# degleris1/CMF.jl

Hardware: NVIDIA B200
Metric: CNMF iterations/sec (higher is better)
Workload: dtype f32

## Files before the change

### cmf.jl_b200/_lib.py

```python
from __future__ import annotations

import ctypes
import os

import numpy as np

_HERE = os.path.dirname(os.path.abspath(__file__))
SO_PATH = os.environ.get("CMF_SM100_LIB") or os.path.join(_HERE, "libcmf_sm100.so")

F64, F32 = 0, 1
MULT, HALS, PGD = 0, 1, 2
_c = ctypes
_i64, _dbl, _int, _vp = _c.c_int64, _c.c_double, _c.c_int, _c.c_void_p
_h = _c.c_void_p

SIGNATURES = {
    "cmf_create": [_c.POINTER(_h), _i64, _i64, _i64, _i64, _int, _int, _int],
    "cmf_create_shard": [_c.POINTER(_h), _i64, _i64, _i64, _i64, _i64, _i64, _int, _int, _int],
    "cmf_create_multi": [_c.POINTER(_h), _i64, _i64, _i64, _i64, _int, _int, _int, _c.POINTER(_int)],
    "cmf_comm_unique_id": [_vp],
    "cmf_create_rank": [_c.POINTER(_h), _i64, _i64, _i64, _i64, _int, _int, _int, _vp, _int, _int],
    "cmf_shard_range": [_i64, _int, _int, _c.POINTER(_i64), _c.POINTER(_i64)],
    "cmf_comm_info": [_h, _c.POINTER(_int), _c.POINTER(_int), _c.POINTER(_i64), _c.POINTER(_i64)],
    "cmf_exchange_halos": [_h],
    "cmf_destroy": [_h],
    "cmf_set_data": [_h, _vp, _i64],
    "cmf_synth_data": [_h, _c.c_uint64, _i64, _i64, _dbl, _dbl],
    "cmf_get_data": [_h, _vp, _int],
    "cmf_data_sumsq": [_h, _c.POINTER(_dbl)],
    "cmf_set_data_norm": [_h, _dbl],
    "cmf_set_factors": [_h, _vp, _vp, _i64],
    "cmf_init_rand": [_h, _c.c_uint64],
    "cmf_init_scale_partials": [_h, _c.POINTER(_dbl)],
    "cmf_scale_factors": [_h, _dbl],
    "cmf_get_factors": [_h, _vp, _vp],
    "cmf_update_motifs": [_h, _dbl, _dbl],
    "cmf_update_feature_maps": [_h, _dbl, _dbl, _c.POINTER(_dbl)],
    "cmf_loss": [_h, _c.POINTER(_dbl)],
    "cmf_fit": [_h, _i64, _dbl, _int, _int, _int, _dbl, _dbl, _dbl, _dbl, _dbl, _c.POINTER(_dbl),
                _c.POINTER(_dbl), _i64, _c.POINTER(_i64), _c.POINTER(_int)],
    "cmf_w_partials": [_h],
    "cmf_w_apply": [_h, _dbl, _dbl],
    "cmf_h_update": [_h, _dbl, _dbl],
    "cmf_loss_partial": [_h, _c.POINTER(_dbl)],
    "cmf_exchange_buffer": [_h, _int, _c.POINTER(_vp), _c.POINTER(_i64), _c.POINTER(_int)],
    "cmf_halo_buffers": [_h, _c.POINTER(_vp), _c.POINTER(_vp), _c.POINTER(_vp), _c.POINTER(_vp),
                         _c.POINTER(_i64)],
    "cmf_sync": [_h],
    "cmf_launch_count": [_h, _c.POINTER(_i64)],
    "cmf_stream": [_h, _c.POINTER(_vp)],
    "cmf_set_stream": [_h, _vp],
    "cmf_set_engine": [_h, _int],
    "cmf_get_engine": [_h, _c.POINTER(_int)],
    "cmf_get_fd_layout": [_h, _c.POINTER(_int), _c.POINTER(_int), _c.POINTER(_i64)],
    "cmf_set_loss_mode": [_h, _int],
    "cmf_get_loss_mode": [_h, _c.POINTER(_int)],
    "cmf_set_loss_guard": [_h, _dbl, _int],
    "cmf_get_loss_stats": [_h, _c.POINTER(_i64), _c.POINTER(_i64), _c.POINTER(_int), _c.POINTER(_dbl)],
    "cmf_profile": [_h, _int],
    "cmf_profile_read": [_h, _int, _c.POINTER(_dbl), _c.POINTER(_i64)],
    "cmf_set_pgd_loss": [_h, _int, _vp],
    "cmf_set_pgd_constraints": [_h, _int, _int],
    "cmf_tensor_conv": [_i64, _i64, _i64, _i64, _int, _vp, _vp, _vp],
    "cmf_tensor_transconv": [_i64, _i64, _i64, _i64, _int, _vp, _vp, _vp],
    "cmf_corr_w": [_i64, _i64, _i64, _i64, _int, _vp, _vp, _vp],
    "cmf_compute_resids": [_i64, _i64, _i64, _i64, _int, _vp, _vp, _vp, _vp],
    "cmf_shift_and_stack": [_i64, _i64, _i64, _int, _vp, _vp],
    "cmf_create_batch": [_c.POINTER(_h), _i64, _i64, _i64, _i64, _int, _int, _i64, _int],
    "cmf_create_batch_ranks": [_c.POINTER(_h), _i64, _i64, _c.POINTER(_i64), _i64, _int, _int, _i64, _int],
    "cmf_set_factors_batch": [_h, _vp, _vp],
    "cmf_get_factors_batch": [_h, _vp, _vp],
    "cmf_init_scale_partials_batch": [_h, _c.POINTER(_dbl)],
    "cmf_scale_factors_batch": [_h, _c.POINTER(_dbl)],
    "cmf_loss_batch": [_h, _c.POINTER(_dbl)],
    "cmf_fit_batch": [_h, _i64, _dbl, _int, _int, _int, _dbl, _c.POINTER(_dbl), _c.POINTER(_dbl), _c.POINTER(_dbl),
                      _c.POINTER(_dbl), _c.POINTER(_dbl), _c.POINTER(_dbl), _i64, _c.POINTER(_i64), _c.POINTER(_int)],
}

_LIB = None


class CMFError(RuntimeError):
    def __init__(self, code, msg):
        super().__init__(f"libcmf_sm100 error {code}: {msg}")
        self.code = code


def load():
    global _LIB
    if _LIB is None:
        if not os.path.exists(SO_PATH):
            raise ImportError(
                f"{SO_PATH} is missing: build it with `python -c 'import __graft_entry__ as g; g.build()'`"
                " (the CUDA path has no CPU fallback)")
        lib = ctypes.CDLL(SO_PATH)
        for name, args in SIGNATURES.items():
            fn = getattr(lib, name)
            fn.argtypes = args
            fn.restype = _int
        lib.cmf_last_error.argtypes = []
        lib.cmf_last_error.restype = _c.c_char_p
        _LIB = lib
    return _LIB


def check(code):
    if code != 0:
        raise CMFError(code, load().cmf_last_error().decode("utf-8", "replace"))


def np_dtype(dtype):
    return np.float64 if dtype == F64 else np.float32


def parse_dtype(d):
    if d in (F64, "f64", "float64", np.float64, "Float64"):
        return F64
    if d in (F32, "f32", "float32", np.float32, "Float32"):
        return F32
    raise ValueError(f"dtype must be f64 or f32, got {d!r}")


def fptr(a):
    return a.ctypes.data_as(_vp)


def julia_array(a, dtype):
    return np.asfortranarray(a, dtype=np_dtype(dtype))
```

### cmf.jl_b200/csrc/cmf_sm100.cu

```cuda
#include "../../include/cmf_sm100.h"

#include <cuda_runtime.h>

#include <algorithm>
#include <chrono>
#include <cmath>
#include <cstdio>
#include <cstring>
#include <map>
#include <memory>
#include <numeric>
#include <mutex>
#include <tuple>
#include <stdexcept>
#include <string>
#include <vector>

#include <type_traits>
#include <variant>

#include "kernels_simt.cuh"
#include "kernels_tc.cuh"
#include "kernels_fd.cuh"
#include "kernels_hals.cuh"
// ... 143 lines not shown
CUtensorMap make_map_mn(void *base, uint64_t rows, uint64_t row_stride, uint64_t groups, uint32_t box_rows, uint32_t box_groups) {
    CUtensorMap m;
    cuuint64_t gdim[3] = {64, rows, groups};
    cuuint64_t gstr[2] = {row_stride, 128};
    cuuint32_t box[3] = {64, box_rows, box_groups};
    cuuint32_t estr[3] = {1, 1, 1};
    CUresult r = encode_tiled_fn()(&m, CU_TENSOR_MAP_DATA_TYPE_BFLOAT16, 3, base, gdim, gstr, box, estr,
                                   CU_TENSOR_MAP_INTERLEAVE_NONE, CU_TENSOR_MAP_SWIZZLE_128B, CU_TENSOR_MAP_L2_PROMOTION_L2_256B,
                                   CU_TENSOR_MAP_FLOAT_OOB_FILL_NONE);
    if (r != CUDA_SUCCESS) throw CmfError(CMF_ERR_CUDA, "cuTensorMapEncodeTiled (3-D) failed with code " + std::to_string((int)r));
    return m;
}

struct TcState {
    bool ok = false, tried = false;
    int Kp = 0, G = 0, num_sms = 148;
    int64_t KLp = 0, rows_u = 0, groups = 0, hrows = 0;
    DevBuf<__nv_bfloat16> X_hi, X_lo, Hw_hi, Hw_lo, Hm_hi, Hm_lo, Wc_hi, Wc_lo, Wu_hi, Wu_lo, Cc_hi, Cc_lo;
    CUtensorMap mWc[2], mHw[2], mHm[2], mWu[2], mXk[2], mXmn[2];
    CUtensorMap mHmn[2];
    CUtensorMap mCu[2];
    CUtensorMap mHk[2];
    CUtensorMap mGc[2];
    CUtensorMap mWuB[2], mWcB[2];
    DevBuf<__nv_bfloat16> Gc_hi, Gc_lo;
    int nsplit = 1, nsplit_g = 1;
    int64_t split_len = 0, split_len_g = 0, tiles_m = 0, tiles_n = 0, groups_c = 0, rows_c = 0;
    bool x_dirty = true, w_dirty = true;
};

struct FdState {
    bool ok = false, tried = false;
    int B = 0, logB = 0, V = 0, F = 0;
    int64_t nblk = 0, nblkp = 0;
    int Kq = 64, MR = 128;
    int V2 = 0;
    int64_t nblk2 = 0;
    DevBuf<__nv_bfloat16> Xf_hi, Xf_lo, Ah_hi, Ah_lo, Aw_hi, Aw_lo, Hf_hi, Hf_lo, Ac_hi, Ac_lo;
    DevBuf<float> Of, Df, Gf, Yf;
    DevBuf<float2> tw;
    DevBuf<__nv_bfloat16> Awm_hi, Awm_lo;
    int64_t nbc = 0;
    bool wx_dirty = true;
    CUtensorMap mXfK[2], mXfMN[2], mAw[2], mAh[2], mHfMN[2], mAc[2], mHf2K[2], mAwm[2], mHcK[2];
    bool x_dirty = true, w_dirty = true, h_dirty = true;
    bool hf2_valid = false;
    std::string why;
    void release() {
        Xf_hi.free(); Xf_lo.free(); Ah_hi.free(); Ah_lo.free(); Aw_hi.free(); Aw_lo.free(); Of.free(); Df.free();
        Hf_hi.free(); Hf_lo.free(); Gf.free(); Ac_hi.free(); Ac_lo.free(); tw.free();
        Yf.free(); Awm_hi.free(); Awm_lo.free(); nbc = 0; wx_dirty = true;
        ok = tried = false;
        x_dirty = w_dirty = h_dirty = true; hf2_valid = false;
    }
};

template <typename Fn>
void fd_with_b(int logB, Fn &&fn) {
    switch (logB) {
    case 6: fn(std::integral_constant<int, 6>{}); break;
    case 7: fn(std::integral_constant<int, 7>{}); break;
    case 8: fn(std::integral_constant<int, 8>{}); break;
    case 9: fn(std::integral_constant<int, 9>{}); break;
    case 10: fn(std::integral_constant<int, 10>{}); break;
    default: REQUIRE(false, "frequency-domain transforms: block length must be a power of two in [64, 1024]");
    }
}
template <typename Fn>
void fd_with_bc(int logB, int C, Fn &&fn) {
    fd_with_b(logB, [&](auto lb) {
        switch (C) {
        case 8: fn(lb, std::integral_constant<int, 8>{}); break;
        case 16: fn(lb, std::integral_constant<int, 16>{}); break;
        case 32: fn(lb, std::integral_constant<int, 32>{}); break;
        default: REQUIRE(false, "frequency-domain transforms: unsupported tile width");
        }
    });
}

template <typename S>
struct Ctx : RankState {
    static constexpr int dtype = std::is_same<S, double>::value ? CMF_F64 : CMF_F32;
    TcState tcs;
    FdState fds;
    DevBuf<S> X, Hbuf, Wi, Wtmp, numW, denW, GS, Cf, numH, denH, tailC;
    DevBuf<int> progress, lockstep;
    DevBuf<S> tailCt;
    int hals_grid = 0;
    DevBuf<double> exch1, corr_part, loss_part, scal;
    S *H = nullptr;
    int nsplit_w = 1, nsplit_g = 1;
    int64_t split_w = 0, split_g = 0;
    int conv_blocks_max = 0;

    static constexpr int TN = sizeof(S) == 4 ? 8 : 4;
    static constexpr int TT = 8, TY = 16;
    static constexpr int BN = 16 * TN, BT = TY * TT;

    int64_t KL() const { return K * L; }

    void hals_setup() {
        REQUIRE(L - 1 <= HW_TC, "HALS: L-1 must not exceed the sweep chunk (1024 columns)");
        const size_t smem = hals_wave_smem_elems<S>(L) * sizeof(S);
        int per_sm = 0, sms = 0, coop = 0;
        CK(cudaDeviceGetAttribute(&sms, cudaDevAttrMultiProcessorCount, device));
        CK(cudaDeviceGetAttribute(&coop, cudaDevAttrCooperativeLaunch, device));
        REQUIRE(coop != 0, "HALS needs cooperative launch support");
        CK(cudaFuncSetAttribute(hals_h_wave_kernel<S>, cudaFuncAttributeMaxDynamicSharedMemorySize, (int)smem));
        CK(cudaOccupancyMaxActiveBlocksPerMultiprocessor(&per_sm, hals_h_wave_kernel<S>, HW_NT, smem));
        hals_grid = (int)std::min<int64_t>(K, (int64_t)per_sm * sms);
        REQUIRE(hals_grid >= 1, "HALS: H sweep kernel does not fit on the device");
        tailC.alloc((size_t)hals_grid * (size_t)(L * L));
        progress.alloc((size_t)K);
    }

    void init() {
        if (R > 0) { init_batch(); return; }
        CK(cudaSetDevice(device));
        CK(cudaStreamCreateWithFlags(&stream, cudaStreamNonBlocking));
        own_stream = true;
        const int64_t hal = L - 1;
        X.alloc((size_t)((Tl + hal) * N));
        Hbuf.alloc((size_t)((Tl + 2 * hal) * K));
        H = Hbuf.p + hal * K;
        Wi.alloc((size_t)(KL() * N));
        Wtmp.alloc((size_t)(KL() * N));
        numW.alloc((size_t)(KL() * N));
        denW.alloc((size_t)(KL() * N));
        GS.alloc((size_t)(KL() * KL()));
        Cf.alloc((size_t)((2 * L - 1) * K * K));
        numH.alloc((size_t)(Tl * K));
        denH.alloc((size_t)(std::max<int64_t>(Tl * K, Tl)));
        exch1.alloc((size_t)(L * K * K + hal * K + 1));
        scal.alloc(8);
        if (alg == CMF_HALS) hals_setup();
        plan_split(N, Tl + hal, nsplit_w, split_w);
        plan_split(K, Tl + hal, nsplit_g, split_g);
        corr_part.alloc((size_t)std::max<int64_t>((int64_t)nsplit_w * KL() * N, (int64_t)nsplit_g * KL() * K));
        conv_blocks_max = (int)(cdiv(N, BN) * cdiv(Tl + hal, BT));
        loss_part.alloc((size_t)std::max(2 * conv_blocks_max, 4096));
        if constexpr (is_f32) {
            if (N >= 256 && Tl >= 4096 && K * L >= 256) {
                tc_setup();
                const char *e = getenv("CMF_ENGINE_DEFAULT");
                if (tcs.ok && engine == 1 && L >= 8 && K <= fd::KQ_MAX && !(e && atoi(e) == 1)) {
                    fd_setup();
                    if (fds.ok) { engine = 2; loss_mode = 1; }
                }
            }
        }
        CK(cudaStreamSynchronize(stream));
    }

    static constexpr bool is_f32 = std::is_same<S, float>::value;
    bool tc_active() const { return engine >= 1 && tcs.ok; }
    bool fd_active() const { return engine == 2 && tcs.ok && fds.ok; }
    bool fd_available() {
        if constexpr (is_f32) {
            if (!tc_available()) return false;
            if (!fds.ok && !fds.tried) fd_setup();
            if (fds.ok) { tcs.X_hi.free(); tcs.X_lo.free(); tcs.x_dirty = true; }
        }
        return fds.ok;
    }
    void fd_release() { fds.release(); }
    void fd_layout(int *B, int *V, int64_t *nblk) {
        *B = fd_active() ? fds.B : 0; *V = fd_active() ? fds.V : 0; *nblk = fd_active() ? fds.nblkp : 0;
    }

    void fd_setup() {
        FdState &f = fds;
        f.tried = true;
        if (!tcs.ok) { f.why = "needs the tcgen05 engine"; return; }
        if (K > fd::KQ_MAX || L > 256 || N < 16) { f.why = "needs K <= 128, L <= 256, N >= 16"; return; }
        f.Kq = (K <= 64) ? 64 : 128;
        f.MR = 2 * f.Kq;
        int B0 = 64;
        while (B0 < 8 * L && B0 < 1024) B0 *= 2;
        while (B0 < 4 * L) B0 *= 2;
        if (B0 / 2 >= 4 * L && B0 / 2 >= 64) {
            auto work = [&](int B) {
                const int64_t nb = cdiv(Tl, (int64_t)(B - (int)L + 1));
                return (double)(B / 2 + 1) * (double)(cdiv(nb, tc::BN) * tc::BN + cdiv(nb, 16) * 16);
            };
            if (work(B0) > 0.97 * work(B0 / 2)) B0 /= 2;
        }
        int forced = 0;
        if (const char *e = getenv("CMF_FD_B")) {
            const int want = atoi(e);
            if (want >= 4 * L && want >= 64 && want <= 1024 && (want & (want - 1)) == 0) forced = want;
        }
        tcs.X_hi.free(); tcs.X_lo.free(); tcs.x_dirty = true;
        size_t free_b = 0, total_b = 0;
        CK(cudaMemGetInfo(&free_b, &total_b));
        size_t later = (size_t)1 << 30;
        if (alg == CMF_HALS) later += (size_t)2 * (size_t)(Tl + 2048) * (size_t)K * 4 + (size_t)hals2::RING * (size_t)cdiv(K, hals2::GS) * (size_t)K * hals2::CW * 4;
        size_t xf = 0, ah = 0, aw = 0, of = 0, df = 0, hf = 0, gf = 0, ac = 0;
        bool fits = false;
        for (int B = forced ? forced : B0; B <= (forced ? forced : std::min(2 * B0, 1024)); B *= 2) {
            int logB = 0;
            while ((1 << logB) < B) ++logB;
            f.B = B; f.logB = logB; f.V = B - (int)L + 1; f.F = B / 2 + 1;
            f.nblk = cdiv(Tl, f.V);
            f.nblkp = cdiv(f.nblk, 16) * 16;
            xf = (size_t)f.F * (size_t)f.nblkp * 2 * (size_t)N + 64;
            ah = (size_t)f.F * (size_t)f.nblkp * 2 * f.MR + 64;
            aw = (size_t)f.F * f.MR * 2 * (size_t)N + 64;
            f.V2 = B - 2 * (int)L + 2;
            f.nblk2 = cdiv(Tl, f.V2);
            of = (size_t)f.F * (size_t)std::max(f.nblkp, f.nblk2) * f.MR; df = (size_t)f.F * f.MR * (size_t)N;
            hf = (size_t)f.F * (size_t)std::max(f.nblkp, f.nblk2) * 2 * f.Kq + 256; gf = (size_t)f.F * f.MR * f.Kq;
            ac = (size_t)f.F * f.MR * f.MR;
            const size_t need = 4 * (xf + ah + aw + hf + ac) + 4 * (of + df + gf);
            const size_t loss_pass = 4 * aw + (size_t)256 * (size_t)f.F * 2 * (size_t)N * sizeof(float);
            if (need + later + loss_pass <= free_b) { fits = true; break; }
        }
        if (!fits) { f.why = "not enough device memory for the spectrum of X"; return; }
        f.Xf_hi.alloc(xf); f.Xf_lo.alloc(xf);
        f.Ah_hi.alloc(ah); f.Ah_lo.alloc(ah);
        f.Aw_hi.alloc(aw); f.Aw_lo.alloc(aw);
        f.Of.alloc(of); f.Df.alloc(df);
        f.Hf_hi.alloc(hf); f.Hf_lo.alloc(hf); f.Gf.alloc(gf);
        f.Ac_hi.alloc(ac); f.Ac_lo.alloc(ac);
        f.tw.alloc((size_t)f.B);
        fd::twiddle_kernel<<<(unsigned)cdiv(f.B, 256), 256, 0, stream>>>(f.tw.p, f.B);
        post_launch();
        __nv_bfloat16 *xs[2] = {f.Xf_hi.p, f.Xf_lo.p}, *as[2] = {f.Ah_hi.p, f.Ah_lo.p}, *ws[2] = {f.Aw_hi.p, f.Aw_lo.p};
        const uint64_t rows = (uint64_t)f.F * (uint64_t)f.nblkp;
        for (int i = 0; i < 2; ++i) {
            f.mXfK[i] = make_map_2d(xs[i], (uint64_t)(2 * N), rows, (uint64_t)N * 4, tc::BK, tc::BN, CU_TENSOR_MAP_SWIZZLE_64B);
            f.mXfMN[i] = make_map_mn(xs[i], rows * 2, (uint64_t)N * 2, (uint64_t)cdiv(N, 64), tc::BK, 4);
            f.mAw[i] = make_map_2d(ws[i], (uint64_t)(2 * N), (uint64_t)f.F * f.MR, (uint64_t)N * 4, tc::BK, tc::BM, CU_TENSOR_MAP_SWIZZLE_64B);
            f.mAh[i] = make_map_mn(as[i], rows * 2, (uint64_t)f.MR * 2, (uint64_t)(f.MR / 64), tc::BK, 2);
            f.mHfMN[i] = make_map_mn(i == 0 ? f.Hf_hi.p : f.Hf_lo.p, rows * 2, (uint64_t)f.Kq * 2, (uint64_t)(f.Kq / 64), tc::BK, 4);
            f.mAc[i] = make_map_2d(i == 0 ? f.Ac_hi.p : f.Ac_lo.p, f.MR, (uint64_t)f.F * f.MR, (uint64_t)f.MR * 2, tc::BK, tc::BM, CU_TENSOR_MAP_SWIZZLE_64B);
            f.mHf2K[i] = make_map_2d(i == 0 ? f.Hf_hi.p : f.Hf_lo.p, f.MR, (uint64_t)f.F * (uint64_t)f.nblk2, (uint64_t)f.MR * 2, tc::BK, tc::BN, CU_TENSOR_MAP_SWIZZLE_64B);
        }
        CK(cudaFuncSetAttribute(tc::tc_kernel<tc::TC_FQT>, cudaFuncAttributeMaxDynamicSharedMemorySize, tc::SMEM_BYTES));
        CK(cudaFuncSetAttribute(tc::tc_kernel<tc::TC_FQC>, cudaFuncAttributeMaxDynamicSharedMemorySize, tc::SMEM_BYTES));
        CK(cudaFuncSetAttribute(tc::tc_kernel<tc::TC_FQX>, cudaFuncAttributeMaxDynamicSharedMemorySize, tc::SMEM_BYTES));

        fd_with_b(f.logB, [&](auto lb) {
            constexpr int LB = decltype(lb)::value;
            const int x16 = (int)fd_smem(16), w = (int)fd_smem(fd_cols_w());
            CK(cudaFuncSetAttribute(fd::fft_x_kernel<LB>, cudaFuncAttributeMaxDynamicSharedMemorySize, x16));
            CK(cudaFuncSetAttribute(fd::ifft_resid_kernel<LB>, cudaFuncAttributeMaxDynamicSharedMemorySize, x16));
            fd_with_bc(f.logB, fd_cols_w(), [&](auto, auto c) {
                constexpr int CW = decltype(c)::value;
                CK(cudaFuncSetAttribute(fd::fft_w_kernel<LB, CW>, cudaFuncAttributeMaxDynamicSharedMemorySize, w));
                CK(cudaFuncSetAttribute(fd::ifft_numW_kernel<float, LB, CW>, cudaFuncAttributeMaxDynamicSharedMemorySize, w));
                CK(cudaFuncSetAttribute(fd::ifft_numW_kernel<double, LB, CW>, cudaFuncAttributeMaxDynamicSharedMemorySize, w));
            });
            for (int ch : {8, 16, 32}) {
                if (LB == 10 && ch == 32) continue;
                const int h = (int)fd_smem(ch);
                fd_with_bc(f.logB, ch, [&](auto, auto c) {
                    constexpr int CH = decltype(c)::value;
                    CK(cudaFuncSetAttribute(fd::fft_h_kernel<LB, CH>, cudaFuncAttributeMaxDynamicSharedMemorySize, h));
                    CK(cudaFuncSetAttribute(fd::ifft_numH_kernel<LB, CH>, cudaFuncAttributeMaxDynamicSharedMemorySize, h));
                });
            }
        });
        f.x_dirty = f.w_dirty = f.h_dirty = true;
        f.ok = true;
    }
    int fd_cols_h() const {
        if (const char *e = getenv("CMF_FD_COLS")) {
            const int c = atoi(e);
            if ((c == 8 || c == 16 || c == 32) && (size_t)fds.B * (size_t)c * sizeof(float2) <= 160 * 1024) return c;
        }
        return fds.B >= 1024 ? 8 : 16;
    }
    int64_t fd_order(int64_t nblocks) const { static const int o = getenv("CMF_FD_ORDER") ? atoi(getenv("CMF_FD_ORDER")) : 0; return o ? nblocks : 0; }
    int fd_cols_w() const { return fds.B >= 1024 ? 8 : 16; }
    size_t fd_smem(int C) const { return ((size_t)fds.B * (size_t)C + (size_t)fds.B) * sizeof(float2); }
    void fd_fft_h(__nv_bfloat16 *hi, __nv_bfloat16 *lo, int64_t nb, int V, int full, int64_t t_off) {
        const int C = fd_cols_h();
        fd_with_bc(fds.logB, C, [&](auto lb, auto c) {
            fd::fft_h_kernel<decltype(lb)::value, decltype(c)::value><<<(unsigned)(nb * (fds.Kq / 2 / C)), fd::NT, fd_smem(C), stream>>>(
                H, hi, lo, K, Tl, Tl + (L - 1), V, nb, full, t_off, fds.Kq, fd_order(nb), fds.tw.p);
        });
    }
    void fd_ifft_numH(const float *Of, float *out, int64_t nb, int V, int64_t nblkp_) {
        const int C = fd_cols_h();
        fd_with_bc(fds.logB, C, [&](auto lb, auto c) {
            fd::ifft_numH_kernel<decltype(lb)::value, decltype(c)::value><<<(unsigned)(nb * (fds.Kq / 2 / C)), fd::NT, fd_smem(C), stream>>>(
                Of, out, K, Tl, V, nblkp_, fds.Kq, fd_order(nb), fds.tw.p);
        });
    }
    void fd_fft_w(const float *src, __nv_bfloat16 *hi, __nv_bfloat16 *lo, int64_t Nw, int64_t Lw, int64_t ldw, int64_t coff, int xmode) {
        const int C = fd_cols_w();
        fd_with_bc(fds.logB, C, [&](auto lb, auto c) {
            fd::fft_w_kernel<decltype(lb)::value, decltype(c)::value><<<dim3((unsigned)cdiv(Nw, 2 * C), (unsigned)K), fd::NT, fd_smem(C), stream>>>(
                src, hi, lo, Nw, K, Lw, ldw, coff, xmode, fds.Kq, fds.tw.p);
        });
    }
    template <typename OutT>
    void fd_ifft_numW(const float *Df, OutT *out, int64_t Nw, int64_t ldi) {
        const int C = fd_cols_w();
        fd_with_bc(fds.logB, C, [&](auto lb, auto c) {
            fd::ifft_numW_kernel<OutT, decltype(lb)::value, decltype(c)::value><<<dim3((unsigned)cdiv(Nw, 2 * C), (unsigned)K), fd::NT, fd_smem(C), stream>>>(
                Df, out, Nw, ldi, K, L, fds.Kq, fds.tw.p);
        });
    }

    void fd_build_X() {
        FdState &f = fds;
        if (!f.x_dirty) return;
        dim3 grid((unsigned)(f.nblkp * cdiv(N, 32)));
        fd_with_b(f.logB, [&](auto lb) {
            fd::fft_x_kernel<decltype(lb)::value><<<grid, fd::NT, fd_smem(16), stream>>>(X.p, f.Xf_hi.p, f.Xf_lo.p, N, Tl + (L - 1), f.V, f.nblkp,
                                                                                        fd_order(f.nblkp), f.tw.p);
        });
        post_launch();
        f.x_dirty = false;
    }
    void fd_corr() {
        FdState &f = fds;
        fd_build_X();
        fd_spectrum_H();
        tc::Params q = tc_base_params();
        q.nprod = 3;
        q.tiles_n = cdiv(N, tc::BN);
        q.nkb = f.nblkp * 2 / tc::BK;
        q.MR = f.MR; q.mtiles = f.MR / tc::BM; q.units = (int64_t)f.F * q.tiles_n * q.mtiles;
        q.fq_rows = f.nblkp * 2;
        q.out = f.Df.p; q.Mrows = f.MR; q.Ncols = N; q.ldo = N;
        const unsigned grid = (unsigned)std::min<int64_t>(q.units, tcs.num_sms);
        prof_begin(PROF_CORR);
        tc::tc_kernel<tc::TC_FQC><<<grid, tc::THREADS, tc::SMEM_BYTES, stream>>>(f.mAh[0], f.mAh[1], f.mXfMN[0], f.mXfMN[1], q);
        prof_end();
        post_launch();
        fd_ifft_numW(f.Df.p, numW.p, N, N);
        post_launch();
    }
    void fd_denomH() {
        FdState &f = fds;
        fd_fft_w(Cf.p, f.Ac_hi.p, f.Ac_lo.p, K, 2 * L - 1, f.MR, f.Kq, 0);
        post_launch();
        fd_denomH_prefetch();
        f.hf2_valid = false;
        tc::Params q = tc_base_params();
        q.nprod = 3;
        q.tiles_n = cdiv(f.nblk2, tc::BN);
        q.nkb = f.MR / tc::BK;
        q.MR = f.MR; q.mtiles = f.MR / tc::BM; q.units = (int64_t)f.F * q.tiles_n * q.mtiles;
        q.fq_rows = f.nblk2;
        q.out = f.Of.p;
        const unsigned grid = (unsigned)std::min<int64_t>(q.units, tcs.num_sms);
        tc::tc_kernel<tc::TC_FQT><<<grid, tc::THREADS, tc::SMEM_BYTES, stream>>>(f.mAc[0], f.mAc[1], f.mHf2K[0], f.mHf2K[1], q);
        post_launch();
        fd_ifft_numH(f.Of.p, denH.p, f.nblk2, f.V2, f.nblk2);
        post_launch();
    }
    void fd_denomH_prefetch() {
        if constexpr (is_f32) {
            FdState &f = fds;
            if (!fd_active() || f.hf2_valid) return;
            fd_fft_h(f.Hf_hi.p, f.Hf_lo.p, f.nblk2, f.V2, 1, -(L - 1));
            post_launch();
            f.hf2_valid = true;
        }
    }
    int64_t fd_conv_loss() {
        FdState &f = fds;
        f.hf2_valid = false;
        const int64_t ntile32 = cdiv(N, 32);
        if (f.Awm_hi.n == 0) {
            const size_t aw = (size_t)f.F * 2 * f.MR * (size_t)N + 64;
            size_t free_b = 0, total_b = 0;
            CK(cudaMemGetInfo(&free_b, &total_b));
            const size_t per_block = (size_t)f.F * 2 * (size_t)N * sizeof(float);
            REQUIRE(free_b > 4 * aw + 256 * per_block + ((size_t)1 << 29), "not enough device memory for the frequency-domain loss pass");
            size_t budget = std::min<size_t>((free_b - 4 * aw - ((size_t)1 << 29)) / 2, (size_t)12 << 30);
            int64_t nbc = (int64_t)(budget / per_block) / tc::BN * tc::BN;
            nbc = std::max<int64_t>(tc::BN, std::min<int64_t>(nbc, cdiv(f.nblk, tc::BN) * tc::BN));
            if (const char *e = getenv("CMF_FD_NBC")) { const int64_t v = atoll(e); if (v >= tc::BN && v % tc::BN == 0 && v < nbc) nbc = v; }
            f.nbc = nbc;
            f.Awm_hi.alloc(aw); f.Awm_lo.alloc(aw);
            f.Yf.alloc((size_t)f.F * (size_t)nbc * 2 * (size_t)N);
            for (int i = 0; i < 2; ++i) {
                f.mAwm[i] = make_map_mn(i == 0 ? f.Awm_hi.p : f.Awm_lo.p, (uint64_t)f.F * 2 * f.MR, (uint64_t)N * 2, (uint64_t)cdiv(N, 64), tc::BK, 2);
                f.mHcK[i] = make_map_2d(i == 0 ? f.Hf_hi.p : f.Hf_lo.p, f.MR, (uint64_t)f.F * (uint64_t)f.nblk, (uint64_t)f.MR * 2, tc::BK, tc::BN, CU_TENSOR_MAP_SWIZZLE_64B);
            }
            f.wx_dirty = true;
        }
        const size_t need_lp = (size_t)(f.nblk * ntile32);
        if (loss_part.n < need_lp) loss_part.alloc(std::max<size_t>(need_lp, 4096));
        if (f.wx_dirty) {
            fd_fft_w(Wi.p, f.Awm_hi.p, f.Awm_lo.p, N, L, 2 * N, N, 1);
            post_launch();
            f.wx_dirty = false;
        }
        fd_fft_h(f.Hf_hi.p, f.Hf_lo.p, f.nblk, f.V, 1, -(L - 1));
        post_launch();
        prof_begin(PROF_CONV);
        for (int64_t b0 = 0; b0 < f.nblk; b0 += f.nbc) {
            const int64_t cur = std::min(f.nbc, f.nblk - b0);
            tc::Params q = tc_base_params();
            q.nprod = 3;
            q.tiles_n = cdiv(cur, tc::BN);
            q.tiles_m = cdiv(N, tc::BM);
            q.nkb = f.MR / tc::BK;
            q.MR = f.MR; q.mtiles = 1; q.units = (int64_t)f.F * 2 * q.tiles_m * q.tiles_n;
            q.fq_rows = f.nblk; q.b_off = b0; q.nbc = cur;
            q.out = f.Yf.p;
            const unsigned grid = (unsigned)std::min<int64_t>(q.units, tcs.num_sms);
            tc::tc_kernel<tc::TC_FQX><<<grid, tc::THREADS, tc::SMEM_BYTES, stream>>>(f.mAwm[0], f.mAwm[1], f.mHcK[0], f.mHcK[1], q);
            post_launch();
            fd_with_b(f.logB, [&](auto lb) {
                fd::ifft_resid_kernel<decltype(lb)::value><<<(unsigned)(cur * ntile32), fd::NT, fd_smem(16), stream>>>(
                    f.Yf.p, X.p, loss_part.p + b0 * ntile32, N, Tl, L, f.V, cur, b0, fd_order(cur), f.tw.p);
            });
            post_launch();
        }
        prof_end();
        return f.nblk * ntile32;
    }
    void fd_spectrum_H() {
        FdState &f = fds;
        if (!f.h_dirty) return;
        fd_fft_h(f.Ah_hi.p, f.Ah_lo.p, f.nblkp, f.V, 0, 0);
        post_launch();
        f.h_dirty = false;
    }
    void fd_gram() {
        FdState &f = fds;
        f.hf2_valid = false;
        fd_spectrum_H();
        fd_fft_h(f.Hf_hi.p, f.Hf_lo.p, f.nblkp, f.V, 1, 0);
        post_launch();
        tc::Params q = tc_base_params();
        q.nprod = 3;
        q.tiles_n = 1;
        q.nkb = f.nblkp * 2 / tc::BK;
        q.MR = f.MR; q.mtiles = f.MR / tc::BM; q.units = (int64_t)f.F * q.mtiles;
        q.fq_rows = f.nblkp * 2;
        q.out = f.Gf.p; q.Mrows = f.MR; q.Ncols = K; q.ldo = f.Kq;
        const unsigned grid = (unsigned)std::min<int64_t>(q.units, tcs.num_sms);
        tc::tc_kernel<tc::TC_FQC><<<grid, tc::THREADS, tc::SMEM_BYTES, stream>>>(f.mAh[0], f.mAh[1], f.mHfMN[0], f.mHfMN[1], q);
        post_launch();
        fd_ifft_numW(f.Gf.p, exch1.p, K, f.Kq);
        post_launch();
    }
    void fd_transconv() {
        FdState &f = fds;
        fd_build_X();
        if (f.w_dirty) {
            fd_fft_w(Wi.p, f.Aw_hi.p, f.Aw_lo.p, N, L, 2 * N, N, 0);
            post_launch();
            f.w_dirty = false;
        }
        tc::Params q = tc_base_params();
        q.nprod = 3;
        q.tiles_n = cdiv(f.nblkp, tc::BN);
        q.nkb = cdiv(2 * N, tc::BK);
        q.MR = f.MR; q.mtiles = f.MR / tc::BM; q.units = (int64_t)f.F * q.tiles_n * q.mtiles;
        q.fq_rows = f.nblkp;
        q.out = f.Of.p;
        const unsigned grid = (unsigned)std::min<int64_t>(q.units, tcs.num_sms);
        prof_begin(PROF_TRANSCONV);
        tc::tc_kernel<tc::TC_FQT><<<grid, tc::THREADS, tc::SMEM_BYTES, stream>>>(f.mAw[0], f.mAw[1], f.mXfK[0], f.mXfK[1], q);
        prof_end();
        post_launch();
        fd_ifft_numH(f.Of.p, numH.p, f.nblk, f.V, f.nblkp);
        post_launch();
    }
    bool tc_available() {
        if constexpr (is_f32) {
            if (!tcs.ok && !tcs.tried) tc_setup();
        }
        return tcs.ok;
    }

    void tc_setup() {
        TcState &t = tcs;
        t.tried = true;
        if (K > 128 || N % 8 != 0) return;
        t.Kp = (int)(cdiv(K, 8) * 8);
        t.G = 128 / t.Kp;
        t.KLp = cdiv(L * t.Kp, 64) * 64;
        t.groups = cdiv(L, t.G);
        t.rows_u = cdiv(L * t.Kp + 128, 128) * 128;
        const int64_t hal = L - 1;
        t.hrows = Tl + hal;
        cudaDeviceProp prop;
        CK(cudaGetDeviceProperties(&prop, device));
        if (prop.major != 10) return;
        t.num_sms = prop.multiProcessorCount;
        t.Wc_hi.alloc((size_t)(N * t.KLp)); t.Wc_lo.alloc((size_t)(N * t.KLp));
        t.Wu_hi.alloc((size_t)(t.rows_u * N)); t.Wu_lo.alloc((size_t)(t.rows_u * N));
        t.groups_c = cdiv(2 * L - 1, t.G);
        t.rows_c = cdiv((2 * L - 1) * t.Kp + 128, 128) * 128;
        t.Cc_hi.alloc((size_t)(t.rows_c * t.Kp)); t.Cc_lo.alloc((size_t)(t.rows_c * t.Kp));
        t.Gc_hi.alloc((size_t)(KL() * t.KLp)); t.Gc_lo.alloc((size_t)(KL() * t.KLp));
        if (GS.n < (size_t)(t.rows_u * t.rows_u)) GS.alloc((size_t)(t.rows_u * t.rows_u));
        __nv_bfloat16 *wc[2] = {t.Wc_hi.p, t.Wc_lo.p};
        __nv_bfloat16 *wu[2] = {t.Wu_hi.p, t.Wu_lo.p};
        for (int i = 0; i < 2; ++i) {
            t.mWc[i] = make_map_2d(wc[i], (uint64_t)t.KLp, (uint64_t)N, (uint64_t)t.KLp * 2, tc::BK, tc::BM, CU_TENSOR_MAP_SWIZZLE_64B);
            t.mWu[i] = make_map_2d(wu[i], (uint64_t)N, (uint64_t)t.rows_u, (uint64_t)N * 2, tc::BK, tc::BM, CU_TENSOR_MAP_SWIZZLE_64B);
            __nv_bfloat16 *cc[2] = {t.Cc_hi.p, t.Cc_lo.p};
            t.mCu[i] = make_map_2d(cc[i], (uint64_t)t.Kp, (uint64_t)t.rows_c, (uint64_t)t.Kp * 2, tc::BK, tc::BM, CU_TENSOR_MAP_SWIZZLE_64B);
            __nv_bfloat16 *gc[2] = {t.Gc_hi.p, t.Gc_lo.p};
            t.mWuB[i] = make_map_2d(wu[i], (uint64_t)N, (uint64_t)t.rows_u, (uint64_t)N * 2, tc::BK, tc::BN, CU_TENSOR_MAP_SWIZZLE_64B);
            t.mWcB[i] = make_map_2d(wc[i], (uint64_t)t.KLp, (uint64_t)N, (uint64_t)t.KLp * 2, tc::BK, tc::BN, CU_TENSOR_MAP_SWIZZLE_64B);
            t.mGc[i] = make_map_2d(gc[i], (uint64_t)t.KLp, (uint64_t)KL(), (uint64_t)t.KLp * 2, tc::BK, tc::BM, CU_TENSOR_MAP_SWIZZLE_64B);
        }
        t.tiles_m = cdiv(t.KLp, tc::BM);
        t.tiles_n = cdiv(N, tc::BN);
        const int64_t tau = Tl + hal, base = t.tiles_m * t.tiles_n;
        double best = -1.0;
        for (int ns = 1; ns <= 16; ++ns) {
            const int64_t sl = cdiv(cdiv(tau, ns), tc::BK) * tc::BK;
            if (ns > 1 && sl < tc::FLUSH_T) break;
            const int64_t units = base * cdiv(tau, sl);
            const double eff = (double)units / (double)(cdiv(units, t.num_sms) * t.num_sms);
            if (eff > best + 1e-9) { best = eff; t.nsplit = (int)cdiv(tau, sl); t.split_len = sl; }
        }
        {
            const int64_t want = std::max<int64_t>(1, cdiv(2 * t.num_sms, t.tiles_m));
            const int64_t maxs = std::max<int64_t>(1, tau / tc::FLUSH_T);
            const int64_t ns = std::min(want, maxs);
            t.split_len_g = cdiv(cdiv(tau, ns), tc::BK) * tc::BK;
            t.nsplit_g = (int)cdiv(tau, t.split_len_g);
        }
        const size_t need = std::max((size_t)t.nsplit * (size_t)(KL() * N), (size_t)t.nsplit_g * (size_t)(KL() * K));
        if (corr_part.n < need) corr_part.alloc(need);
        const size_t need_lp = (size_t)(tc::EPI_WARPS * cdiv(Tl, tc::BN) * cdiv(N, tc::BM));
        if (loss_part.n < need_lp) loss_part.alloc(std::max<size_t>(need_lp, 4096));
        CK(cudaFuncSetAttribute(tc::tc_kernel<tc::TC_CONV>, cudaFuncAttributeMaxDynamicSharedMemorySize, tc::SMEM_BYTES));
        CK(cudaFuncSetAttribute(tc::tc_kernel<tc::TC_TRANS>, cudaFuncAttributeMaxDynamicSharedMemorySize, tc::SMEM_BYTES));
        CK(cudaFuncSetAttribute(tc::tc_kernel<tc::TC_CORR>, cudaFuncAttributeMaxDynamicSharedMemorySize, tc::SMEM_BYTES));
        CK(cudaFuncSetAttribute(tc::tc_kernel<tc::TC_PLAIN>, cudaFuncAttributeMaxDynamicSharedMemorySize, tc::SMEM_BYTES));
        t.ok = true;
        t.x_dirty = t.w_dirty = true;
        if (N >= 256 && Tl >= 4096 && K * L >= 256) engine = 1;
    }

    tc::Params tc_base_params() {
        tc::Params q;
        memset(&q, 0, sizeof(q));
        q.N = N; q.K = K; q.L = L; q.Tl = Tl; q.G = tcs.G; q.Kp = tcs.Kp;
        { const char *e = getenv("CMF_PROMO"); q.promo = e ? std::max(1, atoi(e)) : tc::PROMO; }
        { const char *e = getenv("CMF_TC_PRODUCTS"); q.nprod = (e && atoi(e) == 2) ? 2 : 3; }
        return q;
    }

    void tc_split_X() {
        if (!tcs.ok || !tcs.x_dirty) return;
        TcState &t = tcs;
        if (t.X_hi.n == 0) {
            const int64_t hal = L - 1;
            t.X_hi.alloc(X.n + 64); t.X_lo.alloc(X.n + 64);
            __nv_bfloat16 *xs[2] = {t.X_hi.p, t.X_lo.p};
            for (int i = 0; i < 2; ++i) {
                t.mXk[i] = make_map_2d(xs[i], (uint64_t)N, (uint64_t)(Tl + hal), (uint64_t)N * 2, tc::BK, tc::BN, CU_TENSOR_MAP_SWIZZLE_64B);
                t.mXmn[i] = make_map_mn(xs[i], (uint64_t)(Tl + hal), (uint64_t)N * 2, (uint64_t)cdiv(N, 64), tc::BK, 4);
            }
        }
        tc::split_plain_kernel<<<(unsigned)cdiv((int64_t)X.n, 256), 256, 0, stream>>>(X.p, tcs.X_hi.p, tcs.X_lo.p, (int64_t)X.n);
        post_launch();
        tcs.x_dirty = false;
    }
    void tc_split_W() {
        if (!tcs.w_dirty) return;
        tc::split_W_kernel<<<dim3((unsigned)cdiv(N, 32), (unsigned)cdiv(tcs.Kp, 32), (unsigned)L), dim3(32, 8), 0, stream>>>(
            Wi.p, tcs.Wc_hi.p, tcs.Wc_lo.p, tcs.Wu_hi.p, tcs.Wu_lo.p, N, K, L, tcs.Kp, tcs.KLp);
        post_launch();
        tcs.w_dirty = false;
    }
    void tc_h_planes() {
        TcState &t = tcs;
        if (t.Hw_hi.n != 0) return;
        const int64_t hal = L - 1;
        const size_t hw_elems = (size_t)((Tl + 2 * hal) * t.Kp + t.KLp + 64);
        t.Hw_hi.alloc(hw_elems); t.Hw_lo.alloc(hw_elems);
        t.Hm_hi.alloc(hw_elems); t.Hm_lo.alloc(hw_elems);
        __nv_bfloat16 *hw[2] = {t.Hw_hi.p, t.Hw_lo.p}, *hm[2] = {t.Hm_hi.p, t.Hm_lo.p};
        for (int i = 0; i < 2; ++i) {
            t.mHw[i] = make_map_2d(hw[i], (uint64_t)t.KLp, (uint64_t)t.hrows, (uint64_t)t.Kp * 2, tc::BK, tc::BN, CU_TENSOR_MAP_SWIZZLE_64B);
            t.mHm[i] = make_map_mn(hm[i], (uint64_t)t.hrows, (uint64_t)t.Kp * 2, (uint64_t)(t.KLp / 64), tc::BK, 2);
            t.mHmn[i] = make_map_mn(hw[i] + hal * t.Kp, (uint64_t)(Tl + hal), (uint64_t)t.Kp * 2, (uint64_t)cdiv(t.Kp, 64), tc::BK, 4);
            t.mHk[i] = make_map_2d(hw[i], (uint64_t)t.Kp, (uint64_t)(Tl + 2 * hal), (uint64_t)t.Kp * 2, tc::BK, tc::BN, CU_TENSOR_MAP_SWIZZLE_64B);
        }
    }
    void tc_split_H(bool masked) {
        tc_h_planes();
        const int64_t rows = Tl + 2 * (L - 1);
        tc::split_H_kernel<<<(unsigned)cdiv(rows * tcs.Kp, 256), 256, 0, stream>>>(
            Hbuf.p, masked ? tcs.Hm_hi.p : tcs.Hw_hi.p, masked ? tcs.Hm_lo.p : tcs.Hw_lo.p, rows, K, tcs.Kp,
            L - 1, L - 1 + Tl, masked ? 1 : 0);
        post_launch();
    }

    void tc_corr() {
        tc_split_X();
        tc_split_H(true);
        tc::Params q = tc_base_params();
        q.tiles_m = tcs.tiles_m; q.tiles_n = tcs.tiles_n; q.split_len = tcs.split_len; q.tau_hi = Tl + (L - 1);
        q.units = tcs.tiles_m * tcs.tiles_n * tcs.nsplit;
        q.part = corr_part.p;
        q.corr_order = 0;
        {
            const char *e = getenv("CMF_LOCKSTEP");
            const int w = e ? atoi(e) : 256;
            if (w > 0) {
                if (lockstep.n == 0) lockstep.alloc(1024);
                CK(cudaMemsetAsync(lockstep.p, 0, lockstep.n * sizeof(int), stream));
                q.lockstep = lockstep.p; q.lockstep_window = w;
            }
        }
        const unsigned grid = (unsigned)std::min<int64_t>(q.units, tcs.num_sms);
        prof_begin(PROF_CORR);
        if (q.lockstep != nullptr) {
            void *args[] = {&tcs.mHm[0], &tcs.mHm[1], &tcs.mXmn[0], &tcs.mXmn[1], &q};
            CK(cudaLaunchCooperativeKernel((void *)tc::tc_kernel<tc::TC_CORR>, dim3(grid), dim3(tc::THREADS), args, tc::SMEM_BYTES, stream));
        } else {
            tc::tc_kernel<tc::TC_CORR><<<grid, tc::THREADS, tc::SMEM_BYTES, stream>>>(tcs.mHm[0], tcs.mHm[1], tcs.mXmn[0], tcs.mXmn[1], q);
// ... 169 lines not shown
        const int HW = BT + Lpad - 1;
        const size_t ws_bytes = (size_t)CONV_LC * BN * sizeof(S);
        const size_t budget = 160 * 1024 - ws_bytes;
        int KC = (int)std::min<int64_t>(Kc, (int64_t)(budget / ((size_t)HW * sizeof(S))));
        REQUIRE(KC >= 1, "conv: L too large for the shared-memory H window");
        a.KC = KC;
        const size_t smem = (size_t)KC * HW * sizeof(S) + ws_bytes;
        auto kern = conv_kernel<S, TN, TT, TY>;
        CK(cudaFuncSetAttribute(kern, cudaFuncAttributeMaxDynamicSharedMemorySize, (int)smem));
        dim3 grid((unsigned)cdiv(t_hi - t_lo, BT), (unsigned)cdiv(N, BN), (unsigned)(per_restart ? R : 1));
        prof_begin(PROF_CONV);
        kern<<<grid, dim3(16, TY), smem, stream>>>(a);
        prof_end();
        post_launch();
    }
    int conv_nblocks(int64_t t_lo, int64_t t_hi) const { return (int)(cdiv(N, BN) * cdiv(t_hi - t_lo, BT)); }

    void reduce_scalar(const double *part, int64_t n, double *dst, int nrest = 1) {
        reduce_sum_kernel<<<(unsigned)nrest, 1024, 0, stream>>>(part, n, dst);
        post_launch();
    }
    double fetch_scalar(const double *dst) {
        double v;
        CK(cudaMemcpyAsync(&v, dst, sizeof(double), cudaMemcpyDeviceToHost, stream));
        CK(cudaStreamSynchronize(stream));
        return v;
    }

    void launch_transconv(const S *Wg, const S *Xin, S *out, int64_t Nin, int64_t Kout, int64_t Lin,
                          int64_t ldx, int64_t t_out, int64_t x_cols, bool per_restart = false, int64_t ldo = 0,
                          size_t *split_need = nullptr) {
        const int nrest = per_restart ? (int)R : 1;
        if (t_out <= 0) return;
        int best_tk = 8, best_kg = 1;
        double best_waste = 1e30;
        const int tks[3] = {8, 5, 4};
        for (int tk : tks) {
            int kg = 1;
            while (kg < 16 && kg * tk < Kout) kg *= 2;
            const int64_t kp = (int64_t)kg * tk;
            const double waste = (double)(cdiv(Kout, kp) * kp - Kout) / (double)Kout;
            if (waste < best_waste - 1e-9) { best_waste = waste; best_tk = tk; best_kg = kg; }
        }
        int tg = std::max(128 / best_kg, 8);
        while (tg * best_kg > 32 && cdiv(t_out, (int64_t)tg * 8) < 296) tg /= 2;
        TransArgs<S> a;
        a.Wg = Wg; a.Xin = Xin; a.out = out; a.Nin = Nin; a.Kout = Kout; a.Lin = Lin; a.ldx = ldx;
        a.t_out = t_out; a.x_cols = x_cols; a.kgroups = best_kg; a.tgroups = tg;
        a.ldo = ldo ? ldo : Kout; a.tab = per_restart ? b_tab.p : nullptr;
        const int BTt = tg * 8, Lpad = (int)(cdiv(Lin, 8) * 8);
        const int XW = BTt + Lpad, XWP = XW + XW / 8 + 1, KP = best_kg * best_tk;
        const size_t smem = ((size_t)TR_NC * XWP + (size_t)8 * TR_NC * KP) * sizeof(S);
        REQUIRE(smem <= 200 * 1024, "transconv: L too large for the shared-memory window");
        dim3 grid((unsigned)cdiv(t_out, BTt), (unsigned)cdiv(Kout, KP), (unsigned)nrest);
        const int nthr = best_kg * tg;
        int nsplit = 1;
        a.n_chunk = cdiv(Nin, TR_NC) * TR_NC; a.part_stride = 0;
        const int64_t ctas = (int64_t)grid.x * grid.y;
        if (nrest == 1 && ctas < 296 && Nin >= 64) {
            const int64_t want = std::min<int64_t>(std::min<int64_t>(cdiv(Nin, 32), cdiv(296, ctas)), 32);
            a.n_chunk = cdiv(cdiv(Nin, want), TR_NC) * TR_NC;
            nsplit = (int)cdiv(Nin, a.n_chunk);
            if (nsplit > 1) {
                a.part_stride = t_out * Kout;
                const size_t need = (size_t)nsplit * (size_t)a.part_stride;
                if (split_need) { *split_need = need; return; }
                if (tr_part.n < need) tr_part.alloc(need);
                a.out = tr_part.p;
                a.ldo = Kout;
                grid.z = (unsigned)nsplit;
            }
        }
        if (split_need) { *split_need = 0; return; }
        a.nsplit = nsplit;
#define LAUNCH_TR(TKV)                                                                             \
    {                                                                                              \
        auto kern = transconv_kernel<S, TKV, 8>;                                                   \
        CK(cudaFuncSetAttribute(kern, cudaFuncAttributeMaxDynamicSharedMemorySize, (int)smem));    \
        kern<<<grid, nthr, smem, stream>>>(a);                                                     \
    }
        if (Nin == N) prof_begin(PROF_TRANSCONV);
        if (best_tk == 8) LAUNCH_TR(8) else if (best_tk == 5) LAUNCH_TR(5) else LAUNCH_TR(4)
#undef LAUNCH_TR
        prof_end();
        post_launch();
        if (nsplit > 1) {
            sum_parts_kernel<S><<<(unsigned)cdiv(a.part_stride, 256), 256, 0, stream>>>(tr_part.p, out, a.part_stride, a.part_stride, nsplit);
            post_launch();
        }
    }
    DevBuf<S> tr_part;

    void launch_corr(const S *Xin, int64_t Nin, int64_t ldx, int64_t tau_hi, int nsplit, int64_t split_len,
                     S *out_s, double *out_d, const S *Hs = nullptr, int64_t Kc = 0, int64_t ldh = 0, bool per_restart = false) {
        if (!Hs) Hs = H;
        if (!Kc) Kc = K;
        CorrArgs<S> a;
        a.H = Hs; a.Xin = Xin; a.part = corr_part.p; a.Nin = Nin; a.K = Kc; a.L = L; a.ldx = ldx;
        a.u_hi = Tl; a.tau_hi = tau_hi; a.split_len = split_len;
        a.ldh = ldh ? ldh : Kc; a.nsplit = nsplit;
        const int64_t n = L * Kc * Nin;
        const BatchRest *tab = per_restart ? b_tab.p : nullptr;
        const int nrest = per_restart ? (int)R : 1;
        a.tab = tab;
        const int64_t ngrp = cdiv(L, 8);
        dim3 grid((unsigned)cdiv(Nin, 128), (unsigned)cdiv(Kc * ngrp, CORR_PB), (unsigned)(nsplit * nrest));
        if (Nin == N) prof_begin(PROF_CORR);
        corr_kernel<S><<<grid, dim3(16, 16), 0, stream>>>(a);
        prof_end();
        post_launch();
        reduce_partials_kernel<S><<<dim3((unsigned)cdiv(n, 256), (unsigned)nrest), 256, 0, stream>>>(corr_part.p, nsplit, n, out_s, out_d, tab, L);
        post_launch();
    }

    static GemmRows rows(int64_t ld) { return GemmRows{ld, INT64_MAX, 0, RANK_NONE}; }
    template <bool TB>
    void launch_gemm(const S *A, const S *B, S *C, int64_t M, int64_t Nn, int64_t Kg, int64_t lda, int64_t ldb,
                     int64_t ldc) {
        launch_gemm_rows<TB>(A, B, C, M, Nn, Kg, rows(lda), rows(ldb), rows(ldc), false);
    }
    template <bool TB>
    void launch_gemm_rows(const S *A, const S *B, S *C, int64_t M, int64_t Nn, int64_t Kg, GemmRows ra, GemmRows rb, GemmRows rc,
                          bool per_restart) {
        dim3 grid((unsigned)cdiv(Nn, 64), (unsigned)cdiv(M, 64), (unsigned)(per_restart ? R : 1));
        gemm_kernel<S, TB><<<grid, 256, 0, stream>>>(A, B, C, M, Nn, Kg, ra, rb, rc, per_restart ? b_tab.p : nullptr, L);
        post_launch();
    }

    DevBuf<double> mu_part;
    bool launch_mu(S *x, const S *num, const S *den, double l1, double l2, int64_t n, double *dot_dst = nullptr) {
        if constexpr (is_f32) {
            const bool aligned = (((uintptr_t)x | (uintptr_t)num | (uintptr_t)den) & 15) == 0;
            if (aligned && n % 4 == 0 && n >= 4096) {
                const unsigned grid = (unsigned)std::min<int64_t>(cdiv(n / 4, 256), 148 * 8);
                if (dot_dst && mu_part.n == 0) mu_part.alloc(148 * 8);
                mu_update_vec4_kernel<<<grid, 256, 0, stream>>>(reinterpret_cast<float4 *>(x), reinterpret_cast<const float4 *>(num),
                                                                reinterpret_cast<const float4 *>(den), (float)l1, (float)l2, n / 4,
                                                                dot_dst ? mu_part.p : nullptr);
                post_launch();
                if (dot_dst) reduce_scalar(mu_part.p, grid, dot_dst);
                return dot_dst != nullptr;
            }
        }
        mu_update_kernel<S><<<(unsigned)cdiv(n, 256), 256, 0, stream>>>(x, num, den, (S)l1, (S)l2, n);
        post_launch();
        return false;
    }

    void x_changed() {
        tcs.x_dirty = fds.x_dirty = true;
        numH_valid = numH_dot_valid = false;
        calib_reset();
    }
    void w_changed() {
        tcs.w_dirty = fds.w_dirty = fds.wx_dirty = true;
        numH_valid = numH_dot_valid = false;
    }
    void h_changed() {
        gram_valid = false; fds.h_dirty = true; fds.hf2_valid = false;
        numH_valid = numH_dot_valid = false;
    }
    void factors_replaced() { w_changed(); h_changed(); calib_reset(); }

    void set_data(const void *Xh, int64_t first_col) {
        REQUIRE(Xh != nullptr, "set_data: null pointer");
        REQUIRE(first_col <= t0, "set_data: host array starts after the shard's first column");
        const int64_t hi = std::min(t1 + (L - 1), T);
        CK(cudaMemsetAsync(X.p, 0, X.n * sizeof(S), stream));
        const S *src = static_cast<const S *>(Xh) + (t0 - first_col) * N;
        CK(cudaMemcpyAsync(X.p, src, (size_t)((hi - t0) * N) * sizeof(S), cudaMemcpyHostToDevice, stream));
        finish_data();
    }
    void get_data(void *X_out, int with_halo) {
        const int64_t cols = with_halo ? std::min(t1 + (L - 1), T) - t0 : Tl;
        CK(cudaMemcpyAsync(X_out, X.p, (size_t)(cols * N) * sizeof(S), cudaMemcpyDeviceToHost, stream));
        CK(cudaStreamSynchronize(stream));
    }
    void finish_data() {
        x_changed();
        data_sumsq_local = data_sumsq();
        data_norm = std::sqrt(data_sumsq_local);
        pgd_cur_loss = data_norm;
        have_data = true;
    }
    double data_sumsq() {
        dot_partial_kernel<S><<<1024, 256, 0, stream>>>(X.p, X.p, Tl * N, loss_part.p);
        post_launch();
        reduce_scalar(loss_part.p, 1024, scal.p);
        return fetch_scalar(scal.p);
    }

    void synth_data(uint64_t seed, int64_t Kt, int64_t Lt, double p_h, double noise) {
        REQUIRE(Kt >= 1 && Lt >= 1, "synth_data: bad ground-truth dims");
        DevBuf<S> Wt, Ht;
        Wt.alloc((size_t)(Kt * Lt * N));
        const int64_t cols_out = std::min(Tl + (L - 1), T - t0);
        const int64_t hcols = cols_out + (Lt - 1);
        Ht.alloc((size_t)(hcols * Kt));
        synth_W_kernel<S><<<(unsigned)cdiv(N, 128), 128, 0, stream>>>(Wt.p, Kt, N, Lt, seed, 0.1, 0.2);
        post_launch();
        synth_H_kernel<S><<<(unsigned)cdiv(hcols * Kt, 256), 256, 0, stream>>>(Ht.p, Kt, t0 - (Lt - 1), hcols, T, seed, p_h);
        post_launch();
        CK(cudaMemsetAsync(X.p, 0, X.n * sizeof(S), stream));
        launch_conv(Wt.p, Ht.p + (Lt - 1) * Kt, Kt, Lt, -(Lt - 1), cols_out, 0, cols_out, 8, X.p, nullptr, seed, noise);
        CK(cudaStreamSynchronize(stream));
        finish_data();
    }

    void set_factors(const void *Wh, const void *Hh, int64_t first_col) {
        REQUIRE(Wh && Hh, "set_factors: null pointer");
        const int64_t lo = std::max<int64_t>(t0 - (L - 1), 0), hi = std::min(t1 + (L - 1), T);
        REQUIRE(first_col <= lo, "set_factors: host H starts after the shard's left halo");
        CK(cudaMemcpyAsync(Wtmp.p, Wh, Wi.n * sizeof(S), cudaMemcpyHostToDevice, stream));
        w_julia_to_internal<S><<<(unsigned)cdiv(KL() * N, 256), 256, 0, stream>>>(Wtmp.p, Wi.p, K, N, L, K);
        post_launch();
        CK(cudaMemsetAsync(Hbuf.p, 0, Hbuf.n * sizeof(S), stream));
        const S *src = static_cast<const S *>(Hh) + (lo - first_col) * K;
        CK(cudaMemcpyAsync(H + (lo - t0) * K, src, (size_t)((hi - lo) * K) * sizeof(S), cudaMemcpyHostToDevice, stream));
        CK(cudaStreamSynchronize(stream));
        have_factors = true;
        factors_replaced();
        pgd_stepW = pgd_stepH = 5.0;
        pgd_cur_loss = data_norm;
    }

    void init_rand(uint64_t seed) {
        uniform_kernel<S><<<(unsigned)cdiv(KL() * N, 256), 256, 0, stream>>>(Wtmp.p, KL() * N, seed, 100, 0);
        post_launch();
        w_julia_to_internal<S><<<(unsigned)cdiv(KL() * N, 256), 256, 0, stream>>>(Wtmp.p, Wi.p, K, N, L, K);
        post_launch();
        const int64_t lo = std::max<int64_t>(t0 - (L - 1), 0), hi = std::min(t1 + (L - 1), T);
        CK(cudaMemsetAsync(Hbuf.p, 0, Hbuf.n * sizeof(S), stream));
        uniform_kernel<S><<<(unsigned)cdiv((hi - lo) * K, 256), 256, 0, stream>>>(H + (lo - t0) * K, (hi - lo) * K, seed, 101, lo * K);
        post_launch();
        CK(cudaStreamSynchronize(stream));
        have_factors = true;
        factors_replaced();
    }

    void init_scale_partials(double out[2]) {
        REQUIRE(have_data && have_factors, "init_scale_partials: data and factors must be set");
        const int nb = conv_nblocks(0, Tl);
        launch_conv(Wi.p, H, K, L, -(L - 1), Tl + (L - 1), 0, Tl, 16, nullptr, loss_part.p);
        std::vector<double> hp((size_t)2 * nb);
        CK(cudaMemcpyAsync(hp.data(), loss_part.p, hp.size() * sizeof(double), cudaMemcpyDeviceToHost, stream));
        CK(cudaStreamSynchronize(stream));
        double a = 0.0, b = 0.0;
        for (int i = 0; i < nb; ++i) { a += hp[2 * i]; b += hp[2 * i + 1]; }
        out[0] = a; out[1] = b;
    }

    void scale_factors(double s) {
        scale_kernel<S><<<(unsigned)cdiv(KL() * N, 256), 256, 0, stream>>>(Wi.p, (S)s, KL() * N);
        post_launch();
        scale_kernel<S><<<(unsigned)cdiv((int64_t)Hbuf.n, 256), 256, 0, stream>>>(Hbuf.p, (S)s, (int64_t)Hbuf.n);
        post_launch();
        factors_replaced();
    }

    void get_factors(void *Wo, void *Ho) {
        if (Wo) {
            w_internal_to_julia<S><<<(unsigned)cdiv(KL() * N, 256), 256, 0, stream>>>(Wi.p, Wtmp.p, K, N, L, K);
            post_launch();
            CK(cudaMemcpyAsync(Wo, Wtmp.p, Wi.n * sizeof(S), cudaMemcpyDeviceToHost, stream));
        }
        if (Ho) CK(cudaMemcpyAsync(Ho, H, (size_t)(Tl * K) * sizeof(S), cudaMemcpyDeviceToHost, stream));
        CK(cudaStreamSynchronize(stream));
    }

    std::vector<int64_t> b_K;
    std::vector<BatchRest> b_rest;
    int64_t b_C = 0;
    DevBuf<BatchRest> b_tab;
    DevBuf<int> b_col;
    DevBuf<double> b_reg, b_vals;
    DevBuf<int> b_active;
    int64_t b_exch(int64_t Kr) const { return L * Kr * Kr + (L - 1) * Kr + 1; }
    int64_t b_tail_blocks(int64_t Kr) const { return cdiv((2 * L - 1) * Kr, 256); }
    GemmRows b_wrows() const { return GemmRows{N, INT64_MAX, b_C * N, RANK_W}; }
    GemmRows b_grows() const { return GemmRows{0, INT64_MAX, 0, RANK_G}; }

    size_t batch_buffers(bool alloc) {
        size_t bytes = 0;
        auto take = [&](auto &buf, int64_t count) {
            bytes += (size_t)count * sizeof(*buf.p);
            if (alloc) buf.alloc((size_t)count);
        };
        const int64_t hal = L - 1, KLR = L * b_C;
        plan_split(N, Tl + hal, nsplit_w, split_w, b_C, 1);
        plan_split(K, Tl + hal, nsplit_g, split_g, K, R);
        b_rest.assign((size_t)R, BatchRest{});
        BatchRest e{};
        for (int64_t r = 0; r < R; ++r) {
            const int64_t Kr = b_K[(size_t)r];
            e.K = Kr;
            b_rest[(size_t)r] = e;
            e.off += Kr; e.gs += (Kr * L) * (Kr * L); e.cf += (2 * L - 1) * Kr * Kr; e.ex += b_exch(Kr);
            e.cp += (int64_t)nsplit_g * L * Kr * Kr; e.tp += b_tail_blocks(Kr) * hal * Kr;
        }
        size_t tr_need = 0;
        launch_transconv(nullptr, nullptr, nullptr, N, b_C, L, N, Tl, Tl + hal, false, 0, &tr_need);
        const int nb = conv_nblocks(0, Tl);
        take(X, (Tl + hal) * N);
        take(Hbuf, (Tl + 2 * hal) * b_C);
        take(Wi, KLR * N); take(Wtmp, KLR * N); take(numW, KLR * N); take(denW, KLR * N);
        take(GS, e.gs);
        take(Cf, e.cf);
        take(numH, Tl * b_C); take(denH, Tl * b_C);
        take(exch1, e.ex);
        take(corr_part, std::max<int64_t>((int64_t)nsplit_w * KLR * N, e.cp));
        take(loss_part, std::max<int64_t>(2 * nb * R, 4096));
        take(tail_part, e.tp);
        take(tr_part, (int64_t)tr_need);
        take(scal, 8);
        take(b_reg, 4 * R); take(b_vals, R); take(b_active, R);
        take(b_tab, R); take(b_col, b_C);
        return bytes;
    }

    void init_batch() {
        CK(cudaSetDevice(device));
        size_t free_b = 0, total_b = 0;
        CK(cudaMemGetInfo(&free_b, &total_b));
        const size_t need = batch_buffers(false);
        if (need > free_b)
            throw CmfError(CMF_ERR_ARG, "batch handle: " + std::to_string(R) + " restarts need " + std::to_string(need) +
                                            " bytes of device memory (" + std::to_string(b_C) + " stacked components); " +
                                            std::to_string(free_b) + " bytes are free");
        CK(cudaStreamCreateWithFlags(&stream, cudaStreamNonBlocking));
        own_stream = true;
        H = nullptr;
        batch_buffers(true);
        H = Hbuf.p + (L - 1) * b_C;
        conv_blocks_max = conv_nblocks(0, Tl);
        std::vector<int> col((size_t)b_C);
        for (int64_t r = 0; r < R; ++r)
            for (int64_t k = 0; k < b_K[(size_t)r]; ++k) col[(size_t)(b_rest[(size_t)r].off + k)] = (int)r;
        CK(cudaMemcpyAsync(b_tab.p, b_rest.data(), (size_t)R * sizeof(BatchRest), cudaMemcpyHostToDevice, stream));
        CK(cudaMemcpyAsync(b_col.p, col.data(), col.size() * sizeof(int), cudaMemcpyHostToDevice, stream));
        CK(cudaStreamSynchronize(stream));
    }

    void batch_set_factors(const void *Wh, const void *Hh) {
        REQUIRE(Wh && Hh, "cmf_set_factors_batch: null pointer");
        CK(cudaMemcpyAsync(Wtmp.p, Wh, Wtmp.n * sizeof(S), cudaMemcpyHostToDevice, stream));
        w_julia_to_internal<S><<<dim3((unsigned)cdiv(KL() * N, 256), (unsigned)R), 256, 0, stream>>>(Wtmp.p, Wi.p, K, N, L, b_C, b_tab.p);
        post_launch();
        CK(cudaMemsetAsync(Hbuf.p, 0, Hbuf.n * sizeof(S), stream));
        CK(cudaMemcpyAsync(numH.p, Hh, numH.n * sizeof(S), cudaMemcpyHostToDevice, stream));
        h_stack_kernel<S><<<(unsigned)cdiv(b_C * Tl, 256), 256, 0, stream>>>(numH.p, H, b_C, Tl, b_tab.p, b_col.p, 1);
        post_launch();
        CK(cudaStreamSynchronize(stream));
        have_factors = true;
    }
    void batch_get_factors(void *Wo, void *Ho) {
        REQUIRE(have_factors, "no factors");
        if (Wo) {
            w_internal_to_julia<S><<<dim3((unsigned)cdiv(KL() * N, 256), (unsigned)R), 256, 0, stream>>>(Wi.p, Wtmp.p, K, N, L, b_C, b_tab.p);
            post_launch();
            CK(cudaMemcpyAsync(Wo, Wtmp.p, Wtmp.n * sizeof(S), cudaMemcpyDeviceToHost, stream));
        }
        if (Ho) {
            h_stack_kernel<S><<<(unsigned)cdiv(b_C * Tl, 256), 256, 0, stream>>>(H, numH.p, b_C, Tl, b_tab.p, b_col.p, 0);
            post_launch();
            CK(cudaMemcpyAsync(Ho, numH.p, numH.n * sizeof(S), cudaMemcpyDeviceToHost, stream));
        }
        CK(cudaStreamSynchronize(stream));
    }

    void batch_scale_partials(double *out) {
        REQUIRE(have_data && have_factors, "cmf_init_scale_partials_batch: data and factors must be set");
        const int nb = conv_nblocks(0, Tl);
        launch_conv(Wi.p, H, K, L, -(L - 1), Tl + (L - 1), 0, Tl, 16, nullptr, loss_part.p, 0, 0.0, true, 2 * nb);
        std::vector<double> hp((size_t)(2 * nb * R));
        CK(cudaMemcpyAsync(hp.data(), loss_part.p, hp.size() * sizeof(double), cudaMemcpyDeviceToHost, stream));
        CK(cudaStreamSynchronize(stream));
        for (int64_t r = 0; r < R; ++r) {
            const double *p = hp.data() + 2 * nb * r;
            double a = 0.0, b = 0.0;
            for (int i = 0; i < nb; ++i) { a += p[2 * i]; b += p[2 * i + 1]; }
            out[2 * r] = a; out[2 * r + 1] = b;
        }
    }
    void batch_scale(const double *s) {
        CK(cudaMemcpyAsync(b_vals.p, s, (size_t)R * sizeof(double), cudaMemcpyHostToDevice, stream));
        scale_kernel<S><<<(unsigned)cdiv((int64_t)Wi.n, 256), 256, 0, stream>>>(Wi.p, S(1), (int64_t)Wi.n, b_vals.p, N, b_col.p, b_C);
        post_launch();
        scale_kernel<S><<<(unsigned)cdiv((int64_t)Hbuf.n, 256), 256, 0, stream>>>(Hbuf.p, S(1), (int64_t)Hbuf.n, b_vals.p, 1, b_col.p, b_C);
        post_launch();
        CK(cudaStreamSynchronize(stream));
    }

    void batch_loss(double *out) {
        REQUIRE(have_data && have_factors, "loss: data and factors must be set first");
        const int nb = conv_nblocks(0, Tl);
        launch_conv(Wi.p, H, K, L, -(L - 1), Tl + (L - 1), 0, Tl, 4, nullptr, loss_part.p, 0, 0.0, true, nb);
        reduce_scalar(loss_part.p, nb, b_vals.p, (int)R);
        CK(cudaMemcpyAsync(out, b_vals.p, (size_t)R * sizeof(double), cudaMemcpyDeviceToHost, stream));
        CK(cudaStreamSynchronize(stream));
        for (int64_t r = 0; r < R; ++r) out[r] = std::sqrt(std::max(out[r], 0.0)) / data_norm;
    }

    void batch_set_state(const double *reg, const int *active) {
        if (reg) CK(cudaMemcpyAsync(b_reg.p, reg, (size_t)(4 * R) * sizeof(double), cudaMemcpyHostToDevice, stream));
        if (active) CK(cudaMemcpyAsync(b_active.p, active, (size_t)R * sizeof(int), cudaMemcpyHostToDevice, stream));
        CK(cudaStreamSynchronize(stream));
    }

    void batch_update_motifs() {
        REQUIRE(have_data && have_factors, "update: data and factors must be set first");
        launch_corr(X.p, N, N, Tl + (L - 1), nsplit_w, split_w, numW.p, nullptr, H, b_C, b_C);
        launch_corr(H, K, b_C, Tl + (L - 1), nsplit_g, split_g, nullptr, exch1.p, H, K, b_C, true);
        if (L > 1) {
            h_tail_kernel<S><<<dim3((unsigned)cdiv((L - 1) * K, 256), (unsigned)R), 256, 0, stream>>>(H, exch1.p, K, L, Tl, 1, b_C,
                                                                                                   b_tab.p);
            post_launch();
        }
        build_G_kernel<S><<<dim3((unsigned)cdiv(KL() * KL(), 256), (unsigned)R), 256, 0, stream>>>(exch1.p, nullptr, GS.p, K, L,
                                                                                                    b_tab.p);
        post_launch();
        launch_gemm_rows<false>(GS.p, Wi.p, denW.p, KL(), N, KL(), b_grows(), b_wrows(), b_wrows(), true);
        mu_update_kernel<S><<<(unsigned)cdiv((int64_t)Wi.n, 256), 256, 0, stream>>>(Wi.p, numW.p, denW.p, S(0), S(0), (int64_t)Wi.n,
                                                                                     b_reg.p, b_active.p, N, b_col.p, b_C);
        post_launch();
    }

    void batch_update_feature_maps() {
        REQUIRE(have_data && have_factors, "update: data and factors must be set first");
        launch_transconv(Wi.p, X.p, numH.p, N, b_C, L, N, Tl, Tl + (L - 1));
        launch_gemm_rows<true>(Wi.p, Wi.p, GS.p, KL(), KL(), N, b_wrows(), b_wrows(), b_grows(), true);
        lag_table_kernel<S><<<dim3((unsigned)cdiv((2 * L - 1) * K * K, 256), (unsigned)R), 256, 0, stream>>>(GS.p, Cf.p, K, L, K, KL(),
                                                                                                          b_tab.p);
        post_launch();
        launch_transconv(Cf.p, Hbuf.p, denH.p, K, K, 2 * L - 1, b_C, Tl, Tl + 2 * (L - 1), true, b_C);
        if (L > 1) {
            denomH_tail_prefix_kernel<S><<<dim3((unsigned)b_tail_blocks(K), (unsigned)K, (unsigned)R), 256,
                                           (size_t)8 * (size_t)(L - 1) * sizeof(double), stream>>>(GS.p, H, tail_part.p, K, L, Tl,
                                                                                                    -(L - 1), K, KL(), b_C, b_tab.p);
            post_launch();
            denomH_tail_reduce_kernel<S><<<dim3((unsigned)cdiv((L - 1) * K, 256), (unsigned)R), 256, 0, stream>>>(tail_part.p, denH.p, K, L,
                                                                                                                Tl, 0, b_C, b_tab.p);
            post_launch();
        }
        mu_update_kernel<S><<<(unsigned)cdiv(Tl * b_C, 256), 256, 0, stream>>>(H, numH.p, denH.p, S(0), S(0), Tl * b_C, b_reg.p + 2,
                                                                                 b_active.p, 1, b_col.p, b_C);
        post_launch();
    }


    void compute_numW() {
        if (!tc_active()) launch_corr(X.p, N, N, Tl + (L - 1), nsplit_w, split_w, numW.p, nullptr);
        else if constexpr (is_f32) { if (fd_active()) fd_corr(); else tc_corr(); }
    }
    void compute_numH() {
        if (!tc_active()) launch_transconv(Wi.p, X.p, numH.p, N, K, L, N, Tl, Tl + (L - 1));
        else if constexpr (is_f32) { if (fd_active()) fd_transconv(); else tc_transconv(); }
    }
    void compute_denomW(int64_t j0, int64_t j1) {
        if (!tc_active()) {
            build_G();
            launch_gemm<false>(GS.p + j0 * KL(), Wi.p, denW.p + j0 * N, j1 - j0, N, KL(), KL(), N, N);
        } else if constexpr (is_f32) {
            tc_denomW(j0, j1);
        }
    }
    void compute_denomH() {
        lag_tables();
        if (!tc_active()) launch_transconv(Cf.p, Hbuf.p, denH.p, K, K, 2 * L - 1, K, Tl, Tl + 2 * (L - 1));
        else if constexpr (is_f32) {
            if (fd_active()) fd_denomH();
            else { tc_split_H(false); tc_denomH(); }
        }
        if (is_last && L > 1) launch_denomH_tail();
    }
    void gram_partial() {
        if (!tc_active()) launch_corr(H, K, K, Tl + (L - 1), nsplit_g, split_g, nullptr, exch1.p);
        else if constexpr (is_f32) {
            if (fd_active()) fd_gram();
            else { tc_split_H(true); tc_split_H(false); tc_gram(); }
        }
        if (L > 1) {
            h_tail_kernel<S><<<(unsigned)cdiv((L - 1) * K, 256), 256, 0, stream>>>(H, exch1.p + L * K * K, K, L, Tl, is_last ? 1 : 0, K);
            post_launch();
        }
    }

    void build_G() {
        build_G_kernel<S><<<(unsigned)cdiv(KL() * KL(), 256), 256, 0, stream>>>(exch1.p, exch1.p + L * K * K, GS.p, K, L);
        post_launch();
    }

    void w_partials() {
        REQUIRE(have_data && have_factors, "update: data and factors must be set first");
        compute_numW();
        if (!gram_valid) gram_partial();
        gram_valid = false;
    }

    void w_apply(double l1W, double l2W) {
        if (alg == CMF_HALS) { hals_w_apply(l1W, l2W); return; }
        REQUIRE(alg == CMF_MULT, "the split-phase W update serves MultUpdate and HALSUpdate");
        w_denom_rows(0, KL());
        w_update_rows(l1W, l2W, 0, KL());
    }
    void w_denom_rows(int64_t j0, int64_t j1) { compute_denomW(j0, j1); }
    void w_update_rows(double l1W, double l2W, int64_t j0, int64_t j1) {
        launch_mu(Wi.p + j0 * N, numW.p + j0 * N, denW.p + j0 * N, l1W, l2W, (j1 - j0) * N);
        w_changed();
    }
    void w_rows_buffers(void **numw, void **w, int64_t *row_elems) { *numw = numW.p; *w = Wi.p; *row_elems = N; }

    int64_t s2_ks = 0, s2_ld = 0;

    void lag_tables() {
        if (!tc_active()) {
            launch_gemm<true>(Wi.p, Wi.p, GS.p, KL(), KL(), N, N, N, KL());
            s2_ks = K; s2_ld = KL();
        } else if constexpr (is_f32) {
            tc_split_W();
            tc_plain(tcs.mWu, tcs.mWuB, GS.p, tcs.rows_u, tcs.rows_u, N, tcs.rows_u, true);
            s2_ks = tcs.Kp; s2_ld = tcs.rows_u;
        }
        lag_table_kernel<S><<<(unsigned)cdiv((2 * L - 1) * K * K, 256), 256, 0, stream>>>(GS.p, Cf.p, K, L, s2_ks, s2_ld);
        post_launch();
    }

    DevBuf<double> tail_part;
    void launch_denomH_tail() {
        const int nb = (int)cdiv((2 * L - 1) * K, 256);
        const size_t smem = (size_t)8 * (size_t)(L - 1) * sizeof(double);
        if (getenv("CMF_TAIL_DIRECT") || smem > 48 * 1024) {
            dim3 grid((unsigned)(L - 1), (unsigned)K);
            denomH_tail_kernel<S><<<grid, 256, 0, stream>>>(GS.p, H, denH.p, K, L, Tl, -(L - 1), s2_ks, s2_ld);
            post_launch();
            return;
        }
        const size_t need = (size_t)nb * (size_t)(L - 1) * (size_t)K;
        if (tail_part.n < need) tail_part.alloc(need);
        denomH_tail_prefix_kernel<S><<<dim3((unsigned)nb, (unsigned)K), 256, smem, stream>>>(GS.p, H, tail_part.p, K, L, Tl, -(L - 1), s2_ks, s2_ld,
                                                                                            K);
        post_launch();
        denomH_tail_reduce_kernel<S><<<(unsigned)cdiv((L - 1) * K, 256), 256, 0, stream>>>(tail_part.p, denH.p, K, L, Tl, nb, K);
        post_launch();
    }

    void h_update(double l1H, double l2H) {
        REQUIRE(have_data && have_factors, "update: data and factors must be set first");
        compute_numH();
        compute_denomH();
        const bool dot = launch_mu(H, numH.p, denH.p, l1H, l2H, Tl * K, (loss_mode == 1 && alg == CMF_MULT) ? scal.p + 4 : nullptr);
        h_changed();
        numH_valid = (alg == CMF_MULT);
        numH_dot_valid = dot;
    }

    double *scalars() { return scal.p; }

    int loss_partial_dev() {
        REQUIRE(have_data && have_factors, "loss: data and factors must be set first");
        if (loss_mode == 1 && tc_active()) {
            if (!numH_valid && fd_active()) { compute_numH(); lag_tables(); numH_valid = true; numH_dot_valid = false; }
            if (numH_valid) { loss_partial_expansion_dev(); return 2; }
        }
        int64_t nb = conv_nblocks(0, Tl);
        if (!tc_active()) launch_conv(Wi.p, H, K, L, -(L - 1), Tl + (L - 1), 0, Tl, 4, nullptr, loss_part.p);
        else if constexpr (is_f32) nb = (fd_active() && !getenv("CMF_FD_LOSS_TC")) ? fd_conv_loss() : tc_conv_loss();
        reduce_scalar(loss_part.p, nb, scal.p);
        CK(cudaMemsetAsync(scal.p + 1, 0, sizeof(double), stream));
        return 1;
    }

    double loss_partial() {
        const int n = loss_partial_dev();
        double bc[2];
        CK(cudaMemcpyAsync(bc, scal.p, 2 * sizeof(double), cudaMemcpyDeviceToHost, stream));
        CK(cudaStreamSynchronize(stream));
        return n == 2 ? data_sumsq_local - 2.0 * bc[0] + bc[1] : bc[0];
    }

    void loss_partial_expansion_dev() {
        gram_partial();
        gram_valid = true;
        if (getenv("CMF_G_DIRECT"))
            s2_dot_G_kernel<S><<<1024, 256, 0, stream>>>(GS.p, s2_ks, s2_ld, exch1.p, exch1.p + L * K * K, K, L, loss_part.p + 1024);
        else
            s2_dot_G_diag_kernel<S><<<1024, 256, 0, stream>>>(GS.p, s2_ks, s2_ld, exch1.p, exch1.p + L * K * K, K, L, loss_part.p + 1024);
        post_launch();
        reduce_scalar(loss_part.p + 1024, 1024, scal.p + 1);
        if (numH_dot_valid) {
            CK(cudaMemcpyAsync(scal.p, scal.p + 4, sizeof(double), cudaMemcpyDeviceToDevice, stream));
            numH_dot_valid = false;
            return;
        }
        dot_partial_kernel<S><<<1024, 256, 0, stream>>>(numH.p, H, Tl * K, loss_part.p);
        post_launch();
        reduce_scalar(loss_part.p, 1024, scal.p);
    }

    void hals_w_apply(double l1W, double l2W) {
        compute_denomW(0, KL());
        if (tc_active()) build_G();
        sub_kernel<S><<<(unsigned)cdiv(KL() * N, 256), 256, 0, stream>>>(numW.p, denW.p, numW.p, KL() * N);
        post_launch();
        const size_t smem = (size_t)KL() * sizeof(S);
        REQUIRE(smem <= 200 * 1024, "HALS W sweep: K*L too large for shared memory");
        auto kern = hals_w_sweep_kernel<S>;
        CK(cudaFuncSetAttribute(kern, cudaFuncAttributeMaxDynamicSharedMemorySize, (int)smem));
        kern<<<(unsigned)N, 256, smem, stream>>>(GS.p, numW.p, Wi.p, K, L, N, (S)l1W, (S)l2W);
        post_launch();
        w_changed();
    }

    void hals_h_prepare() {
        REQUIRE(have_data && have_factors, "update: data and factors must be set first");
        compute_numH();
        compute_denomH();
        sub_kernel<S><<<(unsigned)cdiv(Tl * K, 256), 256, 0, stream>>>(numH.p, denH.p, numH.p, Tl * K);
        post_launch();
    }
    void hals_h_local(void **q, void **h, int64_t *count) { *q = numH.p; *h = H; *count = Tl * K; }
    DevBuf<S> Qfull, Hfull, Dfull;
    void hals_h_full(void **q, void **h) {
        const size_t n = (size_t)(T * K);
        if (Qfull.n < n) { Qfull.alloc(n); Hfull.alloc(n); Dfull.alloc(n); }
        *q = Qfull.p; *h = Hfull.p;
    }

    DevBuf<float> h2_Hcm, h2_AD, h2_part, h2_coef;
    DevBuf<unsigned> h2_bar;
    int h2_max_ctas = -1;
    bool hals2_sweep(const S *Qp, S *Hp, int64_t Tt, const S *ct, double l1H, double l2H) {
        if constexpr (!is_f32) { return false; } else {
            if (L > hals2::LMAX || K > 128 || (L > 1 && ct == nullptr)) return false;
            if (const char *e = getenv("CMF_HALS_SWEEP")) { if (atoi(e) == 1) return false; }
            const int G = (int)cdiv(K, hals2::GS);
            const int n_block = G * (G - 1) / 2, n_diag = G, n_rec = (int)cdiv(K, 32);
            const int grid = n_block + n_diag + n_rec;
            const size_t smem = hals2::smem_bytes();
            if (h2_max_ctas < 0) {
                int per_sm = 0, sms = 0;
                CK(cudaDeviceGetAttribute(&sms, cudaDevAttrMultiProcessorCount, device));
                cudaError_t e1 = cudaFuncSetAttribute(hals2::hals2_sweep_kernel, cudaFuncAttributeMaxDynamicSharedMemorySize, (int)smem);
                cudaError_t e2 = cudaOccupancyMaxActiveBlocksPerMultiprocessor(&per_sm, hals2::hals2_sweep_kernel, hals2::NT, smem);
                h2_max_ctas = (e1 == cudaSuccess && e2 == cudaSuccess) ? per_sm * sms : 0;
                if (e1 != cudaSuccess || e2 != cudaSuccess) cudaGetLastError();
            }
            if (grid > h2_max_ctas) return false;
            const int64_t nC = cdiv(Tt, hals2::CW), Tp = nC * hals2::CW;
            const size_t ncm = (size_t)hals2::cells_elems(K, nC), npart = (size_t)G * (size_t)K * hals2::RING * hals2::CW;
            if (h2_Hcm.n < ncm) { h2_Hcm.alloc(ncm); h2_AD.alloc(ncm); }
            if (h2_part.n < npart) h2_part.alloc(npart);
            dim3 tb(32, 8), tg((unsigned)cdiv(Tp, 32), (unsigned)cdiv(K, 32));
            hals2::hals2_prepare_kernel<<<tg, tb, 0, stream>>>(Qp, Hp, h2_AD.p, h2_Hcm.p, K, Tt, Tp);
            post_launch();
            if (h2_coef.n < (size_t)(K * 64)) h2_coef.alloc((size_t)(K * 64));
            hals2::hals2_coef_kernel<<<(unsigned)cdiv(K * 64, 256), 256, 0, stream>>>(Cf.p, h2_coef.p, K, L, (float)l2H);
            post_launch();
            if (h2_bar.n == 0) h2_bar.alloc(32);
            CK(cudaMemsetAsync(h2_bar.p, 0, sizeof(unsigned), stream));
            hals2::Args a;
            a.barrier = h2_bar.p;
            a.coef = h2_coef.p;
            a.Cf = Cf.p; a.Ct = ct; a.S2 = GS.p; a.Ks = s2_ks; a.ld = s2_ld;
            a.H_cm = h2_Hcm.p; a.AD_cm = h2_AD.p; a.part = h2_part.p;
            a.K = K; a.L = L; a.T = Tt; a.nC = nC;
            a.l1 = (float)l1H; a.l2 = (float)l2H;
            a.G = G; a.n_block_items = n_block; a.n_diag_items = n_diag; a.n_rec = n_rec;
            DevBuf<long long> dbgbuf;
            const bool dbg2 = getenv("CMF_HALS_DEBUG") && atoi(getenv("CMF_HALS_DEBUG")) == 1;
            if (dbg2) dbgbuf.alloc((size_t)12 * grid);
            a.dbg = dbg2 ? dbgbuf.p : nullptr;
            a.dbg_mode = getenv("CMF_HALS_DBGMODE") ? atoi(getenv("CMF_HALS_DBGMODE")) : 0;
            void *args[] = {&a};
            prof_begin(PROF_SWEEP);
            CK(cudaLaunchCooperativeKernel((void *)hals2::hals2_sweep_kernel, dim3((unsigned)grid), dim3(hals2::NT), args, smem, stream));
            prof_end();
            post_launch();
            hals2::hals2_finish_kernel<<<dim3((unsigned)cdiv(Tt, 32), (unsigned)cdiv(K, 32)), tb, 0, stream>>>(h2_Hcm.p, Hp, K, Tt, Tp);
            post_launch();
            if (dbg2) {
                std::vector<long long> hv((size_t)12 * grid);
                CK(cudaMemcpyAsync(hv.data(), dbgbuf.p, hv.size() * sizeof(long long), cudaMemcpyDeviceToHost, stream));
                CK(cudaStreamSynchronize(stream));
                fprintf(stderr, "hals2: SM clock over the launch %lld MHz (clock64 / globaltimer, CTA 0)\n", hv[7]);
                const char *names[3] = {"block items", "diagonal items", "recurrence warps"};
                const int lo[4] = {0, n_block, n_block + n_diag, grid};
                for (int r = 0; r < 3; ++r) {
                    double worst = 0.0, mean = 0.0; int cnt = 0, wi = -1;
                    double phw[5] = {0, 0, 0, 0, 0};
                    long long mx = 0, slow = 0, rds = 0;
                    for (int i = lo[r]; i < lo[r + 1]; ++i) {
                        if (hv[12 * i + 1] == 0) continue;
                        const double v = (double)hv[12 * i] / (double)hv[12 * i + 1] / 1e3;
                        if (v > worst) { worst = v; wi = i - lo[r]; for (int q = 0; q < 5; ++q) phw[q] = (double)hv[12 * i + 2 + q] / (double)hv[12 * i + 1] / 1e3; }
                        mean += v; ++cnt;
                        mx = std::max(mx, hv[12 * i + 8]); slow += hv[12 * i + 9]; rds += hv[12 * i + 1];
                    }
                    fprintf(stderr, "hals2 %s: slowest single round %.1f kcycles, %.2f%% of the (CTA, round) pairs above 90 kcycles\n", names[r], mx / 1e3, rds ? 100.0 * slow / rds : 0.0);
                    fprintf(stderr, "hals2 %s: %d CTAs, kcycles of work per active round: mean %.1f, worst %.1f (item %d; phases stage %.1f pull %.1f tail/store %.1f final %.1f, barrier wait %.1f); rounds %lld, chunks %lld\n",
                            names[r], lo[r + 1] - lo[r], cnt ? mean / cnt : 0.0, worst, wi, phw[0], phw[1], phw[2], phw[3], phw[4], (long long)(nC + 4 * (K - 1) + 3), (long long)nC);
                }
            }
            return true;
        }
// ... 225 lines not shown
    }
}

struct DevGuard {
    int prev = -1;
    explicit DevGuard(int dev) {
        if (cudaGetDevice(&prev) != cudaSuccess) prev = -1;
        CK(cudaSetDevice(dev));
    }
    ~DevGuard() { if (prev >= 0) cudaSetDevice(prev); }
    DevGuard(const DevGuard &) = delete;
    DevGuard &operator=(const DevGuard &) = delete;
};
struct DevRestore {
    int prev = -1;
    DevRestore() { if (cudaGetDevice(&prev) != cudaSuccess) { prev = -1; cudaGetLastError(); } }
    ~DevRestore() { if (prev >= 0) cudaSetDevice(prev); }
};

bool converged(const double *loss_hist, int64_t n, int patience, double tol) {
    if (n <= patience) return false;
    for (int64_t i = n - patience; i < n; ++i)
        if (!(std::fabs(loss_hist[i] - loss_hist[i - 1]) < tol)) return false;
    return true;
}

#define NK(call)                                                                                   \
    do {                                                                                           \
        ncclResult_t r__ = (call);                                                                 \
        if (r__ != ncclSuccess)                                                                    \
            throw CmfError(CMF_ERR_NCCL, std::string(#call) + ": " + NcclApi::get().GetErrorString(r__)); \
    } while (0)

NcclApi &nccl() {
    NcclApi &a = NcclApi::get();
    if (!a.ok()) throw CmfError(CMF_ERR_NCCL, "NCCL is not available: " + a.why);
    return a;
}

void shard_range(int64_t T, int world, int rank, int64_t *t0, int64_t *t1) {
    const int64_t base = T / world, rem = T % world;
    *t0 = rank * base + std::min<int64_t>(rank, rem);
    *t1 = *t0 + base + (rank < rem ? 1 : 0);
}

template <typename S>
ncclDataType_t nccl_dt(const Ctx<S> &) { return std::is_same<S, double>::value ? ncclFloat64 : ncclFloat32; }
template <typename S>
constexpr size_t elem_size(const Ctx<S> &) { return sizeof(S); }

template <typename S>
void c_allreduce(Ctx<S> &ctx, void *buf, size_t count, ncclDataType_t dt, ncclRedOp_t op = ncclSum) {
    if (ctx.world() == 1) return;
    NK(nccl().AllReduce(buf, buf, count, dt, op, ctx.comm.comm, ctx.stream));
}

template <typename S>
void c_allreduce_host(Ctx<S> &ctx, double *vals, int n, ncclRedOp_t op = ncclSum) {
    if (ctx.world() == 1) return;
    REQUIRE(n <= 4, "at most 4 scalars");
    double *d = ctx.scalars() + 4;
    CK(cudaMemcpyAsync(d, vals, n * sizeof(double), cudaMemcpyHostToDevice, ctx.stream));
    c_allreduce(ctx, d, (size_t)n, ncclFloat64, op);
    CK(cudaMemcpyAsync(vals, d, n * sizeof(double), cudaMemcpyDeviceToHost, ctx.stream));
    CK(cudaStreamSynchronize(ctx.stream));
}

template <typename S>
void c_halo_exchange(Ctx<S> &ctx) {
    if (ctx.world() == 1 || ctx.L <= 1) return;
    void *sl, *sr, *rl, *rr;
    int64_t cnt;
    ctx.halo_buffers(&sl, &sr, &rl, &rr, &cnt);
    NcclApi &a = nccl();
    const ncclDataType_t dt = nccl_dt(ctx);
    const int r = ctx.rank(), w = ctx.world();
    NK(a.GroupStart());
    if (r + 1 < w) {
        NK(a.Send(sr, (size_t)cnt, dt, r + 1, ctx.comm.comm, ctx.stream));
        NK(a.Recv(rr, (size_t)cnt, dt, r + 1, ctx.comm.comm, ctx.stream));
    }
    if (r > 0) {
        NK(a.Send(sl, (size_t)cnt, dt, r - 1, ctx.comm.comm, ctx.stream));
        NK(a.Recv(rl, (size_t)cnt, dt, r - 1, ctx.comm.comm, ctx.stream));
    }
    NK(a.GroupEnd());
}

template <typename S>
void r_data_norm(Ctx<S> &ctx) {
    double ss = ctx.data_sumsq_local;
    c_allreduce_host(ctx, &ss, 1);
    ctx.data_sumsq_global = ss;
    ctx.data_norm = std::sqrt(ss);
    ctx.pgd_cur_loss = ctx.data_norm;
}

template <typename S>
void r_init_scale_partials(Ctx<S> &ctx, double out[2]) {
    ctx.init_scale_partials(out);
    c_allreduce_host(ctx, out, 2);
}

template <typename S>
double r_loss_sumsq(Ctx<S> &ctx, bool force_direct = false, bool *expansion_used = nullptr) {
    const int saved = ctx.loss_mode;
    if (force_direct) ctx.loss_mode = 0;
    int n;
    try { n = ctx.loss_partial_dev(); } catch (...) { ctx.loss_mode = saved; throw; }
    ctx.loss_mode = saved;
    double *d = ctx.scalars();
    c_allreduce(ctx, d, 2, ncclFloat64);
    double v[2];
    CK(cudaMemcpyAsync(v, d, 2 * sizeof(double), cudaMemcpyDeviceToHost, ctx.stream));
    CK(cudaStreamSynchronize(ctx.stream));
    if (expansion_used) *expansion_used = (n == 2);
    ++(n == 2 ? ctx.n_loss_expansion : ctx.n_loss_direct);
    return n == 2 ? ctx.data_sumsq_global - 2.0 * v[0] + v[1] : v[0];
}

template <typename S>
double r_guarded_loss(Ctx<S> &ctx) {
    if (ctx.loss_mode != 1) return std::sqrt(std::max(r_loss_sumsq(ctx), 0.0)) / ctx.data_norm;
    bool exp_used = false;
    const double se = r_loss_sumsq(ctx, false, &exp_used);
    if (!exp_used) return std::sqrt(std::max(se, 0.0)) / ctx.data_norm;
    const double g2 = ctx.loss_guard * ctx.loss_guard * ctx.data_sumsq_global;
    if (!ctx.calib_have && se > g2) return std::sqrt(se) / ctx.data_norm;
    if (ctx.calib_have && ctx.calib_left > 0 && se - ctx.calib_bias > 0.0) {
        --ctx.calib_left;
        return std::sqrt(se - ctx.calib_bias) / ctx.data_norm;
    }
    const double sd = r_loss_sumsq(ctx, true);
    if (ctx.calib_have && sd > 0.0) {
        const double err = std::fabs((se - ctx.calib_bias) - sd) / (2.0 * sd);
        ctx.calib_last_err = err;
        if (err > 1e-4) { ctx.calib_interval = 1; ++ctx.calib_fail; }
        else {
            ctx.calib_fail = 0;
            if (err > 2e-5) ctx.calib_interval = std::max(1, ctx.calib_interval / 2);
            else if (err < 5e-6) ctx.calib_interval = std::min(ctx.calib_max_interval, ctx.calib_interval * 2);
        }
        if (ctx.calib_fail >= 3) { ctx.loss_mode = 0; ctx.calib_reset(); }
    }
    ctx.calib_bias = se - sd;
    ctx.calib_have = true;
    ctx.calib_left = ctx.calib_interval - 1;
    return std::sqrt(std::max(sd, 0.0)) / ctx.data_norm;
}

template <typename S>
void r_update_motifs(Ctx<S> &ctx, double l1W, double l2W) {
    if (ctx.alg == CMF_PGD) { ctx.pgd_update_motifs(l1W, l2W); return; }
    ctx.w_partials();
    const int64_t KL = ctx.K * ctx.L;
    if (ctx.world() > 1 && ctx.alg == CMF_MULT && KL % ctx.world() == 0 && !getenv("CMF_W_REPLICATED")) {
        NcclApi &a = nccl();
        void *p; int64_t cnt; int dt;
        ctx.exchange_buffer(1, &p, &cnt, &dt);
        c_allreduce(ctx, p, (size_t)cnt, ncclFloat64);
        void *nw, *w; int64_t row;
        ctx.w_rows_buffers(&nw, &w, &row);
        const int64_t rows = KL / ctx.world(), j0 = rows * ctx.rank(), chunk = rows * row;
        const size_t es = elem_size(ctx);
        CK(cudaEventRecord(ctx.ev_a, ctx.stream));
        CK(cudaStreamWaitEvent(ctx.comm_stream, ctx.ev_a, 0));
        NK(a.ReduceScatter(nw, (char *)nw + (size_t)(j0 * row) * es, (size_t)chunk, nccl_dt(ctx), ncclSum, ctx.comm.comm, ctx.comm_stream));
        CK(cudaEventRecord(ctx.ev_b, ctx.comm_stream));
        ctx.w_denom_rows(j0, j0 + rows);
        CK(cudaStreamWaitEvent(ctx.stream, ctx.ev_b, 0));
        ctx.w_update_rows(l1W, l2W, j0, j0 + rows);
        CK(cudaEventRecord(ctx.ev_a, ctx.stream));
        CK(cudaStreamWaitEvent(ctx.comm_stream, ctx.ev_a, 0));
        NK(a.AllGather((char *)w + (size_t)(j0 * row) * es, w, (size_t)chunk, nccl_dt(ctx), ctx.comm.comm, ctx.comm_stream));
        CK(cudaEventRecord(ctx.ev_b, ctx.comm_stream));
        if (ctx.alg == CMF_MULT) ctx.fd_denomH_prefetch();
        CK(cudaStreamWaitEvent(ctx.stream, ctx.ev_b, 0));
        return;
    }
    if (ctx.world() > 1) {
        void *p; int64_t cnt; int dt;
        ctx.exchange_buffer(0, &p, &cnt, &dt);
        c_allreduce(ctx, p, (size_t)cnt, dt == CMF_F64 ? ncclFloat64 : ncclFloat32);
        ctx.exchange_buffer(1, &p, &cnt, &dt);
        c_allreduce(ctx, p, (size_t)cnt, ncclFloat64);
    }
    ctx.w_apply(l1W, l2W);
}

template <typename S>
void r_hals_sweep_sharded(Ctx<S> &ctx, double l1H, double l2H) {
    NcclApi &a = nccl();
    const ncclDataType_t dt = nccl_dt(ctx);
    const size_t es = elem_size(ctx);
    const int w = ctx.world(), r = ctx.rank();
    void *ql, *hl, *qf = nullptr, *hf = nullptr;
    int64_t cnt;
    ctx.hals_h_local(&ql, &hl, &cnt);
    if (r == 0) ctx.hals_h_full(&qf, &hf);
    for (int pass = 0; pass < 2; ++pass) {
        if (pass == 1 && r == 0) ctx.hals_h_sweep(1, l1H, l2H);
        NK(a.GroupStart());
        if (r == 0) {
            for (int p = 1; p < w; ++p) {
                int64_t a0, a1;
                shard_range(ctx.T, w, p, &a0, &a1);
                const size_t off = (size_t)(a0 * ctx.K) * es, c = (size_t)((a1 - a0) * ctx.K);
                if (pass == 0) {
                    NK(a.Recv((char *)qf + off, c, dt, p, ctx.comm.comm, ctx.stream));
                    NK(a.Recv((char *)hf + off, c, dt, p, ctx.comm.comm, ctx.stream));
                } else {
                    NK(a.Send((char *)hf + off, c, dt, p, ctx.comm.comm, ctx.stream));
                }
            }
        } else if (pass == 0) {
            NK(a.Send(ql, (size_t)cnt, dt, 0, ctx.comm.comm, ctx.stream));
            NK(a.Send(hl, (size_t)cnt, dt, 0, ctx.comm.comm, ctx.stream));
        } else {
            NK(a.Recv(hl, (size_t)cnt, dt, 0, ctx.comm.comm, ctx.stream));
        }
        NK(a.GroupEnd());
        if (r == 0) {
            if (pass == 0) {
                CK(cudaMemcpyAsync(qf, ql, (size_t)cnt * es, cudaMemcpyDeviceToDevice, ctx.stream));
                CK(cudaMemcpyAsync(hf, hl, (size_t)cnt * es, cudaMemcpyDeviceToDevice, ctx.stream));
            } else {
                CK(cudaMemcpyAsync(hl, hf, (size_t)cnt * es, cudaMemcpyDeviceToDevice, ctx.stream));
            }
        }
    }
}

template <typename S>
double r_update_feature_maps(Ctx<S> &ctx, double l1H, double l2H) {
    if (ctx.alg == CMF_PGD) {
        const double loss = std::sqrt(ctx.pgd_update_feature_maps(l1H, l2H)) / ctx.data_norm;
        if (ctx.loss_mode == 1 && !(loss > 0.25)) ctx.loss_mode = 0;
        return loss;
    }
    if (ctx.alg == CMF_HALS) {
        ctx.hals_h_prepare();
        if (ctx.world() == 1) ctx.hals_h_sweep(0, l1H, l2H);
        else r_hals_sweep_sharded(ctx, l1H, l2H);
        ctx.h_changed();
    } else {
        ctx.h_update(l1H, l2H);
    }
    c_halo_exchange(ctx);
    return r_guarded_loss(ctx);
}

template <typename S>
void r_fit(Ctx<S> &ctx, int64_t max_itr, double max_time, int eval_mode, int check_convergence, int patience, double tol,
           double l1W, double l2W, double l1H, double l2H, std::vector<double> &loss_hist, std::vector<double> &time_hist,
           int64_t cap, int *converged_early) {
    *converged_early = 0;
    loss_hist.clear(); time_hist.clear();
    loss_hist.push_back(r_guarded_loss(ctx));
    time_hist.push_back(0.0);
    int64_t itr = 1;
    const bool timed = max_time < 1e300;
    while ((max_itr < 0 || itr <= max_itr) && time_hist.back() <= max_time) {
        ++itr;
        REQUIRE((int64_t)loss_hist.size() < cap, "history capacity exhausted");
        auto t_start = std::chrono::steady_clock::now();
        if (!eval_mode) r_update_motifs(ctx, l1W, l2W);
        const double loss = r_update_feature_maps(ctx, l1H, l2H);
        double dur = std::chrono::duration<double>(std::chrono::steady_clock::now() - t_start).count();
        if (timed && ctx.world() > 1) {
            if (ctx.rank() != 0) dur = 0.0;
            c_allreduce_host(ctx, &dur, 1);
        }
        time_hist.push_back(time_hist.back() + dur);
        loss_hist.push_back(loss);
        if (check_convergence && converged(loss_hist.data(), (int64_t)loss_hist.size(), patience, tol)) {
            *converged_early = 1;
            break;
        }
    }
}

template <typename S>
void r_set_engine(Ctx<S> &ctx, int engine) {
    REQUIRE(engine >= 0 && engine <= 2, "engine must be 0 (SIMT), 1 (tcgen05, time domain) or 2 (tcgen05, frequency domain)");
    if (ctx.R > 0 && engine != 0) throw CmfError(CMF_ERR_UNSUPPORTED, "batch handles run the SIMT engine (0) only");
    if (engine == 2 && !ctx.fd_available())
        throw CmfError(CMF_ERR_UNSUPPORTED, "the frequency-domain engine needs an fp32 handle with K <= 128, L <= 256, N % 8 == 0 on sm_100 and room for the spectrum of X");
    if (engine < 2) ctx.fd_release();
    if (engine >= 1 && !ctx.tc_available())
        throw CmfError(CMF_ERR_UNSUPPORTED, "tcgen05 engine needs an fp32 MultUpdate handle with K <= 128 and N % 8 == 0 on sm_100");
    ctx.engine = engine;
    if (!ctx.loss_mode_explicit) ctx.loss_mode = (engine == 2) ? 1 : 0;
}

template <typename S>
void r_agree_engine(Ctx<S> &ctx) {
    if (ctx.world() == 1) return;
    double e = (double)ctx.engine;
    c_allreduce_host(ctx, &e, 1, ncclMin);
    if ((int)e != ctx.engine) r_set_engine(ctx, (int)e);
}

template <typename S>
void attach_comm(Ctx<S> &ctx, ncclComm_t comm, int rank, int world) {
    int64_t a0, a1;
    shard_range(ctx.T, world, rank, &a0, &a1);
    REQUIRE(a0 == ctx.t0 && a1 == ctx.t1, "the handle's column range is not the balanced shard of this rank (use cmf_shard_range)");
    ctx.comm.comm = comm; ctx.comm.rank = rank; ctx.comm.world = world;
    if (world > 1 && !ctx.comm_stream) {
        CK(cudaStreamCreateWithFlags(&ctx.comm_stream, cudaStreamNonBlocking));
        CK(cudaEventCreateWithFlags(&ctx.ev_a, cudaEventDisableTiming));
        CK(cudaEventCreateWithFlags(&ctx.ev_b, cudaEventDisableTiming));
    }
    r_agree_engine(ctx);
}

template <typename S>
void b_fit(Ctx<S> &ctx, int64_t max_itr, double max_time, int eval_mode, int check_convergence, int patience, double tol,
           const double *l1W, const double *l2W, const double *l1H, const double *l2H, double *loss_hist,
           std::vector<double> &time_hist, int64_t cap, int64_t *n_hist, int *converged_early) {
    const int64_t R = ctx.R;
    std::vector<double> reg((size_t)(4 * R));
    for (int64_t r = 0; r < R; ++r) { reg[4 * r] = l1W[r]; reg[4 * r + 1] = l2W[r]; reg[4 * r + 2] = l1H[r]; reg[4 * r + 3] = l2H[r]; }
    std::vector<int> active((size_t)R, 1);
    ctx.batch_set_state(reg.data(), active.data());
    std::vector<double> loss((size_t)R);
    ctx.batch_loss(loss.data());
    for (int64_t r = 0; r < R; ++r) { loss_hist[r * cap] = loss[r]; n_hist[r] = 1; converged_early[r] = 0; }
    time_hist.assign(1, 0.0);
    int64_t itr = 1, n_active = R;
    while (n_active > 0 && (max_itr < 0 || itr <= max_itr) && time_hist.back() <= max_time) {
        ++itr;
        REQUIRE((int64_t)time_hist.size() < cap, "history capacity exhausted");
        auto t_start = std::chrono::steady_clock::now();
        if (!eval_mode) ctx.batch_update_motifs();
        ctx.batch_update_feature_maps();
        ctx.batch_loss(loss.data());
        time_hist.push_back(time_hist.back() + std::chrono::duration<double>(std::chrono::steady_clock::now() - t_start).count());
        bool stopped = false;
        for (int64_t r = 0; r < R; ++r) {
            if (!active[r]) continue;
            double *lh = loss_hist + r * cap;
            lh[n_hist[r]++] = loss[r];
            if (check_convergence && converged(lh, n_hist[r], patience, tol)) {
                converged_early[r] = 1;
                active[r] = 0;
                --n_active;
                stopped = true;
            }
        }
        if (stopped && n_active > 0) ctx.batch_set_state(nullptr, active.data());
    }
}

template <typename S>
using Ranks = std::vector<std::unique_ptr<Ctx<S>>>;

}

struct cmf_ctx {
    std::variant<Ranks<float>, Ranks<double>> ranks;
    std::vector<ncclComm_t> comms;
    std::unique_ptr<cmf::Workers> workers;
    size_t size() const { return std::visit([](auto &v) { return v.size(); }, ranks); }
    ~cmf_ctx() {
        if (!workers) return;
        try {
            std::visit([&](auto &v) {
                workers->run_all([&](int i) {
                    auto &r = v[(size_t)i];
                    if (!r) return;
                    cudaSetDevice(r->device);
                    r.reset();
                    if (comms[(size_t)i]) NcclApi::get().CommDestroy(comms[(size_t)i]);
                });
            }, ranks);
        } catch (...) {}
    }
};

namespace {

template <typename S>
cmf_ctx *handle_of(std::unique_ptr<Ctx<S>> r) {
    Ranks<S> v;
    v.push_back(std::move(r));
    return new cmf_ctx{std::move(v)};
}

RankState &first(cmf_handle h) { return std::visit([](auto &v) -> RankState & { return *v.front(); }, h->ranks); }
RankState &last(cmf_handle h) { return std::visit([](auto &v) -> RankState & { return *v.back(); }, h->ranks); }

template <typename F>
void on_ranks(cmf_handle h, F &&f) {
    REQUIRE(h != nullptr, "null handle");
    std::visit([&](auto &v) {
        if (v.size() == 1) {
            DevGuard g(v[0]->device);
            f(*v[0]);
// ... 143 lines not shown
            Ranks<S> &ranks = std::get<Ranks<S>>(mc->ranks);
            try {
                mc->comms.assign((size_t)ngpu, nullptr);
                mc->workers.reset(new Workers(ngpu));
                NK(nccl().CommInitAll(mc->comms.data(), ngpu, devs.data()));
                cudaSetDevice(prev);
                mc->workers->run_all([&](int i) {
                    DevGuard g(devs[(size_t)i]);
                    int64_t a0, a1;
                    shard_range(T, ngpu, i, &a0, &a1);
                    ranks[(size_t)i] = make_ctx<S>(N, T, a0, a1, K, L, dtype, alg, devs[(size_t)i]);
                });
                mc->workers->run_all([&](int i) {
                    Ctx<S> &r = *ranks[(size_t)i];
                    DevGuard g(r.device);
                    attach_comm(r, mc->comms[(size_t)i], i, ngpu);
                });
            } catch (...) {
                cudaSetDevice(prev);
                delete mc;
                throw;
            }
            *out = mc;
        });
    });
}

int cmf_comm_info(cmf_handle h, int *rank_out, int *world_out, int64_t *t_begin, int64_t *t_end) {
    return guarded([&] {
        REQUIRE(h, "null handle");
        if (rank_out) *rank_out = first(h).rank();
        if (world_out) *world_out = first(h).world();
        if (t_begin) *t_begin = first(h).t0;
        if (t_end) *t_end = last(h).t1;
    });
}

int cmf_destroy(cmf_handle h) {
    return guarded([&] {
        if (!h) return;
        if (h->workers) { delete h; return; }
        DevGuard g(first(h).device);
        delete h;
    });
}

int cmf_set_data(cmf_handle h, const void *X, int64_t first_col) {
    return guarded([&] { on_ranks(h, [&](auto &r) { r.set_data(X, first_col); r_data_norm(r); }); });
}
int cmf_synth_data(cmf_handle h, uint64_t seed, int64_t K_true, int64_t L_true, double p_h, double noise) {
    return guarded([&] { on_ranks(h, [&](auto &r) { r.synth_data(seed, K_true, L_true, p_h, noise); r_data_norm(r); }); });
}
int cmf_data_sumsq(cmf_handle h, double *out) {
    return guarded([&] {
        REQUIRE(out, "null output");
        const RankState &r = first(h);
        REQUIRE(r.have_data, "no data");
        *out = r.world() > 1 ? r.data_sumsq_global : r.data_sumsq_local;
    });
}
int cmf_set_data_norm(cmf_handle h, double norm) {
    return guarded([&] { on_ranks(h, [&](auto &r) { r.data_norm = norm; r.data_sumsq_global = norm * norm; }); });
}
int cmf_set_factors(cmf_handle h, const void *W, const void *H, int64_t first_col) {
    return guarded([&] { single_set(h, "cmf_set_factors_batch"); on_ranks(h, [&](auto &r) { r.set_factors(W, H, first_col); }); });
}
int cmf_exchange_halos(cmf_handle h) {
    return guarded([&] { no_batch_split(h); on_ranks(h, [&](auto &r) { c_halo_exchange(r); r.h_changed(); }); });
}
int cmf_init_rand(cmf_handle h, uint64_t seed) {
    return guarded([&] { single_set(h, "cmf_set_factors_batch with drawn factors"); on_ranks(h, [&](auto &r) { r.init_rand(seed); }); });
}
int cmf_init_scale_partials(cmf_handle h, double out[2]) {
    return guarded([&] { single_set(h, "cmf_init_scale_partials_batch");
        REQUIRE(out, "null output");
        on_ranks(h, [&](auto &r) {
            double v[2];
            r_init_scale_partials(r, v);
            if (&r == &first(h)) { out[0] = v[0]; out[1] = v[1]; }
        });
    });
}
int cmf_scale_factors(cmf_handle h, double s) {
    return guarded([&] { single_set(h, "cmf_scale_factors_batch"); on_ranks(h, [&](auto &r) { r.scale_factors(s); }); });
}
int cmf_get_factors(cmf_handle h, void *W_out, void *H_out) {
    return guarded([&] { single_set(h, "cmf_get_factors_batch");
        on_ranks(h, [&](auto &r) {
            REQUIRE(r.have_factors, "no factors");
            void *Hp = H_out ? (char *)H_out + (size_t)((r.t0 - first(h).t0) * r.K) * elem_size(r) : nullptr;
            r.get_factors(&r == &first(h) ? W_out : nullptr, Hp);
        });
    });
}

int cmf_update_motifs(cmf_handle h, double l1W, double l2W) {
    return guarded([&] { single_set(h, "cmf_fit_batch"); on_ranks(h, [&](auto &r) { r_update_motifs(r, l1W, l2W); }); });
}

int cmf_update_feature_maps(cmf_handle h, double l1H, double l2H, double *loss_out) {
    return guarded([&] { single_set(h, "cmf_fit_batch");
        on_ranks(h, [&](auto &r) {
            const double loss = r_update_feature_maps(r, l1H, l2H);
            if (loss_out && &r == &first(h)) *loss_out = loss;
        });
    });
}

int cmf_loss(cmf_handle h, double *loss_out) {
    return guarded([&] { single_set(h, "cmf_loss_batch");
        REQUIRE(loss_out, "null output");
        on_ranks(h, [&](auto &r) {
            REQUIRE(r.world() > 1 || (r.is_first && r.is_last), "shards without a communicator use cmf_loss_partial");
            const double loss = r_guarded_loss(r);
            if (&r == &first(h)) *loss_out = loss;
        });
    });
}

int cmf_fit(cmf_handle h, int64_t max_itr, double max_time, int eval_mode, int check_convergence, int patience,
            double tol, double l1W, double l2W, double l1H, double l2H, double *loss_hist, double *time_hist,
            int64_t cap, int64_t *n_hist, int *converged_early) {
    return guarded([&] { single_set(h, "cmf_fit_batch");
        REQUIRE(loss_hist && time_hist && n_hist, "null history pointers");
        REQUIRE(patience >= 1, "patience must be >= 1 (src/algs/alternating.jl:30)");
        REQUIRE(cap >= 1, "history capacity must be >= 1");
        if (converged_early) *converged_early = 0;
        on_ranks(h, [&](auto &r) {
            REQUIRE(r.world() > 1 || (r.is_first && r.is_last), "shards without a communicator use the split-phase calls");
            std::vector<double> lh, th;
            int early = 0;
            r_fit(r, max_itr, max_time, eval_mode, check_convergence, patience, tol, l1W, l2W, l1H, l2H, lh, th, cap, &early);
            if (&r == &first(h)) {
                std::copy(lh.begin(), lh.end(), loss_hist);
                std::copy(th.begin(), th.end(), time_hist);
                *n_hist = (int64_t)lh.size();
                if (converged_early) *converged_early = early;
            }
        });
    });
}

int cmf_w_partials(cmf_handle h) {
    return guarded([&] { no_batch_split(h); single_rank(h); on_ranks(h, [&](auto &r) { r.w_partials(); }); });
}
int cmf_w_apply(cmf_handle h, double l1W, double l2W) {
    return guarded([&] { no_batch_split(h); single_rank(h); on_ranks(h, [&](auto &r) { r.w_apply(l1W, l2W); }); });
}
int cmf_h_update(cmf_handle h, double l1H, double l2H) {
    return guarded([&] { no_batch_split(h);
        single_rank(h);
        on_ranks(h, [&](auto &r) {
            REQUIRE(r.alg == CMF_MULT, "the split-phase H update is MultUpdate only");
            r.h_update(l1H, l2H);
        });
    });
}
int cmf_loss_partial(cmf_handle h, double *sumsq_out) {
    return guarded([&] { no_batch_split(h); single_rank(h); REQUIRE(sumsq_out, "null output"); on_ranks(h, [&](auto &r) { *sumsq_out = r.loss_partial(); }); });
}
int cmf_exchange_buffer(cmf_handle h, int which, void **dev_ptr, int64_t *count, int *dtype) {
    return guarded([&] { no_batch_split(h); single_rank(h); REQUIRE(dev_ptr && count && dtype, "null output"); on_first(h, [&](auto &r) { r.exchange_buffer(which, dev_ptr, count, dtype); }); });
}
int cmf_halo_buffers(cmf_handle h, void **sl, void **sr, void **rl, void **rr, int64_t *count) {
    return guarded([&] { no_batch_split(h); single_rank(h); REQUIRE(sl && sr && rl && rr && count, "null output"); on_first(h, [&](auto &r) { r.halo_buffers(sl, sr, rl, rr, count); }); });
}
int cmf_sync(cmf_handle h) {
    return guarded([&] { on_ranks(h, [&](auto &r) { CK(cudaStreamSynchronize(r.stream)); }); });
}
int cmf_launch_count(cmf_handle h, int64_t *out) {
    return guarded([&] {
        REQUIRE(h && out, "null argument");
        *out = std::visit([](auto &v) { int64_t n = 0; for (auto &r : v) n += r->launches; return n; }, h->ranks);
    });
}
int cmf_stream(cmf_handle h, void **stream_out) {
    return guarded([&] { REQUIRE(h && stream_out, "null argument"); *stream_out = (void *)first(h).stream; });
}
int cmf_get_data(cmf_handle h, void *X_out, int with_halo) {
    return guarded([&] {
        REQUIRE(X_out, "null output");
        on_ranks(h, [&](auto &r) {
            REQUIRE(r.have_data, "no data");
            r.get_data((char *)X_out + (size_t)((r.t0 - first(h).t0) * r.N) * elem_size(r), h->size() > 1 ? 0 : with_halo);
        });
    });
}
int cmf_profile(cmf_handle h, int enable) {
    return guarded([&] {
        on_ranks(h, [&](auto &r) {
            CK(cudaStreamSynchronize(r.stream));
            r.prof_clear();
            r.profiling = enable != 0;
        });
    });
}
int cmf_profile_read(cmf_handle h, int which, double *ms_total, int64_t *count) {
    return guarded([&] {
        REQUIRE(h && ms_total && count, "null output");
        REQUIRE(which >= 0 && which < PROF_NCLASS, "which must be 0 (conv), 1 (transconv), 2 (corr) or 3 (HALS H sweep)");
        RankState &r = first(h);
        DevGuard g(r.device);
        CK(cudaStreamSynchronize(r.stream));
        double tot = 0.0;
        int64_t n = 0;
        for (auto &e : r.prof_events) {
            if (e.which != which) continue;
            float ms = 0.f;
            CK(cudaEventElapsedTime(&ms, e.a, e.b));
            tot += ms;
            ++n;
        }
        *ms_total = tot;
        *count = n;
    });
}
int cmf_set_stream(cmf_handle h, void *stream) {
    return guarded([&] {
        single_rank(h);
        RankState &r = first(h);
        DevGuard g(r.device);
        CK(cudaStreamSynchronize(r.stream));
        if (r.own_stream && r.stream) cudaStreamDestroy(r.stream);
        r.own_stream = false;
        r.stream = (cudaStream_t)stream;
    });
}
int cmf_set_engine(cmf_handle h, int engine) {
    return guarded([&] { on_ranks(h, [&](auto &r) { r_set_engine(r, engine); }); });
}

int cmf_set_loss_mode(cmf_handle h, int mode) {
    return guarded([&] {
        REQUIRE(mode == 0 || mode == 1, "loss mode must be 0 (direct) or 1 (expansion)");
        if (h && first(h).R > 0 && mode != 0) throw CmfError(CMF_ERR_UNSUPPORTED, "batch handles evaluate the loss by the direct pass (mode 0) only");
        on_ranks(h, [&](auto &r) { r.loss_mode = mode; r.loss_mode_explicit = true; r.calib_reset(); });
    });
}
int cmf_set_loss_guard(cmf_handle h, double guard, int max_interval) {
    return guarded([&] {
        REQUIRE(guard >= 0.0, "loss guard must be >= 0");
        REQUIRE(max_interval >= 1 && max_interval <= 1024, "calibration interval must be in [1, 1024]");
        on_ranks(h, [&](auto &r) { r.loss_guard = guard; r.calib_max_interval = max_interval; r.calib_reset(); });
    });
}
int cmf_get_loss_stats(cmf_handle h, int64_t *n_direct, int64_t *n_expansion, int *interval, double *last_err) {
    return guarded([&] {
        REQUIRE(h, "null handle");
        const RankState &r = first(h);
        if (n_direct) *n_direct = r.n_loss_direct;
        if (n_expansion) *n_expansion = r.n_loss_expansion;
        if (interval) *interval = r.calib_have ? r.calib_interval : 0;
        if (last_err) *last_err = r.calib_last_err;
    });
}
int cmf_get_loss_mode(cmf_handle h, int *mode_out) {
    return guarded([&] { REQUIRE(h && mode_out, "null argument"); *mode_out = first(h).loss_mode; });
}
int cmf_get_fd_layout(cmf_handle h, int *block_len, int *hop, int64_t *nblocks) {
    return guarded([&] {
        REQUIRE(h && block_len && hop && nblocks, "null argument");
        on_first(h, [&](auto &r) { r.fd_layout(block_len, hop, nblocks); });
    });
}
int cmf_get_engine(cmf_handle h, int *engine_out) {
    return guarded([&] { REQUIRE(h && engine_out, "null argument"); *engine_out = first(h).engine; });
}

static int current_device() {
    int d = 0;
    if (cudaGetDevice(&d) != cudaSuccess) d = 0;
    return d;
}

int cmf_set_pgd_constraints(cmf_handle h, int constrW, int constrH) {
    return guarded([&] { single_rank(h); on_first(h, [&](auto &r) { r.set_pgd_constraints(constrW, constrH); }); });
}
int cmf_set_pgd_loss(cmf_handle h, int loss_func, const void *mask) {
    return guarded([&] { single_rank(h); on_ranks(h, [&](auto &r) { r.set_pgd_loss(loss_func, mask); }); });
}

int cmf_tensor_conv(int64_t N, int64_t T, int64_t K, int64_t L, int dtype, const void *W, const void *H, void *out) {
    return guarded([&] {
        REQUIRE(W && H && out, "null pointer");
        with_dtype(dtype, [&](auto s) {
            auto c = make_ctx<decltype(s)>(N, T, 0, T, K, L, dtype, CMF_MULT, current_device());
            c->set_factors(W, H, 0);
            c->prim_conv(out);
        });
    });
}
int cmf_tensor_transconv(int64_t N, int64_t T, int64_t K, int64_t L, int dtype, const void *W, const void *X, void *out) {
    return guarded([&] {
        REQUIRE(W && X && out, "null pointer");
        with_dtype(dtype, [&](auto s) {
            auto c = make_ctx<decltype(s)>(N, T, 0, T, K, L, dtype, CMF_MULT, current_device());
            std::vector<decltype(s)> Hz((size_t)(K * T), 0);
            c->set_factors(W, Hz.data(), 0);
            c->prim_transconv(X, out);
        });
    });
}
int cmf_corr_w(int64_t N, int64_t T, int64_t K, int64_t L, int dtype, const void *H, const void *X, void *out) {
    return guarded([&] {
        REQUIRE(H && X && out, "null pointer");
        with_dtype(dtype, [&](auto s) {
            auto c = make_ctx<decltype(s)>(N, T, 0, T, K, L, dtype, CMF_MULT, current_device());
            std::vector<decltype(s)> Wz((size_t)(K * N * L), 0);
            c->set_factors(Wz.data(), H, 0);
            c->prim_corr(X, out);
        });
    });
}
int cmf_compute_resids(int64_t N, int64_t T, int64_t K, int64_t L, int dtype, const void *X, const void *W, const void *H, void *out) {
    return guarded([&] {
        REQUIRE(X && W && H && out, "null pointer");
        with_dtype(dtype, [&](auto s) {
            auto c = make_ctx<decltype(s)>(N, T, 0, T, K, L, dtype, CMF_MULT, current_device());
            c->set_data(X, 0);
            c->set_factors(W, H, 0);
            c->prim_resids(out);
        });
    });
}
int cmf_shift_and_stack(int64_t K, int64_t T, int64_t L, int dtype, const void *H, void *out) {
    return guarded([&] {
        REQUIRE(H && out, "null pointer");
        with_dtype(dtype, [&](auto s) {
            auto c = make_ctx<decltype(s)>(8, T, 0, T, K, L, dtype, CMF_MULT, current_device());
            std::vector<decltype(s)> Wz((size_t)(K * 8 * L), 0);
            c->set_factors(Wz.data(), H, 0);
            c->prim_shift_and_stack(out);
        });
    });
}

int cmf_create_batch(cmf_handle *out, int64_t N, int64_t T, int64_t K, int64_t L, int dtype, int alg, int64_t R, int device) {
    return guarded([&] {
        REQUIRE(out != nullptr, "null output pointer");
        REQUIRE(R >= 1 && R <= 32768, "R (restarts) must be in 1..32768");
        DevRestore g;
        *out = make_batch(N, T, std::vector<int64_t>((size_t)R, K), L, dtype, alg, device);
    });
}
int cmf_create_batch_ranks(cmf_handle *out, int64_t N, int64_t T, const int64_t *K, int64_t L, int dtype, int alg, int64_t R,
                           int device) {
    return guarded([&] {
        REQUIRE(out != nullptr, "null output pointer");
        REQUIRE(K != nullptr, "null rank array K");
        REQUIRE(R >= 1 && R <= 32768, "R (restarts) must be in 1..32768");
        DevRestore g;
        *out = make_batch(N, T, std::vector<int64_t>(K, K + R), L, dtype, alg, device);
    });
}
int cmf_set_factors_batch(cmf_handle h, const void *W, const void *H) {
    return guarded([&] { batch_handle(h); on_ranks(h, [&](auto &r) { r.batch_set_factors(W, H); }); });
}
int cmf_get_factors_batch(cmf_handle h, void *W_out, void *H_out) {
    return guarded([&] { batch_handle(h); on_ranks(h, [&](auto &r) { r.batch_get_factors(W_out, H_out); }); });
}
int cmf_init_scale_partials_batch(cmf_handle h, double *out) {
    return guarded([&] { REQUIRE(out, "null output"); batch_handle(h); on_ranks(h, [&](auto &r) { r.batch_scale_partials(out); }); });
}
int cmf_scale_factors_batch(cmf_handle h, const double *s) {
    return guarded([&] { REQUIRE(s, "null scale factors"); batch_handle(h); on_ranks(h, [&](auto &r) { r.batch_scale(s); }); });
}
int cmf_loss_batch(cmf_handle h, double *loss_out) {
    return guarded([&] { REQUIRE(loss_out, "null output"); batch_handle(h); on_ranks(h, [&](auto &r) { r.batch_loss(loss_out); }); });
}
int cmf_fit_batch(cmf_handle h, int64_t max_itr, double max_time, int eval_mode, int check_convergence, int patience, double tol,
                  const double *l1W, const double *l2W, const double *l1H, const double *l2H, double *loss_hist, double *time_hist,
                  int64_t cap, int64_t *n_hist, int *converged_early) {
    return guarded([&] {
        batch_handle(h);
        REQUIRE(l1W && l2W && l1H && l2H, "null regulariser arrays");
        REQUIRE(loss_hist && time_hist && n_hist && converged_early, "null history pointers");
        REQUIRE(patience >= 1, "patience must be >= 1 (src/algs/alternating.jl:30)");
        REQUIRE(cap >= 1, "history capacity must be >= 1");
        on_ranks(h, [&](auto &r) {
            std::vector<double> th;
            b_fit(r, max_itr, max_time, eval_mode, check_convergence, patience, tol, l1W, l2W, l1H, l2H, loss_hist, th, cap, n_hist,
                  converged_early);
            std::copy(th.begin(), th.end(), time_hist);
        });
    });
}

}
```

### cmf.jl_b200/csrc/kernels_fd.cuh

```cuda
#pragma once
#include <cuda_bf16.h>
#include <cuda_runtime.h>
#include <stdint.h>

namespace cmf {
namespace fd {

#ifndef CMF_FD_MINB
#define CMF_FD_MINB 3
#endif
constexpr int LD_U = 8;
constexpr int NT = 512;
constexpr int KQ_MAX = 128;

__device__ __forceinline__ float2 add2(float2 a, float2 b) { return __fadd2_rn(a, b); }
__device__ __forceinline__ float2 sub2(float2 a, float2 b) { return __fadd2_rn(a, make_float2(-b.x, -b.y)); }
__device__ __forceinline__ float2 mul2(float2 a, float2 b) { return __fmul2_rn(a, b); }
__device__ __forceinline__ float2 fma2(float2 a, float2 b, float2 c) { return __ffma2_rn(a, b, c); }
__device__ __forceinline__ float2 bcast(float x) { return make_float2(x, x); }

__global__ void twiddle_kernel(float2 *__restrict__ tw, int B) {
    const int m = blockIdx.x * blockDim.x + threadIdx.x;
    if (m < B) {
        float s, c;
        sincospif(-2.0f * (float)m / (float)B, &s, &c);
        tw[m] = make_float2(c, s);
    }
}
template <int B>
__device__ __forceinline__ void load_twiddles(float2 *tw, const float2 *__restrict__ twg) {
#pragma unroll
    for (int m = threadIdx.x; m < B; m += NT) tw[m] = twg[m];
}

__device__ __forceinline__ void grid_block_tile(int64_t nbx, int ny, int &blk, int &tile) {
    const unsigned dv = nbx ? (unsigned)nbx : (unsigned)ny, q = blockIdx.x / dv, r = blockIdx.x - q * dv;
    blk = (int)(nbx ? r : q);
    tile = (int)(nbx ? q : r);
}

template <int LOGB> __device__ __forceinline__ int rev(int x) { return (int)(__brev((unsigned)x) >> (32 - LOGB)); }

template <bool INV> __device__ __forceinline__ float2 twmul(float2 a, float2 w) {
    const float2 t = mul2(make_float2(a.y, a.x), INV ? make_float2(w.y, -w.y) : make_float2(-w.y, w.y));
    return fma2(a, bcast(w.x), t);
}
template <bool INV> __device__ __forceinline__ float2 mul_mi(float2 a) { return INV ? make_float2(-a.y, a.x) : make_float2(a.y, -a.x); }
template <bool INV> __device__ __forceinline__ float2 w8_sum(float2 a) {
    return INV ? add2(make_float2(a.x, a.x), make_float2(-a.y, a.y)) : add2(a, make_float2(a.y, -a.x));
}
template <bool INV> __device__ __forceinline__ float2 w83_sum(float2 a) {
    return INV ? add2(make_float2(-a.x, a.x), make_float2(-a.y, -a.y)) : add2(make_float2(a.y, -a.x), make_float2(-a.x, -a.y));
}

template <bool INV, int LOGB, int C>
__device__ __forceinline__ void fft_passes(float2 *d, const float2 *tw) {
    constexpr int B = 1 << LOGB, JSTEP = NT / C;
    const float2 rr = bcast(0.70710678118654752f);
    const int c = threadIdx.x % C, j0 = threadIdx.x / C;
#pragma unroll
    for (int s = 0; s + 2 < LOGB; s += 3) {
        const int lq = LOGB - s - 3, q = 1 << lq, qC = q * C;
#pragma unroll 1
        for (int jj = 0; jj < (B / 8 + JSTEP - 1) / JSTEP; ++jj) {
            const int j = j0 + jj * JSTEP;
            if ((B / 8) % JSTEP != 0 && j >= B / 8) break;
            const int pos = j & (q - 1), g = j >> lq;
            float2 *r = d + ((g << (lq + 3)) + pos) * C + c;
            float2 a0 = r[0], a1 = r[qC], a2 = r[2 * qC], a3 = r[3 * qC], a4 = r[4 * qC], a5 = r[5 * qC], a6 = r[6 * qC], a7 = r[7 * qC];
            float2 t, u5, v7;
            t = sub2(a0, a4); a0 = add2(a0, a4); a4 = t;
            t = sub2(a1, a5); a1 = add2(a1, a5); u5 = w8_sum<INV>(t);
            t = sub2(a2, a6); a2 = add2(a2, a6); a6 = mul_mi<INV>(t);
            t = sub2(a3, a7); a3 = add2(a3, a7); v7 = mul2(w83_sum<INV>(t), rr);
            t = sub2(a0, a2); a0 = add2(a0, a2); a2 = t;
            t = sub2(a1, a3); a1 = add2(a1, a3); a3 = mul_mi<INV>(t);
            t = sub2(a4, a6); a4 = add2(a4, a6); a6 = t;
            t = fma2(u5, rr, make_float2(-v7.x, -v7.y)); a5 = fma2(u5, rr, v7); a7 = mul_mi<INV>(t);
            t = sub2(a0, a1); a0 = add2(a0, a1); a1 = t;
            t = sub2(a2, a3); a2 = add2(a2, a3); a3 = t;
            t = sub2(a4, a5); a4 = add2(a4, a5); a5 = t;
            t = sub2(a6, a7); a6 = add2(a6, a7); a7 = t;
            if (lq > 0) {
                const int e = pos << s;
                a1 = twmul<INV>(a1, tw[4 * e]); a2 = twmul<INV>(a2, tw[2 * e]); a3 = twmul<INV>(a3, tw[6 * e]);
                a4 = twmul<INV>(a4, tw[e]);     a5 = twmul<INV>(a5, tw[5 * e]); a6 = twmul<INV>(a6, tw[3 * e]);
                a7 = twmul<INV>(a7, tw[7 * e]);
            }
            r[0] = a0; r[qC] = a1; r[2 * qC] = a2; r[3 * qC] = a3; r[4 * qC] = a4; r[5 * qC] = a5; r[6 * qC] = a6; r[7 * qC] = a7;
        }
        __syncthreads();
    }
    if constexpr (LOGB % 3 == 2) {
#pragma unroll
        for (int jj = 0; jj < (B / 4 + JSTEP - 1) / JSTEP; ++jj) {
            const int j = j0 + jj * JSTEP;
            if ((B / 4) % JSTEP != 0 && j >= B / 4) break;
            float2 *r = d + (4 * j) * C + c;
            float2 a0 = r[0], a1 = r[C], a2 = r[2 * C], a3 = r[3 * C], t;
            t = sub2(a0, a2); a0 = add2(a0, a2); a2 = t;
            t = sub2(a1, a3); a1 = add2(a1, a3); a3 = mul_mi<INV>(t);
            r[0] = add2(a0, a1); r[C] = sub2(a0, a1); r[2 * C] = add2(a2, a3); r[3 * C] = sub2(a2, a3);
        }
        __syncthreads();
    } else if constexpr (LOGB % 3 == 1) {
#pragma unroll
        for (int jj = 0; jj < (B / 2 + JSTEP - 1) / JSTEP; ++jj) {
            const int j = j0 + jj * JSTEP;
            if ((B / 2) % JSTEP != 0 && j >= B / 2) break;
            float2 *r0 = d + (2 * j) * C + c, *r1 = r0 + C;
            const float2 a = *r0, b = *r1;
            *r0 = add2(a, b);
            *r1 = sub2(a, b);
        }
        __syncthreads();
    }
}

template <int LOGB, int C>
__device__ __forceinline__ void unpack_pair(const float2 *d, int f, int p, float2 &re, float2 &im) {
    constexpr int B = 1 << LOGB;
    const float2 z = d[rev<LOGB>(f) * C + p], y = d[rev<LOGB>((B - f) & (B - 1)) * C + p];
    const float2 sm = add2(z, y), df = sub2(z, y);
    re = mul2(sm, bcast(0.5f));
    im = mul2(make_float2(df.y, df.x), make_float2(0.5f, -0.5f));
}

template <int LOGB, int C>
__device__ __forceinline__ void pack_pair(float2 *d, int f, int p, float2 re, float2 im) {
    constexpr int B = 1 << LOGB;
    if (f == 0 || f == B / 2) im = make_float2(0.f, 0.f);
    const float2 v = make_float2(im.y, im.x);
    const float2 sm = add2(re, v), df = sub2(re, v);
    d[f * C + p] = make_float2(df.x, sm.y);
    if (f > 0 && f < B / 2) d[(B - f) * C + p] = make_float2(sm.x, df.y);
}

__device__ __forceinline__ void split2(float2 ab, uint32_t &h, uint32_t &l) {
    const __nv_bfloat162 hh = __floats2bfloat162_rn(ab.x, ab.y);
    const float2 lf = sub2(ab, __bfloat1622float2(hh));
    const __nv_bfloat162 ll = __floats2bfloat162_rn(lf.x, lf.y);
    h = *reinterpret_cast<const uint32_t *>(&hh);
    l = *reinterpret_cast<const uint32_t *>(&ll);
}
__device__ __forceinline__ void store_split2(__nv_bfloat16 *hi, __nv_bfloat16 *lo, int64_t idx, float2 ab) {
    uint32_t h, l;
    split2(ab, h, l);
    *reinterpret_cast<uint32_t *>(hi + idx) = h;
    *reinterpret_cast<uint32_t *>(lo + idx) = l;
}

template <int LOGB>
__global__ void __launch_bounds__(NT, CMF_FD_MINB)
fft_x_kernel(const float *__restrict__ X, __nv_bfloat16 *__restrict__ hi, __nv_bfloat16 *__restrict__ lo, int64_t N, int64_t xcols,
             int V, int64_t nblkp, int64_t nbx, const float2 *__restrict__ twg) {
    constexpr int B = 1 << LOGB, C = 16, ISTEP = NT / C;
    extern __shared__ float2 fd_smem[];
    float2 *d = fd_smem, *tw = fd_smem + B * C;
    int b, tile;
    grid_block_tile(nbx, (int)((N + 31) / 32), b, tile);
    const int p = threadIdx.x % C;
    const int n = tile * 32 + 2 * p;
    load_twiddles<B>(tw, twg);
    {
        const int i0 = threadIdx.x / C;
        const int64_t lim64 = xcols - (int64_t)b * V;
        const int lim = (n < N) ? (int)(lim64 < 0 ? 0 : (lim64 > B ? B : lim64)) : 0;
        const float *src = X + ((int64_t)b * V + i0) * N + n;
        float2 *dst = d + i0 * C + p;
#pragma unroll 1
        for (int i = i0; i < B; i += LD_U * ISTEP, src += (int64_t)LD_U * ISTEP * N, dst += LD_U * ISTEP * C) {
            float2 v[LD_U];
#pragma unroll
            for (int u = 0; u < LD_U; ++u) {
                v[u] = make_float2(0.f, 0.f);
                if (i + u * ISTEP < lim) v[u] = *reinterpret_cast<const float2 *>(src + (int64_t)u * ISTEP * N);
            }
#pragma unroll
            for (int u = 0; u < LD_U; ++u)
                if (B % (LD_U * ISTEP) == 0 || i + u * ISTEP < B) dst[u * ISTEP * C] = v[u];
        }
    }
    __syncthreads();
    fft_passes<false, LOGB, C>(d, tw);
    if (n >= N) return;
    for (int f = threadIdx.x / C; f <= B / 2; f += NT / C) {
        float2 re, im;
        unpack_pair<LOGB, C>(d, f, p, re, im);
        const int64_t r = ((int64_t)f * nblkp + b) * 2;
        store_split2(hi, lo, r * N + n, re);
        store_split2(hi, lo, (r + 1) * N + n, im);
    }
}

template <int LOGB, int C>
__global__ void __launch_bounds__(NT, CMF_FD_MINB)
fft_h_kernel(const float *__restrict__ H, __nv_bfloat16 *__restrict__ hi, __nv_bfloat16 *__restrict__ lo, int64_t K, int64_t Tl,
             int64_t hcols, int V, int64_t nblkp, int full, int64_t t_off, int kq, int64_t nbx,
             const float2 *__restrict__ twg) {
    constexpr int B = 1 << LOGB, ISTEP = NT / C;
    const int64_t KQ = kq, MROWS = 2 * kq;
    extern __shared__ float2 fd_smem[];
    float2 *d = fd_smem, *tw = fd_smem + B * C;
    int bi, tile;
    grid_block_tile(nbx, (kq / 2) / C, bi, tile);
    const int64_t b = bi;
    const int p = threadIdx.x % C;
    const int k = 2 * (tile * C + p);
    load_twiddles<B>(tw, twg);
    {
        const int i0 = threadIdx.x / C;
        const int64_t tb = b * V + t_off;
        const int64_t lim64 = full ? (hcols - tb) : ((Tl - tb < V) ? Tl - tb : V);
        const int lim = (int)(lim64 < 0 ? 0 : (lim64 > B ? B : lim64));
        const float *src = H + (tb + i0) * K + k;
        float2 *dst = d + i0 * C + p;
        const bool pair = ((K & 1) == 0) && (k + 1 < K);
#pragma unroll 1
        for (int i = i0; i < B; i += LD_U * ISTEP, src += (int64_t)LD_U * ISTEP * K, dst += LD_U * ISTEP * C) {
            float2 v[LD_U];
#pragma unroll
            for (int u = 0; u < LD_U; ++u) {
                v[u] = make_float2(0.f, 0.f);
                if (i + u * ISTEP < lim) {
                    const float *q = src + (int64_t)u * ISTEP * K;
                    if (pair) v[u] = *reinterpret_cast<const float2 *>(q);
                    else { if (k < K) v[u].x = q[0]; if (k + 1 < K) v[u].y = q[1]; }
                }
            }
#pragma unroll
            for (int u = 0; u < LD_U; ++u)
                if (B % (LD_U * ISTEP) == 0 || i + u * ISTEP < B) dst[u * ISTEP * C] = v[u];
        }
    }
    __syncthreads();
    fft_passes<false, LOGB, C>(d, tw);
    const int64_t rs = full ? 2 * KQ : 2 * MROWS;
    const int64_t rstep = (int64_t)(NT / C) * nblkp * rs;
    int64_t r = ((int64_t)(threadIdx.x / C) * nblkp + b) * rs + k;
    for (int f = threadIdx.x / C; f <= B / 2; f += NT / C, r += rstep) {
        float2 re, im;
        unpack_pair<LOGB, C>(d, f, p, re, im);
        uint32_t hr, lr, hi_, li_;
        split2(re, hr, lr);
        split2(im, hi_, li_);
        if (full) {
            *reinterpret_cast<uint32_t *>(hi + r) = hr; *reinterpret_cast<uint32_t *>(lo + r) = lr;
            *reinterpret_cast<uint32_t *>(hi + r + KQ) = hi_; *reinterpret_cast<uint32_t *>(lo + r + KQ) = li_;
            continue;
        }
        const uint32_t sg = 0x80008000u;
        *reinterpret_cast<uint32_t *>(hi + r) = hr; *reinterpret_cast<uint32_t *>(lo + r) = lr;
        *reinterpret_cast<uint32_t *>(hi + r + KQ) = hi_ ^ sg; *reinterpret_cast<uint32_t *>(lo + r + KQ) = li_ ^ sg;
        *reinterpret_cast<uint32_t *>(hi + r + MROWS) = hi_; *reinterpret_cast<uint32_t *>(lo + r + MROWS) = li_;
        *reinterpret_cast<uint32_t *>(hi + r + MROWS + KQ) = hr; *reinterpret_cast<uint32_t *>(lo + r + MROWS + KQ) = lr;
    }
}

template <int LOGB, int C>
__global__ void __launch_bounds__(NT, CMF_FD_MINB)
fft_w_kernel(const float *__restrict__ Wi, __nv_bfloat16 *__restrict__ hi, __nv_bfloat16 *__restrict__ lo, int64_t N, int64_t K,
             int64_t L, int64_t ldw, int64_t coff, int xmode, int kq, const float2 *__restrict__ twg) {
    constexpr int B = 1 << LOGB, ISTEP = NT / C;
    const int64_t KQ = kq, MROWS = 2 * kq;
    extern __shared__ float2 fd_smem[];
    float2 *d = fd_smem, *tw = fd_smem + B * C;
    const int64_t k = blockIdx.y;
    const int p = threadIdx.x % C;
    const int64_t n = (int64_t)blockIdx.x * (2 * C) + 2 * p;
    load_twiddles<B>(tw, twg);
    {
        const int i0 = threadIdx.x / C;
        const float *src = Wi + ((int64_t)i0 * K + k) * N + n;
        float2 *dst = d + i0 * C + p;
#pragma unroll 1
        for (int i = i0; i < B; i += LD_U * ISTEP, src += (int64_t)LD_U * ISTEP * K * N, dst += LD_U * ISTEP * C) {
            float2 v[LD_U];
#pragma unroll
            for (int u = 0; u < LD_U; ++u) {
                const int ii = i + u * ISTEP;
                v[u] = make_float2(0.f, 0.f);
                if (ii < L && n < N) {
                    const float *q = src + (int64_t)u * ISTEP * K * N;
                    if ((N & 1) == 0) v[u] = *reinterpret_cast<const float2 *>(q);
                    else { v[u].x = q[0]; if (n + 1 < N) v[u].y = q[1]; }
                }
            }
#pragma unroll
            for (int u = 0; u < LD_U; ++u)
                if (B % (LD_U * ISTEP) == 0 || i + u * ISTEP < B) dst[u * ISTEP * C] = v[u];
        }
    }
    __syncthreads();
    fft_passes<false, LOGB, C>(d, tw);
    if (n >= N) return;
    for (int f = threadIdx.x / C; f <= B / 2; f += NT / C) {
        float2 re, im;
        unpack_pair<LOGB, C>(d, f, p, re, im);
        const float2 nim = make_float2(-im.x, -im.y);
        if (xmode) {
            const int64_t r0 = (((int64_t)f * 2 + 0) * MROWS + k) * N + n, r1 = r0 + MROWS * N;
            store_split2(hi, lo, r0, re);
            store_split2(hi, lo, r0 + KQ * N, nim);
            store_split2(hi, lo, r1, im);
            store_split2(hi, lo, r1 + KQ * N, re);
            continue;
        }
        const int64_t rw = ((int64_t)f * MROWS + k) * ldw + n, iw = rw + KQ * ldw;
        store_split2(hi, lo, rw, re);
        store_split2(hi, lo, rw + coff, im);
        store_split2(hi, lo, iw, nim);
        store_split2(hi, lo, iw + coff, re);
    }
}

template <int LOGB, int C>
__global__ void __launch_bounds__(NT, CMF_FD_MINB)
ifft_numH_kernel(const float *__restrict__ Of, float *__restrict__ numH, int64_t K, int64_t Tl, int V, int64_t nblkp, int kq,
                 int64_t nbx, const float2 *__restrict__ twg) {
    constexpr int B = 1 << LOGB, FSTEP = NT / C;
    const int64_t KQ = kq, MROWS = 2 * kq;
    extern __shared__ float2 fd_smem[];
    float2 *d = fd_smem, *tw = fd_smem + B * C;
    int bi, tile;
    grid_block_tile(nbx, (kq / 2) / C, bi, tile);
    const int64_t b = bi;
    const int p = threadIdx.x % C;
    const int k = 2 * (tile * C + p);
    load_twiddles<B>(tw, twg);
    {
        const int f0 = threadIdx.x / C;
        const int64_t ustep = (int64_t)FSTEP * nblkp * MROWS;
        const float *o = Of + ((int64_t)f0 * nblkp + b) * MROWS + k;
#pragma unroll 1
        for (int f = f0; f <= B / 2; f += 4 * FSTEP, o += 4 * ustep) {
            float2 re[4], im[4];
#pragma unroll
            for (int u = 0; u < 4; ++u)
                if (f + u * FSTEP <= B / 2) {
                    const float *q = o + u * ustep;
                    re[u] = *reinterpret_cast<const float2 *>(q); im[u] = *reinterpret_cast<const float2 *>(q + KQ);
                }
#pragma unroll
            for (int u = 0; u < 4; ++u)
                if (f + u * FSTEP <= B / 2) pack_pair<LOGB, C>(d, f + u * FSTEP, p, re[u], im[u]);
        }
    }
    __syncthreads();
    fft_passes<true, LOGB, C>(d, tw);
    const float2 sc = bcast(1.0f / (float)B);
    const bool pair = ((K & 1) == 0) && (k + 1 < K);
    for (int i = threadIdx.x / C; i < V; i += NT / C) {
        const int64_t t = b * V + i;
        if (t >= Tl) break;
        const float2 z = mul2(d[rev<LOGB>(i) * C + p], sc);
        if (pair) *reinterpret_cast<float2 *>(numH + t * K + k) = z;
        else { if (k < K) numH[t * K + k] = z.x; if (k + 1 < K) numH[t * K + k + 1] = z.y; }
    }
}

template <int LOGB>
__global__ void __launch_bounds__(NT, CMF_FD_MINB)
ifft_resid_kernel(const float *__restrict__ Yf, const float *__restrict__ X, double *__restrict__ partial, int64_t N, int64_t Tl,
                  int64_t L, int V, int64_t nbc, int64_t b0, int64_t nbx, const float2 *__restrict__ twg) {
    constexpr int B = 1 << LOGB, C = 16, FSTEP = NT / C, ISTEP = NT / C;
    extern __shared__ float2 fd_smem[];
    __shared__ double red[NT / 32];
    float2 *d = fd_smem, *tw = fd_smem + B * C;
    const int ny = (int)((N + 31) / 32);
    int bc, by;
    grid_block_tile(nbx, ny, bc, by);
    const int p = threadIdx.x % C;
    const int n = by * 32 + 2 * p;
    load_twiddles<B>(tw, twg);
    {
        const int f0 = threadIdx.x / C;
        const int64_t ustep = (int64_t)FSTEP * nbc * 2 * N;
        const float *y = Yf + (((int64_t)f0 * nbc + bc) * 2) * N + n;
#pragma unroll 1
        for (int f = f0; f <= B / 2; f += 4 * FSTEP, y += 4 * ustep) {
            float2 re[4], im[4];
#pragma unroll
            for (int u = 0; u < 4; ++u) {
                re[u] = make_float2(0.f, 0.f); im[u] = re[u];
                if (f + u * FSTEP <= B / 2 && n < N) {
                    const float *q = y + u * ustep;
                    re[u] = *reinterpret_cast<const float2 *>(q); im[u] = *reinterpret_cast<const float2 *>(q + N);
                }
            }
#pragma unroll
            for (int u = 0; u < 4; ++u)
                if (f + u * FSTEP <= B / 2) pack_pair<LOGB, C>(d, f + u * FSTEP, p, re[u], im[u]);
        }
    }
    __syncthreads();
    fft_passes<true, LOGB, C>(d, tw);
    const float2 sc = bcast(1.0f / (float)B);
    double accd = 0.0;
    if (n < N) {
        const int64_t tb = (b0 + bc) * (int64_t)V - (L - 1);
        const int lim = (int)(Tl - tb < B ? Tl - tb : B);
        const int i0 = (int)(L - 1) + threadIdx.x / C;
        const float *xs = X + (tb + i0) * N + n;
#pragma unroll 1
        for (int i = i0; i < B; i += LD_U * ISTEP, xs += (int64_t)LD_U * ISTEP * N) {
            float2 x[LD_U];
#pragma unroll
            for (int u = 0; u < LD_U; ++u) {
                x[u] = make_float2(0.f, 0.f);
                if (i + u * ISTEP < lim) x[u] = *reinterpret_cast<const float2 *>(xs + (int64_t)u * ISTEP * N);
            }
            float acc = 0.f;
#pragma unroll
            for (int u = 0; u < LD_U; ++u) {
                const int ii = i + u * ISTEP;
                if (ii < lim) {
                    const float2 r = fma2(d[rev<LOGB>(ii) * C + p], sc, make_float2(-x[u].x, -x[u].y));
                    acc = fmaf(r.x, r.x, acc);
                    acc = fmaf(r.y, r.y, acc);
                }
            }
            accd += (double)acc;
        }
    }
#pragma unroll
    for (int o = 16; o > 0; o >>= 1) accd += __shfl_xor_sync(0xffffffffu, accd, o);
    if ((threadIdx.x & 31) == 0) red[threadIdx.x >> 5] = accd;
    __syncthreads();
    if (threadIdx.x == 0) {
        double s = 0.0;
        for (int w = 0; w < NT / 32; ++w) s += red[w];
        partial[(int64_t)bc * ny + by] = s;
    }
}

template <typename OutT, int LOGB, int C>
__global__ void __launch_bounds__(NT, CMF_FD_MINB)
ifft_numW_kernel(const float *__restrict__ Df, OutT *__restrict__ out, int64_t N, int64_t ldi, int64_t K, int64_t L, int kq,
                 const float2 *__restrict__ twg) {
    constexpr int B = 1 << LOGB, FSTEP = NT / C;
    const int64_t KQ = kq, MROWS = 2 * kq;
    extern __shared__ float2 fd_smem[];
    float2 *d = fd_smem, *tw = fd_smem + B * C;
    const int64_t k = blockIdx.y;
    const int p = threadIdx.x % C;
    const int64_t n = (int64_t)blockIdx.x * (2 * C) + 2 * p;
    load_twiddles<B>(tw, twg);
    {
        const int f0 = threadIdx.x / C;
        const int64_t ustep = (int64_t)FSTEP * MROWS * ldi;
        const float *src = Df + ((int64_t)f0 * MROWS + k) * ldi + n;
#pragma unroll 1
        for (int f = f0; f <= B / 2; f += 4 * FSTEP, src += 4 * ustep) {
            float2 re[4], im[4];
#pragma unroll
            for (int u = 0; u < 4; ++u) {
                re[u] = make_float2(0.f, 0.f); im[u] = re[u];
                if (f + u * FSTEP <= B / 2 && n < N) {
                    re[u] = *reinterpret_cast<const float2 *>(src + u * ustep);
                    im[u] = *reinterpret_cast<const float2 *>(src + u * ustep + KQ * ldi);
                }
            }
#pragma unroll
            for (int u = 0; u < 4; ++u)
                if (f + u * FSTEP <= B / 2) pack_pair<LOGB, C>(d, f + u * FSTEP, p, re[u], im[u]);
        }
    }
    __syncthreads();
    fft_passes<true, LOGB, C>(d, tw);
    if (n >= N) return;
    const float2 sc = bcast(1.0f / (float)B);
    for (int l = threadIdx.x / C; l < L; l += NT / C) {
        const float2 z = mul2(d[rev<LOGB>(l) * C + p], sc);
        OutT *o = out + ((int64_t)l * K + k) * N + n;
        if (sizeof(OutT) == 4) {
            *reinterpret_cast<float2 *>(o) = z;
        } else {
            o[0] = (OutT)z.x;
            if (n + 1 < N) o[1] = (OutT)z.y;
        }
    }
}

}
}
```

### cmf.jl_b200/csrc/kernels_simt.cuh

```cuda
#pragma once
#include <cuda_runtime.h>
#include <stdint.h>

namespace cmf {

#define CMF_EPS 2.220446049250313e-16

__device__ __forceinline__ double warp_sum(double v) {
#pragma unroll
    for (int o = 16; o > 0; o >>= 1) v += __shfl_xor_sync(0xffffffffu, v, o);
    return v;
}

__device__ __forceinline__ double block_sum(double v, double *red) {
    const int tid = threadIdx.y * blockDim.x + threadIdx.x;
    const int nthr = blockDim.x * blockDim.y;
    v = warp_sum(v);
    __syncthreads();
    if ((tid & 31) == 0) red[tid >> 5] = v;
    __syncthreads();
    double r = 0.0;
    if (tid < 32) {
        r = (tid < (nthr + 31) / 32) ? red[tid] : 0.0;
        r = warp_sum(r);
// ... 534 lines not shown
                                const double *__restrict__ Ht, int64_t K, int64_t L, double *__restrict__ partial) {
    __shared__ double red[32];
    const int64_t KL = K * L;
    double acc = 0.0;
    for (int64_t idx = (int64_t)blockIdx.x * blockDim.x + threadIdx.x; idx < KL * KL; idx += (int64_t)gridDim.x * blockDim.x) {
        const int64_t jp = idx % KL, j = idx / KL;
        const int64_t k = j % K, l = j / K, kp = jp % K, lp = jp / K;
        double g = (l >= lp) ? Rg[((l - lp) * K + k) * K + kp] : Rg[((lp - l) * K + kp) * K + k];
        const int64_t m = l < lp ? l : lp;
        for (int64_t i = 0; i < m; ++i) g -= Ht[(L - 1 - l + i) * K + k] * Ht[(L - 1 - lp + i) * K + kp];
        acc += g * (double)S2[(l * Ks + k) * ld + lp * Ks + kp];
    }
    acc = block_sum(acc, red);
    if (threadIdx.x == 0) partial[blockIdx.x] = acc;
}

template <typename S>
__global__ void s2_dot_G_diag_kernel(const S *__restrict__ S2, int64_t Ks, int64_t ld, const double *__restrict__ Rg,
                                     const double *__restrict__ Ht, int64_t K, int64_t L, double *__restrict__ partial) {
    __shared__ double red[32];
    double acc = 0.0;
    const int64_t total = (2 * L - 1) * K * K;
    for (int64_t e = (int64_t)blockIdx.x * blockDim.x + threadIdx.x; e < total; e += (int64_t)gridDim.x * blockDim.x) {
        const int64_t kp = e % K, k = (e / K) % K, d = e / (K * K) - (L - 1);
        const double r = (d >= 0) ? Rg[(d * K + k) * K + kp] : Rg[((-d) * K + kp) * K + k];
        const int64_t steps = L - (d >= 0 ? d : -d);
        int64_t l = d >= 0 ? d : 0, lp = d >= 0 ? 0 : -d;
        double tail = 0.0;
        for (int64_t s_ = 0; s_ < steps; ++s_, ++l, ++lp) {
            acc += (r - tail) * (double)S2[(l * Ks + k) * ld + lp * Ks + kp];
            if (s_ + 1 < steps) tail += Ht[(L - 2 - l) * K + k] * Ht[(L - 2 - lp) * K + kp];
        }
    }
    acc = block_sum(acc, red);
    if (threadIdx.x == 0) partial[blockIdx.x] = acc;
}

template <typename S>
__global__ void lag_table_kernel(const S *__restrict__ S2, S *__restrict__ Cf, int64_t K, int64_t L, int64_t Ks, int64_t ld,
                                 const BatchRest *tab = nullptr) {
    if (tab) {
        const BatchRest r = tab[blockIdx.y];
        K = Ks = r.K; ld = r.K * L; S2 += r.gs; Cf += r.cf;
    }
    const int64_t idx = (int64_t)blockIdx.x * blockDim.x + threadIdx.x;
    if (idx >= (2 * L - 1) * K * K) return;
    const int64_t kp = idx % K, k = (idx / K) % K, d = idx / (K * K) - (L - 1);
    double s = 0.0;
    for (int64_t l = (d > 0 ? d : 0); l < L && l - d < L; ++l) s += (double)S2[(l * Ks + k) * ld + (l - d) * Ks + kp];
    Cf[idx] = (S)s;
}

template <typename S>
__global__ void __launch_bounds__(256) denomH_tail_kernel(const S *__restrict__ S2, const S *__restrict__ H,
                                                           S *__restrict__ den, int64_t K, int64_t L,
                                                           int64_t Tl, int64_t h_lo, int64_t Ks, int64_t ld) {
    __shared__ double red[32];
    const int KL = (int)(K * L), Ki = (int)K;
    const int64_t c = blockIdx.x;
    const int64_t k = blockIdx.y;
    const int64_t t = Tl - (L - 1) + c;
    if (t < 0) return;
    const int w = (int)(Tl - t);
    double s = 0.0;
    for (int jp = threadIdx.x; jp < KL; jp += blockDim.x) {
        const int lp = jp / Ki, kp = jp - lp * Ki;
        const S *s2col = S2 + (int64_t)lp * Ks + kp;
        const S *hcol = H + kp;
        S acc = S(0);
        for (int l = 0; l < w; ++l) {
            const int64_t u = t + l - lp;
            if (u < h_lo) continue;
            acc = fma(s2col[((int64_t)l * Ks + k) * ld], hcol[u * K], acc);
        }
        s += (double)acc;
    }
    s = block_sum(s, red);
    if (threadIdx.x == 0) den[t * K + k] = (S)s;
}

template <typename S>
__global__ void __launch_bounds__(256) denomH_tail_prefix_kernel(const S *__restrict__ S2, const S *__restrict__ H,
                                                                  double *__restrict__ part, int64_t K, int64_t L, int64_t Tl,
                                                                  int64_t h_lo, int64_t Ks, int64_t ld, int64_t ldh,
                                                                  const BatchRest *tab = nullptr) {
    extern __shared__ double tail_sm[];
    const int64_t k = blockIdx.y;
    if (tab) {
        const BatchRest r = tab[blockIdx.z];
        K = Ks = r.K; ld = r.K * L;
        if (k >= K || (int64_t)blockIdx.x * blockDim.x >= (2 * L - 1) * K) return;
        S2 += r.gs; H += r.off; part += r.tp;
    }
    const int64_t e = (int64_t)blockIdx.x * blockDim.x + threadIdx.x;
    const bool live = e < (2 * L - 1) * K;
    const int64_t dq = live ? e / K : 0, kp = live ? e - dq * K : 0;
    const int64_t d = dq - (L - 1);
    const int warp = threadIdx.x >> 5, lane = threadIdx.x & 31;
    const int Lm = (int)(L - 1);
    S pre = S(0);
    S nxt[8];
#pragma unroll
    for (int q = 0; q < 8; ++q) {
        const int64_t l = q, lp = l - d;
        nxt[q] = (live && q < Lm && lp >= 0 && lp < L) ? S2[(l * Ks + k) * ld + lp * Ks + kp] : S(0);
    }
    for (int w0 = 1; w0 <= Lm; w0 += 8) {
        S cur[8];
#pragma unroll
        for (int q = 0; q < 8; ++q) cur[q] = nxt[q];
#pragma unroll
        for (int q = 0; q < 8; ++q) {
            const int64_t l = w0 - 1 + 8 + q, lp = l - d;
            nxt[q] = (live && l < Lm && lp >= 0 && lp < L) ? S2[(l * Ks + k) * ld + lp * Ks + kp] : S(0);
        }
#pragma unroll
    for (int q = 0; q < 8; ++q) {
        const int w = w0 + q;
        if (w > Lm) break;
        pre += cur[q];
        const int64_t u = Tl - w + d;
        double v = 0.0;
        if (live && pre != S(0) && u >= h_lo) v = (double)(pre * H[u * ldh + kp]);
#pragma unroll
        for (int o = 16; o > 0; o >>= 1) v += __shfl_xor_sync(0xffffffffu, v, o);
        if (lane == 0) tail_sm[warp * Lm + (w - 1)] = v;
    }
    }
    __syncthreads();
    for (int w = threadIdx.x + 1; w <= Lm; w += blockDim.x) {
        double s = 0.0;
        for (int q = 0; q < 8; ++q) s += tail_sm[q * Lm + (w - 1)];
        part[((int64_t)blockIdx.x * Lm + (Lm - w)) * K + k] = s;
    }
}

template <typename S>
__global__ void denomH_tail_reduce_kernel(const double *__restrict__ part, S *__restrict__ den, int64_t K, int64_t L, int64_t Tl,
                                          int nblocks, int64_t ldd, const BatchRest *tab = nullptr) {
    if (tab) {
        const BatchRest r = tab[blockIdx.y];
        K = r.K; nblocks = (int)(((2 * L - 1) * K + 255) / 256); part += r.tp; den += r.off;
    }
    const int64_t i = (int64_t)blockIdx.x * blockDim.x + threadIdx.x;
    if (i >= (L - 1) * K) return;
    const int64_t c = i / K, k = i - c * K, t = Tl - (L - 1) + c;
    if (t < 0) return;
    double s = 0.0;
    for (int b = 0; b < nblocks; ++b) s += part[(int64_t)b * (L - 1) * K + i];
    den[t * ldd + k] = (S)s;
}

template <typename S>
__global__ void mu_update_kernel(S *__restrict__ x, const S *__restrict__ num, const S *__restrict__ den,
                                 S l1, S l2, int64_t n, const double *__restrict__ reg = nullptr,
                                 const int *__restrict__ active = nullptr, int64_t inner = 1, const int *__restrict__ col_rest = nullptr,
                                 int64_t C = 1) {
    const int64_t i = (int64_t)blockIdx.x * blockDim.x + threadIdx.x;
    if (i >= n) return;
    if (reg) {
        const int64_t r = restart_of(i, inner, col_rest, C);
        if (!active[r]) return;
        l1 = (S)reg[4 * r];
        l2 = (S)reg[4 * r + 1];
    }
    const S eps = (S)CMF_EPS;
    S v = x[i];
    v = v * (num[i] / (den[i] + l1 + S(2) * l2 * v + eps));
    x[i] = v > eps ? v : eps;
}

__global__ void __launch_bounds__(256) mu_update_vec4_kernel(float4 *__restrict__ x, const float4 *__restrict__ num, const float4 *__restrict__ den,
                                                             float l1, float l2, int64_t n4, double *__restrict__ partial) {
    __shared__ double red[32];
    const float eps = (float)CMF_EPS;
    double acc = 0.0;
    for (int64_t i = (int64_t)blockIdx.x * blockDim.x + threadIdx.x; i < n4; i += (int64_t)gridDim.x * blockDim.x) {
        float4 v = x[i];
        const float4 a = __ldg(num + i), d = __ldg(den + i);
        v.x = v.x * (a.x / (d.x + l1 + 2.f * l2 * v.x + eps)); v.x = v.x > eps ? v.x : eps;
        v.y = v.y * (a.y / (d.y + l1 + 2.f * l2 * v.y + eps)); v.y = v.y > eps ? v.y : eps;
        v.z = v.z * (a.z / (d.z + l1 + 2.f * l2 * v.z + eps)); v.z = v.z > eps ? v.z : eps;
        v.w = v.w * (a.w / (d.w + l1 + 2.f * l2 * v.w + eps)); v.w = v.w > eps ? v.w : eps;
        x[i] = v;
        if (partial) acc += (double)a.x * (double)v.x + (double)a.y * (double)v.y + (double)a.z * (double)v.z + (double)a.w * (double)v.w;
    }
    if (partial) {
        acc = block_sum(acc, red);
        if (threadIdx.x == 0) partial[blockIdx.x] = acc;
    }
}

template <typename S>
__global__ void scale_kernel(S *__restrict__ x, S s, int64_t n, const double *__restrict__ s_r = nullptr, int64_t inner = 1,
                             const int *__restrict__ col_rest = nullptr, int64_t C = 1) {
    const int64_t i = (int64_t)blockIdx.x * blockDim.x + threadIdx.x;
    if (i >= n) return;
    if (s_r) s = (S)s_r[restart_of(i, inner, col_rest, C)];
    x[i] *= s;
}

template <typename S>
__global__ void dot_partial_kernel(const S *__restrict__ a, const S *__restrict__ b, int64_t n,
                                   double *__restrict__ partial) {
    __shared__ double red[32];
    double s = 0.0;
    for (int64_t i = (int64_t)blockIdx.x * blockDim.x + threadIdx.x; i < n; i += (int64_t)gridDim.x * blockDim.x)
        s += (double)a[i] * (double)b[i];
    s = block_sum(s, red);
    if (threadIdx.x == 0) partial[blockIdx.x] = s;
}

template <typename S>
__global__ void w_julia_to_internal(const S *__restrict__ Wj, S *__restrict__ Wi, int64_t K, int64_t N, int64_t L, int64_t ldk,
                                    const BatchRest *tab = nullptr) {
    if (tab) {
        const BatchRest r = tab[blockIdx.y];
        K = r.K; Wj += r.off * N * L; Wi += r.off * N;
    }
    const int64_t idx = (int64_t)blockIdx.x * blockDim.x + threadIdx.x;
    if (idx >= K * N * L) return;
    const int64_t n = idx % N, k = (idx / N) % K, l = idx / (N * K);
    Wi[(l * ldk + k) * N + n] = Wj[k + K * (n + N * l)];
}
template <typename S>
__global__ void w_internal_to_julia(const S *__restrict__ Wi, S *__restrict__ Wj, int64_t K, int64_t N, int64_t L, int64_t ldk,
                                    const BatchRest *tab = nullptr) {
    if (tab) {
        const BatchRest r = tab[blockIdx.y];
        K = r.K; Wj += r.off * N * L; Wi += r.off * N;
    }
    const int64_t idx = (int64_t)blockIdx.x * blockDim.x + threadIdx.x;
    if (idx >= K * N * L) return;
    const int64_t k = idx % K, n = (idx / K) % N, l = idx / (K * N);
    Wj[idx] = Wi[(l * ldk + k) * N + n];
}

template <typename S>
__global__ void h_stack_kernel(const S *__restrict__ src, S *__restrict__ dst, int64_t C, int64_t T, const BatchRest *__restrict__ tab,
                               const int *__restrict__ col_rest, int to_stacked) {
    const int64_t i = (int64_t)blockIdx.x * blockDim.x + threadIdx.x;
    if (i >= C * T) return;
    const int64_t c = i % C, t = i / C;
    const BatchRest r = tab[col_rest[c]];
    const int64_t b = T * r.off + t * r.K + (c - r.off);
    if (to_stacked) dst[i] = src[b];
    else dst[b] = src[i];
}

template <typename S>
__global__ void shift_stack_kernel(const S *__restrict__ H, S *__restrict__ out, int64_t K, int64_t L, int64_t T) {
    const int64_t e = (int64_t)blockIdx.x * blockDim.x + threadIdx.x;
    if (e >= K * L * T) return;
    const int64_t j = e % (K * L), t = e / (K * L), l = j / K, k = j % K;
    out[e] = (t >= l) ? H[(t - l) * K + k] : S(0);
}

template <typename S>
__global__ void h_tail_kernel(const S *__restrict__ H, double *__restrict__ tail, int64_t K, int64_t L,
                              int64_t Tl, int is_last, int64_t ldh, const BatchRest *tab = nullptr) {
    if (tab) {
        const BatchRest r = tab[blockIdx.y];
        K = r.K; H += r.off; tail += r.ex + L * K * K;
    }
    const int64_t idx = (int64_t)blockIdx.x * blockDim.x + threadIdx.x;
    if (idx >= (L - 1) * K) return;
    const int64_t c = idx / K, k = idx % K;
    tail[idx] = is_last ? (double)H[(Tl - (L - 1) + c) * ldh + k] : 0.0;
}

template <typename S>
__global__ void uniform_kernel(S *__restrict__ x, int64_t n, uint64_t seed, uint64_t stream, int64_t idx0) {
    const int64_t i = (int64_t)blockIdx.x * blockDim.x + threadIdx.x;
    if (i < n) x[i] = (S)u01(seed, stream, (uint64_t)(idx0 + i));
}

template <typename S>
__global__ void synth_H_kernel(S *__restrict__ H, int64_t K, int64_t t_first, int64_t cols, int64_t T,
                               uint64_t seed, double p_h) {
    const int64_t i = (int64_t)blockIdx.x * blockDim.x + threadIdx.x;
    if (i >= K * cols) return;
    const int64_t k = i % K, t = t_first + i / K;
    S v = S(0);
    if (t >= 0 && t < T) {
        const uint64_t id = (uint64_t)(t * K + k);
        if (u01(seed, 1, id) < p_h) v = (S)(-log(u01(seed, 2, id)));
    }
    H[i] = v;
}

__device__ inline double gamma_draw(double alpha, uint64_t seed, uint64_t stream, uint64_t id) {
    const double a = alpha + 1.0, d = a - 1.0 / 3.0, c = 1.0 / sqrt(9.0 * d);
    double g = d;
    for (uint64_t it = 0; it < 32; ++it) {
        const double x = gauss01(seed, stream, id * 64 + it);
        const double v0 = 1.0 + c * x;
        if (v0 <= 0.0) continue;
        const double v = v0 * v0 * v0, u = u01(seed, stream + 1, id * 64 + it);
        if (log(u) < 0.5 * x * x + d - d * v + d * log(v)) { g = d * v; break; }
    }
    return g * pow(u01(seed, stream + 2, id), 1.0 / alpha);
}

template <typename S>
__global__ void synth_W_kernel(S *__restrict__ Wi, int64_t K, int64_t N, int64_t L, uint64_t seed,
                               double alpha, double sigma) {
    const int64_t n = (int64_t)blockIdx.x * blockDim.x + threadIdx.x;
    if (n >= N) return;
    double tot = 0.0;
    for (int64_t k = 0; k < K; ++k) tot += gamma_draw(alpha, seed, 10, (uint64_t)(n * K + k));
    for (int64_t k = 0; k < K; ++k) {
        const double wgt = gamma_draw(alpha, seed, 10, (uint64_t)(n * K + k)) / tot;
        const double cent = 2.0 * u01(seed, 20, (uint64_t)(n * K + k)) - 1.0;
        for (int64_t l = 0; l < L; ++l) {
            const double x = (L > 1) ? (-1.0 + 2.0 * (double)l / (double)(L - 1)) : -1.0;
            const double z = (x - cent) / sigma;
            Wi[(l * K + k) * N + n] = (S)(wgt * exp(-0.5 * z * z) / (sigma * 2.5066282746310002));
        }
    }
}

template <typename S>
__global__ void __launch_bounds__(256) hals_w_sweep_kernel(const S *__restrict__ G, const S *__restrict__ P ,
                                                            S *__restrict__ Wi , int64_t K, int64_t L,
                                                            int64_t N, S l1, S l2) {
    extern __shared__ __align__(16) unsigned char smem_raw[];
    const int64_t KL = K * L;
    S *Ps = reinterpret_cast<S *>(smem_raw);
    __shared__ S delta_s;
    const int64_t n = blockIdx.x;
    for (int64_t j = threadIdx.x; j < KL; j += blockDim.x) Ps[j] = P[j * N + n];
    __syncthreads();
    for (int64_t k = 0; k < K; ++k)
        for (int64_t l = 0; l < L; ++l) {
            const int64_t j = l * K + k;
            if (threadIdx.x == 0) {
// ... 434 lines not shown
```

### include/cmf_sm100.h

```cpp
#ifndef CMF_SM100_H
#define CMF_SM100_H

#include <stdint.h>

#ifdef __cplusplus
extern "C" {
#endif

typedef struct cmf_ctx *cmf_handle;

enum { CMF_F64 = 0, CMF_F32 = 1 };
enum { CMF_MULT = 0, CMF_HALS = 1, CMF_PGD = 2 };
enum {
    CMF_OK = 0,
    CMF_ERR_ARG = 1,
    CMF_ERR_CUDA = 2,
    CMF_ERR_UNSUPPORTED = 3,
    CMF_ERR_NCCL = 4
};


int cmf_create(cmf_handle *out, int64_t N, int64_t T, int64_t K, int64_t L, int dtype, int alg,
               int device);

int cmf_create_shard(cmf_handle *out, int64_t N, int64_t T_global, int64_t t_begin, int64_t t_end,
                     int64_t K, int64_t L, int dtype, int alg, int device);

int cmf_create_multi(cmf_handle *out, int64_t N, int64_t T, int64_t K, int64_t L, int dtype, int alg,
                     int ngpu, const int *devices);

int cmf_comm_unique_id(void *id_out_128_bytes);
int cmf_create_rank(cmf_handle *out, int64_t N, int64_t T, int64_t K, int64_t L, int dtype, int alg,
                    int device, const void *unique_id_128_bytes, int rank, int world);
int cmf_shard_range(int64_t T, int world, int rank, int64_t *t_begin, int64_t *t_end);
int cmf_comm_info(cmf_handle h, int *rank_out, int *world_out, int64_t *t_begin, int64_t *t_end);
int cmf_exchange_halos(cmf_handle h);

int cmf_destroy(cmf_handle h);

const char *cmf_last_error(void);


int cmf_set_data(cmf_handle h, const void *X, int64_t first_col);

int cmf_synth_data(cmf_handle h, uint64_t seed, int64_t K_true, int64_t L_true, double p_h,
                   double noise);

int cmf_get_data(cmf_handle h, void *X_out, int with_halo);

int cmf_data_sumsq(cmf_handle h, double *out);
int cmf_set_data_norm(cmf_handle h, double norm);

int cmf_set_factors(cmf_handle h, const void *W, const void *H, int64_t first_col);

int cmf_init_rand(cmf_handle h, uint64_t seed);
int cmf_init_scale_partials(cmf_handle h, double out_dot_norm2[2]);
int cmf_scale_factors(cmf_handle h, double s);

int cmf_get_factors(cmf_handle h, void *W_out, void *H_out);


int cmf_update_motifs(cmf_handle h, double l1W, double l2W);
int cmf_update_feature_maps(cmf_handle h, double l1H, double l2H, double *loss_out);
int cmf_loss(cmf_handle h, double *loss_out);

int cmf_fit(cmf_handle h, int64_t max_itr, double max_time, int eval_mode, int check_convergence,
            int patience, double tol, double l1W, double l2W, double l1H, double l2H,
            double *loss_hist, double *time_hist, int64_t cap, int64_t *n_hist,
            int *converged_early);


int cmf_create_batch(cmf_handle *out, int64_t N, int64_t T, int64_t K, int64_t L, int dtype, int alg, int64_t R,
                     int device);
int cmf_create_batch_ranks(cmf_handle *out, int64_t N, int64_t T, const int64_t *K , int64_t L, int dtype,
                           int alg, int64_t R, int device);
int cmf_set_factors_batch(cmf_handle h, const void *W, const void *H);
int cmf_get_factors_batch(cmf_handle h, void *W_out, void *H_out);
int cmf_init_scale_partials_batch(cmf_handle h, double *out );
int cmf_scale_factors_batch(cmf_handle h, const double *s );
int cmf_loss_batch(cmf_handle h, double *loss_out );
int cmf_fit_batch(cmf_handle h, int64_t max_itr, double max_time, int eval_mode, int check_convergence, int patience,
                  double tol, const double *l1W, const double *l2W, const double *l1H, const double *l2H,
                  double *loss_hist , double *time_hist , int64_t cap,
                  int64_t *n_hist , int *converged_early );


int cmf_w_partials(cmf_handle h);
int cmf_w_apply(cmf_handle h, double l1W, double l2W);
int cmf_h_update(cmf_handle h, double l1H, double l2H);
int cmf_loss_partial(cmf_handle h, double *sumsq_out);

int cmf_exchange_buffer(cmf_handle h, int which, void **dev_ptr, int64_t *count, int *dtype);
int cmf_halo_buffers(cmf_handle h, void **send_left, void **send_right, void **recv_left,
                     void **recv_right, int64_t *count);

int cmf_sync(cmf_handle h);
int cmf_launch_count(cmf_handle h, int64_t *out);
int cmf_stream(cmf_handle h, void **stream_out);
int cmf_set_stream(cmf_handle h, void *stream);
int cmf_profile(cmf_handle h, int enable);
int cmf_profile_read(cmf_handle h, int which, double *ms_total, int64_t *count);
int cmf_set_engine(cmf_handle h, int engine);
int cmf_set_loss_mode(cmf_handle h, int mode);
int cmf_get_loss_mode(cmf_handle h, int *mode_out);
int cmf_set_loss_guard(cmf_handle h, double guard, int max_interval);
int cmf_get_loss_stats(cmf_handle h, int64_t *n_direct, int64_t *n_expansion, int *interval, double *last_err);
int cmf_get_fd_layout(cmf_handle h, int *block_len, int *hop, int64_t *nblocks);
int cmf_get_engine(cmf_handle h, int *engine_out);

int cmf_set_pgd_loss(cmf_handle h, int loss_func, const void *mask);
int cmf_set_pgd_constraints(cmf_handle h, int constrW, int constrH);


int cmf_tensor_conv(int64_t N, int64_t T, int64_t K, int64_t L, int dtype, const void *W,
                    const void *H, void *out);
int cmf_tensor_transconv(int64_t N, int64_t T, int64_t K, int64_t L, int dtype, const void *W,
                         const void *X, void *out);
int cmf_corr_w(int64_t N, int64_t T, int64_t K, int64_t L, int dtype, const void *H,
               const void *X, void *out);
int cmf_compute_resids(int64_t N, int64_t T, int64_t K, int64_t L, int dtype, const void *X,
                       const void *W, const void *H, void *out);
int cmf_shift_and_stack(int64_t K, int64_t T, int64_t L, int dtype, const void *H, void *out);

#ifdef __cplusplus
}
#endif
#endif
```

Baseline: 24.97.

## Fuse inverse FFT, multiplicative update, and forward FFT into single FD step kernels

Adds fd_w_step and fd_h_step kernels that take the frequency-domain correlation output, inverse-FFT it in shared memory, apply the multiplicative update to W or H in place, and forward-FFT the new factor straight into the bf16 hi/lo spectrum buffers. The separate ifft-numerator, mu_update and later fft-of-factor launches, along with their global-memory round trips, are skipped on the single-rank MULT path. Dirty flags are adjusted so the freshly written spectrum is reused, and a debug accessor for the spectra is added. This gives higher per-kernel shared memory and register pressure, and the W spectrum now depends on the update ordering being correct.

```diff
diff --git a/cmf.jl_b200/_lib.py b/cmf.jl_b200/_lib.py
--- a/cmf.jl_b200/_lib.py
+++ b/cmf.jl_b200/_lib.py
@@ -53,6 +53,7 @@
     "cmf_set_engine": [_h, _int],
     "cmf_get_engine": [_h, _c.POINTER(_int)],
     "cmf_get_fd_layout": [_h, _c.POINTER(_int), _c.POINTER(_int), _c.POINTER(_i64)],
+    "cmf_get_fd_operand": [_h, _int, _vp, _vp, _c.POINTER(_i64)],
     "cmf_set_loss_mode": [_h, _int],
     "cmf_get_loss_mode": [_h, _c.POINTER(_int)],
     "cmf_set_loss_guard": [_h, _dbl, _int],
diff --git a/cmf.jl_b200/csrc/cmf_sm100.cu b/cmf.jl_b200/csrc/cmf_sm100.cu
--- a/cmf.jl_b200/csrc/cmf_sm100.cu
+++ b/cmf.jl_b200/csrc/cmf_sm100.cu
@@ -319,6 +319,8 @@
         CK(cudaStreamSynchronize(stream));
     }
 
+    struct MuStep { double l1, l2; double *dot_dst; };
+
     static constexpr bool is_f32 = std::is_same<S, float>::value;
     bool tc_active() const { return engine >= 1 && tcs.ok; }
     bool fd_active() const { return engine == 2 && tcs.ok && fds.ok; }
@@ -417,6 +419,7 @@
                 CK(cudaFuncSetAttribute(fd::fft_w_kernel<LB, CW>, cudaFuncAttributeMaxDynamicSharedMemorySize, w));
                 CK(cudaFuncSetAttribute(fd::ifft_numW_kernel<float, LB, CW>, cudaFuncAttributeMaxDynamicSharedMemorySize, w));
                 CK(cudaFuncSetAttribute(fd::ifft_numW_kernel<double, LB, CW>, cudaFuncAttributeMaxDynamicSharedMemorySize, w));
+                CK(cudaFuncSetAttribute(fd::fd_w_step_kernel<LB, CW>, cudaFuncAttributeMaxDynamicSharedMemorySize, w));
             });
             for (int ch : {8, 16, 32}) {
                 if (LB == 10 && ch == 32) continue;
@@ -425,6 +428,7 @@
                     constexpr int CH = decltype(c)::value;
                     CK(cudaFuncSetAttribute(fd::fft_h_kernel<LB, CH>, cudaFuncAttributeMaxDynamicSharedMemorySize, h));
                     CK(cudaFuncSetAttribute(fd::ifft_numH_kernel<LB, CH>, cudaFuncAttributeMaxDynamicSharedMemorySize, h));
+                    CK(cudaFuncSetAttribute(fd::fd_h_step_kernel<LB, CH>, cudaFuncAttributeMaxDynamicSharedMemorySize, h));
                 });
             }
         });
@@ -482,7 +486,7 @@
         post_launch();
         f.x_dirty = false;
     }
-    void fd_corr() {
+    void fd_corr(bool keep_spectrum) {
         FdState &f = fds;
         fd_build_X();
         fd_spectrum_H();
@@ -498,7 +502,17 @@
         tc::tc_kernel<tc::TC_FQC><<<grid, tc::THREADS, tc::SMEM_BYTES, stream>>>(f.mAh[0], f.mAh[1], f.mXfMN[0], f.mXfMN[1], q);
         prof_end();
         post_launch();
+        if (keep_spectrum) return;
         fd_ifft_numW(f.Df.p, numW.p, N, N);
+        post_launch();
+    }
+    void fd_w_step(double l1W, double l2W) {
+        FdState &f = fds;
+        const int C = fd_cols_w();
+        fd_with_bc(f.logB, C, [&](auto lb, auto c) {
+            fd::fd_w_step_kernel<decltype(lb)::value, decltype(c)::value><<<dim3((unsigned)cdiv(N, 2 * C), (unsigned)K), fd::NT, fd_smem(C), stream>>>(
+                f.Df.p, Wi.p, denW.p, (float)l1W, (float)l2W, f.Aw_hi.p, f.Aw_lo.p, N, K, L, f.Kq, f.tw.p);
+        });
         post_launch();
     }
     void fd_denomH() {
@@ -591,6 +605,26 @@
         post_launch();
         f.h_dirty = false;
     }
+    void fd_spectrum_W() {
+        FdState &f = fds;
+        if (!f.w_dirty) return;
+        fd_fft_w(Wi.p, f.Aw_hi.p, f.Aw_lo.p, N, L, 2 * N, N, 0);
+        post_launch();
+        f.w_dirty = false;
+    }
+    void fd_operand(int which, void *hi, void *lo, int64_t *count) {
+        if (!fd_active()) throw CmfError(CMF_ERR_UNSUPPORTED, "the frequency-domain engine is not active on this handle");
+        REQUIRE(which == 0 || which == 1, "which must be 0 (spectrum of W) or 1 (spectrum of H)");
+        if constexpr (is_f32) {
+            FdState &f = fds;
+            if (which == 0) fd_spectrum_W(); else fd_spectrum_H();
+            const DevBuf<__nv_bfloat16> &bh = which ? f.Ah_hi : f.Aw_hi, &bl = which ? f.Ah_lo : f.Aw_lo;
+            *count = (int64_t)bh.n;
+            if (hi) CK(cudaMemcpyAsync(hi, bh.p, bh.n * sizeof(__nv_bfloat16), cudaMemcpyDeviceToHost, stream));
+            if (lo) CK(cudaMemcpyAsync(lo, bl.p, bl.n * sizeof(__nv_bfloat16), cudaMemcpyDeviceToHost, stream));
+            CK(cudaStreamSynchronize(stream));
+        }
+    }
     void fd_gram() {
         FdState &f = fds;
         f.hf2_valid = false;
@@ -610,14 +644,10 @@
         fd_ifft_numW(f.Gf.p, exch1.p, K, f.Kq);
         post_launch();
     }
-    void fd_transconv() {
+    void fd_transconv(const MuStep *upd) {
         FdState &f = fds;
         fd_build_X();
-        if (f.w_dirty) {
-            fd_fft_w(Wi.p, f.Aw_hi.p, f.Aw_lo.p, N, L, 2 * N, N, 0);
-            post_launch();
-            f.w_dirty = false;
-        }
+        fd_spectrum_W();
         tc::Params q = tc_base_params();
         q.nprod = 3;
         q.tiles_n = cdiv(f.nblkp, tc::BN);
@@ -630,8 +660,22 @@
         tc::tc_kernel<tc::TC_FQT><<<grid, tc::THREADS, tc::SMEM_BYTES, stream>>>(f.mAw[0], f.mAw[1], f.mXfK[0], f.mXfK[1], q);
         prof_end();
         post_launch();
+        if (upd) { fd_h_step(*upd); return; }
         fd_ifft_numH(f.Of.p, numH.p, f.nblk, f.V, f.nblkp);
         post_launch();
+    }
+    void fd_h_step(const MuStep &u) {
+        FdState &f = fds;
+        const int C = fd_cols_h();
+        const int64_t grid = f.nblkp * (f.Kq / 2 / C);
+        if (u.dot_dst && mu_part.n < (size_t)grid) mu_part.alloc((size_t)grid);
+        fd_with_bc(f.logB, C, [&](auto lb, auto c) {
+            fd::fd_h_step_kernel<decltype(lb)::value, decltype(c)::value><<<(unsigned)grid, fd::NT, fd_smem(C), stream>>>(
+                f.Of.p, numH.p, H, denH.p, (float)u.l1, (float)u.l2, f.Ah_hi.p, f.Ah_lo.p, K, Tl, f.V, f.nblkp, f.Kq, fd_order(f.nblkp),
+                f.tw.p, u.dot_dst ? mu_part.p : nullptr);
+        });
+        post_launch();
+        if (u.dot_dst) reduce_scalar(mu_part.p, grid, u.dot_dst);
     }
     bool tc_available() {
         if constexpr (is_f32) {
@@ -1107,12 +1151,13 @@
         numH_valid = numH_dot_valid = false;
         calib_reset();
     }
-    void w_changed() {
-        tcs.w_dirty = fds.w_dirty = fds.wx_dirty = true;
+    void w_changed(bool aw_fresh = false) {
+        tcs.w_dirty = fds.wx_dirty = true;
+        fds.w_dirty = !aw_fresh;
         numH_valid = numH_dot_valid = false;
     }
-    void h_changed() {
-        gram_valid = false; fds.h_dirty = true; fds.hf2_valid = false;
+    void h_changed(bool ah_fresh = false) {
+        gram_valid = false; fds.h_dirty = !ah_fresh; fds.hf2_valid = false;
         numH_valid = numH_dot_valid = false;
     }
     void factors_replaced() { w_changed(); h_changed(); calib_reset(); }
@@ -1403,13 +1448,21 @@
     }
 
 
-    void compute_numW() {
+    bool compute_numW(bool keep_spectrum = false) {
         if (!tc_active()) launch_corr(X.p, N, N, Tl + (L - 1), nsplit_w, split_w, numW.p, nullptr);
-        else if constexpr (is_f32) { if (fd_active()) fd_corr(); else tc_corr(); }
-    }
-    void compute_numH() {
+        else if constexpr (is_f32) {
+            if (fd_active()) { fd_corr(keep_spectrum); return keep_spectrum; }
+            tc_corr();
+        }
+        return false;
+    }
+    bool compute_numH(const MuStep *upd = nullptr) {
         if (!tc_active()) launch_transconv(Wi.p, X.p, numH.p, N, K, L, N, Tl, Tl + (L - 1));
-        else if constexpr (is_f32) { if (fd_active()) fd_transconv(); else tc_transconv(); }
+        else if constexpr (is_f32) {
+            if (fd_active()) { fd_transconv(upd); return upd != nullptr; }
+            tc_transconv();
+        }
+        return false;
     }
     void compute_denomW(int64_t j0, int64_t j1) {
         if (!tc_active()) {
@@ -1445,11 +1498,19 @@
         post_launch();
     }
 
-    void w_partials() {
+    bool w_partials(bool keep_spectrum = false) {
         REQUIRE(have_data && have_factors, "update: data and factors must be set first");
-        compute_numW();
+        const bool spectrum = compute_numW(keep_spectrum);
         if (!gram_valid) gram_partial();
         gram_valid = false;
+        return spectrum;
+    }
+    void w_update(double l1W, double l2W) {
+        const bool fused = w_partials(true);
+        w_denom_rows(0, KL());
+        if (!fused) { w_update_rows(l1W, l2W, 0, KL()); return; }
+        if constexpr (is_f32) fd_w_step(l1W, l2W);
+        w_changed(true);
     }
 
     void w_apply(double l1W, double l2W) {
@@ -1499,12 +1560,13 @@
         post_launch();
     }
 
-    void h_update(double l1H, double l2H) {
+    void h_update(double l1H, double l2H, bool fused) {
         REQUIRE(have_data && have_factors, "update: data and factors must be set first");
-        compute_numH();
         compute_denomH();
-        const bool dot = launch_mu(H, numH.p, denH.p, l1H, l2H, Tl * K, (loss_mode == 1 && alg == CMF_MULT) ? scal.p + 4 : nullptr);
-        h_changed();
+        const MuStep u{l1H, l2H, (loss_mode == 1 && alg == CMF_MULT) ? scal.p + 4 : nullptr};
+        const bool ah_fresh = compute_numH(fused ? &u : nullptr);
+        const bool dot = ah_fresh ? u.dot_dst != nullptr : launch_mu(H, numH.p, denH.p, l1H, l2H, Tl * K, u.dot_dst);
+        h_changed(ah_fresh);
         numH_valid = (alg == CMF_MULT);
         numH_dot_valid = dot;
     }
@@ -2036,6 +2098,7 @@
 template <typename S>
 void r_update_motifs(Ctx<S> &ctx, double l1W, double l2W) {
     if (ctx.alg == CMF_PGD) { ctx.pgd_update_motifs(l1W, l2W); return; }
+    if (ctx.world() == 1 && ctx.alg == CMF_MULT) { ctx.w_update(l1W, l2W); return; }
     ctx.w_partials();
     const int64_t KL = ctx.K * ctx.L;
     if (ctx.world() > 1 && ctx.alg == CMF_MULT && KL % ctx.world() == 0 && !getenv("CMF_W_REPLICATED")) {
@@ -2128,7 +2191,7 @@
         else r_hals_sweep_sharded(ctx, l1H, l2H);
         ctx.h_changed();
     } else {
-        ctx.h_update(l1H, l2H);
+        ctx.h_update(l1H, l2H, true);
     }
     c_halo_exchange(ctx);
     return r_guarded_loss(ctx);
@@ -2578,7 +2641,7 @@
         single_rank(h);
         on_ranks(h, [&](auto &r) {
             REQUIRE(r.alg == CMF_MULT, "the split-phase H update is MultUpdate only");
-            r.h_update(l1H, l2H);
+            r.h_update(l1H, l2H, false);
         });
     });
 }
@@ -2689,6 +2752,13 @@
         on_first(h, [&](auto &r) { r.fd_layout(block_len, hop, nblocks); });
     });
 }
+int cmf_get_fd_operand(cmf_handle h, int which, void *hi_out, void *lo_out, int64_t *count) {
+    return guarded([&] {
+        REQUIRE(h && count, "null argument");
+        single_rank(h);
+        on_first(h, [&](auto &r) { r.fd_operand(which, hi_out, lo_out, count); });
+    });
+}
 int cmf_get_engine(cmf_handle h, int *engine_out) {
     return guarded([&] { REQUIRE(h && engine_out, "null argument"); *engine_out = first(h).engine; });
 }
diff --git a/cmf.jl_b200/csrc/kernels_fd.cuh b/cmf.jl_b200/csrc/kernels_fd.cuh
--- a/cmf.jl_b200/csrc/kernels_fd.cuh
+++ b/cmf.jl_b200/csrc/kernels_fd.cuh
@@ -150,91 +150,35 @@
     *reinterpret_cast<uint32_t *>(lo + idx) = l;
 }
 
-template <int LOGB>
-__global__ void __launch_bounds__(NT, CMF_FD_MINB)
-fft_x_kernel(const float *__restrict__ X, __nv_bfloat16 *__restrict__ hi, __nv_bfloat16 *__restrict__ lo, int64_t N, int64_t xcols,
-             int V, int64_t nblkp, int64_t nbx, const float2 *__restrict__ twg) {
-    constexpr int B = 1 << LOGB, C = 16, ISTEP = NT / C;
-    extern __shared__ float2 fd_smem[];
-    float2 *d = fd_smem, *tw = fd_smem + B * C;
-    int b, tile;
-    grid_block_tile(nbx, (int)((N + 31) / 32), b, tile);
-    const int p = threadIdx.x % C;
-    const int n = tile * 32 + 2 * p;
-    load_twiddles<B>(tw, twg);
-    {
-        const int i0 = threadIdx.x / C;
-        const int64_t lim64 = xcols - (int64_t)b * V;
-        const int lim = (n < N) ? (int)(lim64 < 0 ? 0 : (lim64 > B ? B : lim64)) : 0;
-        const float *src = X + ((int64_t)b * V + i0) * N + n;
-        float2 *dst = d + i0 * C + p;
-#pragma unroll 1
-        for (int i = i0; i < B; i += LD_U * ISTEP, src += (int64_t)LD_U * ISTEP * N, dst += LD_U * ISTEP * C) {
-            float2 v[LD_U];
-#pragma unroll
-            for (int u = 0; u < LD_U; ++u) {
-                v[u] = make_float2(0.f, 0.f);
-                if (i + u * ISTEP < lim) v[u] = *reinterpret_cast<const float2 *>(src + (int64_t)u * ISTEP * N);
-            }
-#pragma unroll
-            for (int u = 0; u < LD_U; ++u)
-                if (B % (LD_U * ISTEP) == 0 || i + u * ISTEP < B) dst[u * ISTEP * C] = v[u];
-        }
-    }
-    __syncthreads();
-    fft_passes<false, LOGB, C>(d, tw);
-    if (n >= N) return;
-    for (int f = threadIdx.x / C; f <= B / 2; f += NT / C) {
-        float2 re, im;
-        unpack_pair<LOGB, C>(d, f, p, re, im);
-        const int64_t r = ((int64_t)f * nblkp + b) * 2;
-        store_split2(hi, lo, r * N + n, re);
-        store_split2(hi, lo, (r + 1) * N + n, im);
-    }
-}
-
-template <int LOGB, int C>
-__global__ void __launch_bounds__(NT, CMF_FD_MINB)
-fft_h_kernel(const float *__restrict__ H, __nv_bfloat16 *__restrict__ hi, __nv_bfloat16 *__restrict__ lo, int64_t K, int64_t Tl,
-             int64_t hcols, int V, int64_t nblkp, int full, int64_t t_off, int kq, int64_t nbx,
-             const float2 *__restrict__ twg) {
-    constexpr int B = 1 << LOGB, ISTEP = NT / C;
+template <int LOGB, int C>
+__device__ __forceinline__ void fill_h_spectrum(float2 *d, const float *__restrict__ Of, int64_t b, int k, int64_t nblkp, int kq) {
+    constexpr int B = 1 << LOGB, FSTEP = NT / C;
     const int64_t KQ = kq, MROWS = 2 * kq;
-    extern __shared__ float2 fd_smem[];
-    float2 *d = fd_smem, *tw = fd_smem + B * C;
-    int bi, tile;
-    grid_block_tile(nbx, (kq / 2) / C, bi, tile);
-    const int64_t b = bi;
-    const int p = threadIdx.x % C;
-    const int k = 2 * (tile * C + p);
-    load_twiddles<B>(tw, twg);
-    {
-        const int i0 = threadIdx.x / C;
-        const int64_t tb = b * V + t_off;
-        const int64_t lim64 = full ? (hcols - tb) : ((Tl - tb < V) ? Tl - tb : V);
-        const int lim = (int)(lim64 < 0 ? 0 : (lim64 > B ? B : lim64));
-        const float *src = H + (tb + i0) * K + k;
-        float2 *dst = d + i0 * C + p;
-        const bool pair = ((K & 1) == 0) && (k + 1 < K);
-#pragma unroll 1
-        for (int i = i0; i < B; i += LD_U * ISTEP, src += (int64_t)LD_U * ISTEP * K, dst += LD_U * ISTEP * C) {
-            float2 v[LD_U];
-#pragma unroll
-            for (int u = 0; u < LD_U; ++u) {
-                v[u] = make_float2(0.f, 0.f);
-                if (i + u * ISTEP < lim) {
-                    const float *q = src + (int64_t)u * ISTEP * K;
-                    if (pair) v[u] = *reinterpret_cast<const float2 *>(q);
-                    else { if (k < K) v[u].x = q[0]; if (k + 1 < K) v[u].y = q[1]; }
-                }
-            }
-#pragma unroll
-            for (int u = 0; u < LD_U; ++u)
-                if (B % (LD_U * ISTEP) == 0 || i + u * ISTEP < B) dst[u * ISTEP * C] = v[u];
-        }
-    }
-    __syncthreads();
-    fft_passes<false, LOGB, C>(d, tw);
+    const int p = threadIdx.x % C;
+    const int f0 = threadIdx.x / C;
+    const int64_t ustep = (int64_t)FSTEP * nblkp * MROWS;
+    const float *o = Of + ((int64_t)f0 * nblkp + b) * MROWS + k;
+#pragma unroll 1
+    for (int f = f0; f <= B / 2; f += 4 * FSTEP, o += 4 * ustep) {
+        float2 re[4], im[4];
+#pragma unroll
+        for (int u = 0; u < 4; ++u)
+            if (f + u * FSTEP <= B / 2) {
+                const float *q = o + u * ustep;
+                re[u] = *reinterpret_cast<const float2 *>(q); im[u] = *reinterpret_cast<const float2 *>(q + KQ);
+            }
+#pragma unroll
+        for (int u = 0; u < 4; ++u)
+            if (f + u * FSTEP <= B / 2) pack_pair<LOGB, C>(d, f + u * FSTEP, p, re[u], im[u]);
+    }
+}
+
+template <int LOGB, int C>
+__device__ __forceinline__ void store_h_spectrum(const float2 *d, __nv_bfloat16 *__restrict__ hi, __nv_bfloat16 *__restrict__ lo, int64_t b,
+                                                 int k, int64_t nblkp, int full, int kq) {
+    constexpr int B = 1 << LOGB;
+    const int64_t KQ = kq, MROWS = 2 * kq;
+    const int p = threadIdx.x % C;
     const int64_t rs = full ? 2 * KQ : 2 * MROWS;
     const int64_t rstep = (int64_t)(NT / C) * nblkp * rs;
     int64_t r = ((int64_t)(threadIdx.x / C) * nblkp + b) * rs + k;
@@ -258,42 +202,36 @@
 }
 
 template <int LOGB, int C>
-__global__ void __launch_bounds__(NT, CMF_FD_MINB)
-fft_w_kernel(const float *__restrict__ Wi, __nv_bfloat16 *__restrict__ hi, __nv_bfloat16 *__restrict__ lo, int64_t N, int64_t K,
-             int64_t L, int64_t ldw, int64_t coff, int xmode, int kq, const float2 *__restrict__ twg) {
-    constexpr int B = 1 << LOGB, ISTEP = NT / C;
+__device__ __forceinline__ void fill_w_spectrum(float2 *d, const float *__restrict__ Df, int64_t k, int64_t n, int64_t N, int64_t ldi, int kq) {
+    constexpr int B = 1 << LOGB, FSTEP = NT / C;
     const int64_t KQ = kq, MROWS = 2 * kq;
-    extern __shared__ float2 fd_smem[];
-    float2 *d = fd_smem, *tw = fd_smem + B * C;
-    const int64_t k = blockIdx.y;
-    const int p = threadIdx.x % C;
-    const int64_t n = (int64_t)blockIdx.x * (2 * C) + 2 * p;
-    load_twiddles<B>(tw, twg);
-    {
-        const int i0 = threadIdx.x / C;
-        const float *src = Wi + ((int64_t)i0 * K + k) * N + n;
-        float2 *dst = d + i0 * C + p;
-#pragma unroll 1
-        for (int i = i0; i < B; i += LD_U * ISTEP, src += (int64_t)LD_U * ISTEP * K * N, dst += LD_U * ISTEP * C) {
-            float2 v[LD_U];
-#pragma unroll
-            for (int u = 0; u < LD_U; ++u) {
-                const int ii = i + u * ISTEP;
-                v[u] = make_float2(0.f, 0.f);
-                if (ii < L && n < N) {
-                    const float *q = src + (int64_t)u * ISTEP * K * N;
-                    if ((N & 1) == 0) v[u] = *reinterpret_cast<const float2 *>(q);
-                    else { v[u].x = q[0]; if (n + 1 < N) v[u].y = q[1]; }
-                }
-            }
-#pragma unroll
-            for (int u = 0; u < LD_U; ++u)
-                if (B % (LD_U * ISTEP) == 0 || i + u * ISTEP < B) dst[u * ISTEP * C] = v[u];
-        }
-    }
-    __syncthreads();
-    fft_passes<false, LOGB, C>(d, tw);
-    if (n >= N) return;
+    const int p = threadIdx.x % C;
+    const int f0 = threadIdx.x / C;
+    const int64_t ustep = (int64_t)FSTEP * MROWS * ldi;
+    const float *src = Df + ((int64_t)f0 * MROWS + k) * ldi + n;
+#pragma unroll 1
+    for (int f = f0; f <= B / 2; f += 4 * FSTEP, src += 4 * ustep) {
+        float2 re[4], im[4];
+#pragma unroll
+        for (int u = 0; u < 4; ++u) {
+            re[u] = make_float2(0.f, 0.f); im[u] = re[u];
+            if (f + u * FSTEP <= B / 2 && n < N) {
+                re[u] = *reinterpret_cast<const float2 *>(src + u * ustep);
+                im[u] = *reinterpret_cast<const float2 *>(src + u * ustep + KQ * ldi);
+            }
+        }
+#pragma unroll
+        for (int u = 0; u < 4; ++u)
+            if (f + u * FSTEP <= B / 2) pack_pair<LOGB, C>(d, f + u * FSTEP, p, re[u], im[u]);
+    }
+}
+
+template <int LOGB, int C>
+__device__ __forceinline__ void store_w_spectrum(const float2 *d, __nv_bfloat16 *__restrict__ hi, __nv_bfloat16 *__restrict__ lo, int64_t k,
+                                                 int64_t n, int64_t N, int64_t ldw, int64_t coff, int xmode, int kq) {
+    constexpr int B = 1 << LOGB;
+    const int64_t KQ = kq, MROWS = 2 * kq;
+    const int p = threadIdx.x % C;
     for (int f = threadIdx.x / C; f <= B / 2; f += NT / C) {
         float2 re, im;
         unpack_pair<LOGB, C>(d, f, p, re, im);
@@ -314,12 +252,137 @@
     }
 }
 
+template <int LOGB>
+__global__ void __launch_bounds__(NT, CMF_FD_MINB)
+fft_x_kernel(const float *__restrict__ X, __nv_bfloat16 *__restrict__ hi, __nv_bfloat16 *__restrict__ lo, int64_t N, int64_t xcols,
+             int V, int64_t nblkp, int64_t nbx, const float2 *__restrict__ twg) {
+    constexpr int B = 1 << LOGB, C = 16, ISTEP = NT / C;
+    extern __shared__ float2 fd_smem[];
+    float2 *d = fd_smem, *tw = fd_smem + B * C;
+    int b, tile;
+    grid_block_tile(nbx, (int)((N + 31) / 32), b, tile);
+    const int p = threadIdx.x % C;
+    const int n = tile * 32 + 2 * p;
+    load_twiddles<B>(tw, twg);
+    {
+        const int i0 = threadIdx.x / C;
+        const int64_t lim64 = xcols - (int64_t)b * V;
+        const int lim = (n < N) ? (int)(lim64 < 0 ? 0 : (lim64 > B ? B : lim64)) : 0;
+        const float *src = X + ((int64_t)b * V + i0) * N + n;
+        float2 *dst = d + i0 * C + p;
+#pragma unroll 1
+        for (int i = i0; i < B; i += LD_U * ISTEP, src += (int64_t)LD_U * ISTEP * N, dst += LD_U * ISTEP * C) {
+            float2 v[LD_U];
+#pragma unroll
+            for (int u = 0; u < LD_U; ++u) {
+                v[u] = make_float2(0.f, 0.f);
+                if (i + u * ISTEP < lim) v[u] = *reinterpret_cast<const float2 *>(src + (int64_t)u * ISTEP * N);
+            }
+#pragma unroll
+            for (int u = 0; u < LD_U; ++u)
+                if (B % (LD_U * ISTEP) == 0 || i + u * ISTEP < B) dst[u * ISTEP * C] = v[u];
+        }
+    }
+    __syncthreads();
+    fft_passes<false, LOGB, C>(d, tw);
+    if (n >= N) return;
+    for (int f = threadIdx.x / C; f <= B / 2; f += NT / C) {
+        float2 re, im;
+        unpack_pair<LOGB, C>(d, f, p, re, im);
+        const int64_t r = ((int64_t)f * nblkp + b) * 2;
+        store_split2(hi, lo, r * N + n, re);
+        store_split2(hi, lo, (r + 1) * N + n, im);
+    }
+}
+
+template <int LOGB, int C>
+__global__ void __launch_bounds__(NT, CMF_FD_MINB)
+fft_h_kernel(const float *__restrict__ H, __nv_bfloat16 *__restrict__ hi, __nv_bfloat16 *__restrict__ lo, int64_t K, int64_t Tl,
+             int64_t hcols, int V, int64_t nblkp, int full, int64_t t_off, int kq, int64_t nbx,
+             const float2 *__restrict__ twg) {
+    constexpr int B = 1 << LOGB, ISTEP = NT / C;
+    extern __shared__ float2 fd_smem[];
+    float2 *d = fd_smem, *tw = fd_smem + B * C;
+    int bi, tile;
+    grid_block_tile(nbx, (kq / 2) / C, bi, tile);
+    const int64_t b = bi;
+    const int p = threadIdx.x % C;
+    const int k = 2 * (tile * C + p);
+    load_twiddles<B>(tw, twg);
+    {
+        const int i0 = threadIdx.x / C;
+        const int64_t tb = b * V + t_off;
+        const int64_t lim64 = full ? (hcols - tb) : ((Tl - tb < V) ? Tl - tb : V);
+        const int lim = (int)(lim64 < 0 ? 0 : (lim64 > B ? B : lim64));
+        const float *src = H + (tb + i0) * K + k;
+        float2 *dst = d + i0 * C + p;
+        const bool pair = ((K & 1) == 0) && (k + 1 < K);
+#pragma unroll 1
+        for (int i = i0; i < B; i += LD_U * ISTEP, src += (int64_t)LD_U * ISTEP * K, dst += LD_U * ISTEP * C) {
+            float2 v[LD_U];
+#pragma unroll
+            for (int u = 0; u < LD_U; ++u) {
+                v[u] = make_float2(0.f, 0.f);
+                if (i + u * ISTEP < lim) {
+                    const float *q = src + (int64_t)u * ISTEP * K;
+                    if (pair) v[u] = *reinterpret_cast<const float2 *>(q);
+                    else { if (k < K) v[u].x = q[0]; if (k + 1 < K) v[u].y = q[1]; }
+                }
+            }
+#pragma unroll
+            for (int u = 0; u < LD_U; ++u)
+                if (B % (LD_U * ISTEP) == 0 || i + u * ISTEP < B) dst[u * ISTEP * C] = v[u];
+        }
+    }
+    __syncthreads();
+    fft_passes<false, LOGB, C>(d, tw);
+    store_h_spectrum<LOGB, C>(d, hi, lo, b, k, nblkp, full, kq);
+}
+
+template <int LOGB, int C>
+__global__ void __launch_bounds__(NT, CMF_FD_MINB)
+fft_w_kernel(const float *__restrict__ Wi, __nv_bfloat16 *__restrict__ hi, __nv_bfloat16 *__restrict__ lo, int64_t N, int64_t K,
+             int64_t L, int64_t ldw, int64_t coff, int xmode, int kq, const float2 *__restrict__ twg) {
+    constexpr int B = 1 << LOGB, ISTEP = NT / C;
+    extern __shared__ float2 fd_smem[];
+    float2 *d = fd_smem, *tw = fd_smem + B * C;
+    const int64_t k = blockIdx.y;
+    const int p = threadIdx.x % C;
+    const int64_t n = (int64_t)blockIdx.x * (2 * C) + 2 * p;
+    load_twiddles<B>(tw, twg);
+    {
+        const int i0 = threadIdx.x / C;
+        const float *src = Wi + ((int64_t)i0 * K + k) * N + n;
+        float2 *dst = d + i0 * C + p;
+#pragma unroll 1
+        for (int i = i0; i < B; i += LD_U * ISTEP, src += (int64_t)LD_U * ISTEP * K * N, dst += LD_U * ISTEP * C) {
+            float2 v[LD_U];
+#pragma unroll
+            for (int u = 0; u < LD_U; ++u) {
+                const int ii = i + u * ISTEP;
+                v[u] = make_float2(0.f, 0.f);
+                if (ii < L && n < N) {
+                    const float *q = src + (int64_t)u * ISTEP * K * N;
+                    if ((N & 1) == 0) v[u] = *reinterpret_cast<const float2 *>(q);
+                    else { v[u].x = q[0]; if (n + 1 < N) v[u].y = q[1]; }
+                }
+            }
+#pragma unroll
+            for (int u = 0; u < LD_U; ++u)
+                if (B % (LD_U * ISTEP) == 0 || i + u * ISTEP < B) dst[u * ISTEP * C] = v[u];
+        }
+    }
+    __syncthreads();
+    fft_passes<false, LOGB, C>(d, tw);
+    if (n >= N) return;
+    store_w_spectrum<LOGB, C>(d, hi, lo, k, n, N, ldw, coff, xmode, kq);
+}
+
 template <int LOGB, int C>
 __global__ void __launch_bounds__(NT, CMF_FD_MINB)
 ifft_numH_kernel(const float *__restrict__ Of, float *__restrict__ numH, int64_t K, int64_t Tl, int V, int64_t nblkp, int kq,
                  int64_t nbx, const float2 *__restrict__ twg) {
-    constexpr int B = 1 << LOGB, FSTEP = NT / C;
-    const int64_t KQ = kq, MROWS = 2 * kq;
+    constexpr int B = 1 << LOGB;
     extern __shared__ float2 fd_smem[];
     float2 *d = fd_smem, *tw = fd_smem + B * C;
     int bi, tile;
@@ -328,24 +391,7 @@
     const int p = threadIdx.x % C;
     const int k = 2 * (tile * C + p);
     load_twiddles<B>(tw, twg);
-    {
-        const int f0 = threadIdx.x / C;
-        const int64_t ustep = (int64_t)FSTEP * nblkp * MROWS;
-        const float *o = Of + ((int64_t)f0 * nblkp + b) * MROWS + k;
-#pragma unroll 1
-        for (int f = f0; f <= B / 2; f += 4 * FSTEP, o += 4 * ustep) {
-            float2 re[4], im[4];
-#pragma unroll
-            for (int u = 0; u < 4; ++u)
-                if (f + u * FSTEP <= B / 2) {
-                    const float *q = o + u * ustep;
-                    re[u] = *reinterpret_cast<const float2 *>(q); im[u] = *reinterpret_cast<const float2 *>(q + KQ);
-                }
-#pragma unroll
-            for (int u = 0; u < 4; ++u)
-                if (f + u * FSTEP <= B / 2) pack_pair<LOGB, C>(d, f + u * FSTEP, p, re[u], im[u]);
-        }
-    }
+    fill_h_spectrum<LOGB, C>(d, Of, b, k, nblkp, kq);
     __syncthreads();
     fft_passes<true, LOGB, C>(d, tw);
     const float2 sc = bcast(1.0f / (float)B);
@@ -438,34 +484,14 @@
 __global__ void __launch_bounds__(NT, CMF_FD_MINB)
 ifft_numW_kernel(const float *__restrict__ Df, OutT *__restrict__ out, int64_t N, int64_t ldi, int64_t K, int64_t L, int kq,
                  const float2 *__restrict__ twg) {
-    constexpr int B = 1 << LOGB, FSTEP = NT / C;
-    const int64_t KQ = kq, MROWS = 2 * kq;
+    constexpr int B = 1 << LOGB;
     extern __shared__ float2 fd_smem[];
     float2 *d = fd_smem, *tw = fd_smem + B * C;
     const int64_t k = blockIdx.y;
     const int p = threadIdx.x % C;
     const int64_t n = (int64_t)blockIdx.x * (2 * C) + 2 * p;
     load_twiddles<B>(tw, twg);
-    {
-        const int f0 = threadIdx.x / C;
-        const int64_t ustep = (int64_t)FSTEP * MROWS * ldi;
-        const float *src = Df + ((int64_t)f0 * MROWS + k) * ldi + n;
-#pragma unroll 1
-        for (int f = f0; f <= B / 2; f += 4 * FSTEP, src += 4 * ustep) {
-            float2 re[4], im[4];
-#pragma unroll
-            for (int u = 0; u < 4; ++u) {
-                re[u] = make_float2(0.f, 0.f); im[u] = re[u];
-                if (f + u * FSTEP <= B / 2 && n < N) {
-                    re[u] = *reinterpret_cast<const float2 *>(src + u * ustep);
-                    im[u] = *reinterpret_cast<const float2 *>(src + u * ustep + KQ * ldi);
-                }
-            }
-#pragma unroll
-            for (int u = 0; u < 4; ++u)
-                if (f + u * FSTEP <= B / 2) pack_pair<LOGB, C>(d, f + u * FSTEP, p, re[u], im[u]);
-        }
-    }
+    fill_w_spectrum<LOGB, C>(d, Df, k, n, N, ldi, kq);
     __syncthreads();
     fft_passes<true, LOGB, C>(d, tw);
     if (n >= N) return;
@@ -482,5 +508,128 @@
     }
 }
 
-}
-}
+constexpr int STEP_H = 2;
+
+__device__ __forceinline__ float2 load_kpair(const float *__restrict__ a, int64_t idx, int k, int64_t K) {
+    if (((K & 1) == 0) && (k + 1 < K)) return *reinterpret_cast<const float2 *>(a + idx);
+    float2 v = make_float2(0.f, 0.f);
+    if (k < K) v.x = a[idx];
+    if (k + 1 < K) v.y = a[idx + 1];
+    return v;
+}
+__device__ __forceinline__ void store_kpair(float *__restrict__ a, int64_t idx, int k, int64_t K, float2 v) {
+    if (((K & 1) == 0) && (k + 1 < K)) { *reinterpret_cast<float2 *>(a + idx) = v; return; }
+    if (k < K) a[idx] = v.x;
+    if (k + 1 < K) a[idx + 1] = v.y;
+}
+
+template <int LOGB, int C>
+__global__ void __launch_bounds__(NT, 2)
+fd_h_step_kernel(const float *__restrict__ Of, float *__restrict__ numH, float *__restrict__ H, const float *__restrict__ denH, float l1,
+                 float l2, __nv_bfloat16 *__restrict__ hi, __nv_bfloat16 *__restrict__ lo, int64_t K, int64_t Tl, int V, int64_t nblkp,
+                 int kq, int64_t nbx, const float2 *__restrict__ twg, double *__restrict__ partial) {
+    constexpr int B = 1 << LOGB, JSTEP = NT / C;
+    extern __shared__ float2 fd_smem[];
+    __shared__ double red[32];
+    float2 *d = fd_smem, *tw = fd_smem + B * C;
+    int bi, tile;
+    grid_block_tile(nbx, (kq / 2) / C, bi, tile);
+    const int64_t b = bi;
+    const int p = threadIdx.x % C;
+    const int k = 2 * (tile * C + p);
+    load_twiddles<B>(tw, twg);
+    fill_h_spectrum<LOGB, C>(d, Of, b, k, nblkp, kq);
+    __syncthreads();
+    fft_passes<true, LOGB, C>(d, tw);
+    const float2 sc = bcast(1.0f / (float)B);
+    const int64_t tb = b * V;
+    const int lim = (int)(Tl - tb < 0 ? 0 : (Tl - tb < V ? Tl - tb : V));
+    const float2 z0 = make_float2(0.f, 0.f);
+    double acc = 0.0;
+#pragma unroll 1
+    for (int i0 = threadIdx.x / C; i0 < B; i0 += STEP_H * JSTEP) {
+        float2 hv[2 * STEP_H], dv[2 * STEP_H];
+#pragma unroll
+        for (int s = 0; s < 2 * STEP_H; ++s) {
+            const int i = i0 + (s / 2) * JSTEP, j = rev<LOGB>(i & (B - 1)), r = (s & 1) ? j : i;
+            hv[s] = dv[s] = z0;
+            if (i < B && (s & 1 ? j > i : j >= i) && r < lim) {
+                hv[s] = load_kpair(H, (tb + r) * K + k, k, K);
+                dv[s] = load_kpair(denH, (tb + r) * K + k, k, K);
+            }
+        }
+#pragma unroll
+        for (int u = 0; u < STEP_H; ++u) {
+            const int i = i0 + u * JSTEP, j = rev<LOGB>(i & (B - 1));
+            if (i >= B || j < i) continue;
+            const float2 z[2] = {mul2(d[j * C + p], sc), mul2(d[i * C + p], sc)};
+            const int rows[2] = {i, j};
+#pragma unroll
+            for (int q = 0; q < 2; ++q) {
+                const int r = rows[q];
+                if (q == 1 && j == i) break;
+                float2 h = z0;
+                if (r < lim) {
+                    const int s = 2 * u + q;
+                    const int64_t idx = (tb + r) * K + k;
+                    h = make_float2(k < K ? mu_elem(hv[s].x, z[q].x, dv[s].x, l1, l2) : 0.f,
+                                    k + 1 < K ? mu_elem(hv[s].y, z[q].y, dv[s].y, l1, l2) : 0.f);
+                    store_kpair(numH, idx, k, K, z[q]);
+                    store_kpair(H, idx, k, K, h);
+                    acc += (double)z[q].x * (double)h.x + (double)z[q].y * (double)h.y;
+                }
+                d[r * C + p] = h;
+            }
+        }
+    }
+    if (partial) {
+        acc = block_sum(acc, red);
+        if (threadIdx.x == 0) partial[blockIdx.x] = acc;
+    }
+    __syncthreads();
+    fft_passes<false, LOGB, C>(d, tw);
+    store_h_spectrum<LOGB, C>(d, hi, lo, b, k, nblkp, 0, kq);
+}
+
+template <int LOGB, int C>
+__global__ void __launch_bounds__(NT, CMF_FD_MINB)
+fd_w_step_kernel(const float *__restrict__ Df, float *__restrict__ Wi, const float *__restrict__ denW, float l1, float l2,
+                 __nv_bfloat16 *__restrict__ hi, __nv_bfloat16 *__restrict__ lo, int64_t N, int64_t K, int64_t L, int kq,
+                 const float2 *__restrict__ twg) {
+    constexpr int B = 1 << LOGB;
+    extern __shared__ float2 fd_smem[];
+    float2 *d = fd_smem, *tw = fd_smem + B * C;
+    const int64_t k = blockIdx.y;
+    const int p = threadIdx.x % C;
+    const int64_t n = (int64_t)blockIdx.x * (2 * C) + 2 * p;
+    load_twiddles<B>(tw, twg);
+    fill_w_spectrum<LOGB, C>(d, Df, k, n, N, N, kq);
+    __syncthreads();
+    fft_passes<true, LOGB, C>(d, tw);
+    const float2 sc = bcast(1.0f / (float)B);
+    const int lim = n < N ? (int)L : 0;
+    auto step = [&](float2 z, int l) {
+        const int64_t idx = ((int64_t)l * K + k) * N + n;
+        z = mul2(z, sc);
+        const float2 v = *reinterpret_cast<const float2 *>(Wi + idx), dn = *reinterpret_cast<const float2 *>(denW + idx);
+        const float2 w = make_float2(mu_elem(v.x, z.x, dn.x, l1, l2), mu_elem(v.y, z.y, dn.y, l1, l2));
+        *reinterpret_cast<float2 *>(Wi + idx) = w;
+        return w;
+    };
+#pragma unroll 1
+    for (int i = threadIdx.x / C; i < B; i += NT / C) {
+        const int j = rev<LOGB>(i);
+        if (j < i) continue;
+        const float2 zi = d[j * C + p], zj = d[i * C + p];
+        const float2 z0 = make_float2(0.f, 0.f);
+        d[i * C + p] = i < lim ? step(zi, i) : z0;
+        if (j != i) d[j * C + p] = j < lim ? step(zj, j) : z0;
+    }
+    __syncthreads();
+    fft_passes<false, LOGB, C>(d, tw);
+    if (n >= N) return;
+    store_w_spectrum<LOGB, C>(d, hi, lo, k, n, N, 2 * N, N, 0, kq);
+}
+
+}
+}
diff --git a/cmf.jl_b200/csrc/kernels_simt.cuh b/cmf.jl_b200/csrc/kernels_simt.cuh
--- a/cmf.jl_b200/csrc/kernels_simt.cuh
+++ b/cmf.jl_b200/csrc/kernels_simt.cuh
@@ -710,6 +710,13 @@
 }
 
 template <typename S>
+__device__ __forceinline__ S mu_elem(S v, S num, S den, S l1, S l2) {
+    const S eps = (S)CMF_EPS;
+    v = v * (num / (den + l1 + S(2) * l2 * v + eps));
+    return v > eps ? v : eps;
+}
+
+template <typename S>
 __global__ void mu_update_kernel(S *__restrict__ x, const S *__restrict__ num, const S *__restrict__ den,
                                  S l1, S l2, int64_t n, const double *__restrict__ reg = nullptr,
                                  const int *__restrict__ active = nullptr, int64_t inner = 1, const int *__restrict__ col_rest = nullptr,
@@ -722,24 +729,20 @@
         l1 = (S)reg[4 * r];
         l2 = (S)reg[4 * r + 1];
     }
-    const S eps = (S)CMF_EPS;
-    S v = x[i];
-    v = v * (num[i] / (den[i] + l1 + S(2) * l2 * v + eps));
-    x[i] = v > eps ? v : eps;
+    x[i] = mu_elem(x[i], num[i], den[i], l1, l2);
 }
 
 __global__ void __launch_bounds__(256) mu_update_vec4_kernel(float4 *__restrict__ x, const float4 *__restrict__ num, const float4 *__restrict__ den,
                                                              float l1, float l2, int64_t n4, double *__restrict__ partial) {
     __shared__ double red[32];
-    const float eps = (float)CMF_EPS;
     double acc = 0.0;
     for (int64_t i = (int64_t)blockIdx.x * blockDim.x + threadIdx.x; i < n4; i += (int64_t)gridDim.x * blockDim.x) {
         float4 v = x[i];
         const float4 a = __ldg(num + i), d = __ldg(den + i);
-        v.x = v.x * (a.x / (d.x + l1 + 2.f * l2 * v.x + eps)); v.x = v.x > eps ? v.x : eps;
-        v.y = v.y * (a.y / (d.y + l1 + 2.f * l2 * v.y + eps)); v.y = v.y > eps ? v.y : eps;
-        v.z = v.z * (a.z / (d.z + l1 + 2.f * l2 * v.z + eps)); v.z = v.z > eps ? v.z : eps;
-        v.w = v.w * (a.w / (d.w + l1 + 2.f * l2 * v.w + eps)); v.w = v.w > eps ? v.w : eps;
+        v.x = mu_elem(v.x, a.x, d.x, l1, l2);
+        v.y = mu_elem(v.y, a.y, d.y, l1, l2);
+        v.z = mu_elem(v.z, a.z, d.z, l1, l2);
+        v.w = mu_elem(v.w, a.w, d.w, l1, l2);
         x[i] = v;
         if (partial) acc += (double)a.x * (double)v.x + (double)a.y * (double)v.y + (double)a.z * (double)v.z + (double)a.w * (double)v.w;
     }
diff --git a/include/cmf_sm100.h b/include/cmf_sm100.h
--- a/include/cmf_sm100.h
+++ b/include/cmf_sm100.h
@@ -106,6 +106,7 @@
 int cmf_set_loss_guard(cmf_handle h, double guard, int max_interval);
 int cmf_get_loss_stats(cmf_handle h, int64_t *n_direct, int64_t *n_expansion, int *interval, double *last_err);
 int cmf_get_fd_layout(cmf_handle h, int *block_len, int *hop, int64_t *nblocks);
+int cmf_get_fd_operand(cmf_handle h, int which, void *hi_out, void *lo_out, int64_t *count);
 int cmf_get_engine(cmf_handle h, int *engine_out);
 
 int cmf_set_pgd_loss(cmf_handle h, int loss_func, const void *mask);
```

Result: no change. 24.93 (median of 6 runs) (-0.1%).
